# vshmyhlo/retinanet-tensorflow

Hardware: AMD Instinct MI355X
Metric: train images/sec (MobileNetV2-FPN RetinaNet 512x512, bs=2/GPU) (higher is better)
Workload: dtype f32

## Files before the change

include/rn_hip.h:

```cpp
#ifndef RN_HIP_H
#define RN_HIP_H

#include <stddef.h>
#include <stdint.h>

#ifdef __cplusplus
extern "C" {
#endif

typedef void* rn_stream_t;

enum rn_status {
  RN_OK = 0,
  RN_EINVAL = -1,
  RN_EUNSUPPORTED = -2,
  RN_EHIP = -3,
  RN_EWORKSPACE = -4
};

enum rn_act { RN_ACT_NONE = 0, RN_ACT_RELU = 1, RN_ACT_ELU = 2, RN_ACT_RELU6 = 3, RN_ACT_SIGMOID = 4 };
enum rn_loss_mode { RN_LOSS_BCE_DICE = 0, RN_LOSS_FOCAL = 1 };
enum rn_opt { RN_OPT_MOMENTUM = 0, RN_OPT_RMSPROP = 1, RN_OPT_ADAM = 2 };

#define RN_MAX_SEG 16

typedef struct rn_reduce_list rn_reduce_list;

#define RN_API_VERSION 408
int rn_version(void);
const char* rn_last_error(void);

void rn_same_pad(int n, int k, int s, int* out, int* pad_before);

typedef struct rn_conv_seg {
  const float* x;
  const float* wgt;
  const float* bias;
  float* y;
  const float* dy;
  float* dx;
  int32_t n, h, w;
  int32_t cout;
  int32_t x_ld;
  int32_t x_coff;
  int64_t wgt_bytes;
} rn_conv_seg;

typedef struct rn_conv_geom {
  int32_t kh, kw, stride, cin;
  int32_t groups;
} rn_conv_geom;

size_t rn_conv2d_fwd_workspace(const rn_conv_seg* segs, int nseg, const rn_conv_geom* g);
size_t rn_conv2d_dgrad_workspace(const rn_conv_seg* segs, int nseg, const rn_conv_geom* g);
int rn_conv2d_fwd(const rn_conv_seg* segs, int nseg, const rn_conv_geom* g, void* workspace, size_t workspace_bytes,
                  rn_stream_t stream);
int rn_conv2d_dgrad(const rn_conv_seg* segs, int nseg, const rn_conv_geom* g, void* workspace, size_t workspace_bytes,
                    rn_stream_t stream);
typedef struct rn_gn_rows {
  void* rows;
  int32_t rows_per_sample, per_group, groups;
} rn_gn_rows;
size_t rn_conv2d_stats_rows(const rn_conv_seg* segs, int nseg, const rn_conv_geom* g, size_t workspace_bytes, int groups,
                            rn_gn_rows* layout);
int rn_conv2d_fwd_stats(const rn_conv_seg* segs, int nseg, const rn_conv_geom* g, void* workspace, size_t workspace_bytes,
                        const rn_gn_rows* rows, rn_stream_t stream);

size_t rn_conv2d_dropout_rows(const rn_conv_seg* segs, int nseg, const rn_conv_geom* g, int groups, rn_gn_rows* layout, int* fused_ok);
int rn_conv2d_fwd_dropout(const rn_conv_seg* segs, int nseg, const rn_conv_geom* g, float rate, uint64_t seed, const uint64_t* seed_dev,
                          const rn_gn_rows* rows, rn_stream_t stream);

size_t rn_conv2d_wgrad_workspace(const rn_conv_seg* segs, int nseg, const rn_conv_geom* g);
int rn_conv2d_wgrad(const rn_conv_seg* segs, int nseg, const rn_conv_geom* g, float* dw, int accumulate,
                    void* workspace, size_t workspace_bytes, rn_stream_t stream, rn_reduce_list* defer);

int rn_conv2d_bwd(const rn_conv_seg* segs, int nseg, const rn_conv_geom* g, float* dw, void* workspace,
                  size_t workspace_bytes, rn_stream_t stream, rn_reduce_list* defer);

size_t rn_conv2d_bias_grad_workspace(int cout);
int rn_conv2d_bias_grad(const rn_conv_seg* segs, int nseg, const rn_conv_geom* g, float* dbias, void* workspace,
                        size_t workspace_bytes, rn_stream_t stream, rn_reduce_list* defer);

typedef struct rn_reduce_desc {
  const float* in;
  float* out;
  int32_t count;
  uint16_t nrows, accumulate;
} rn_reduce_desc;
struct rn_reduce_list {
  rn_reduce_desc* desc;
  int32_t capacity;
  int32_t count;
};
int rn_flush_reductions(rn_reduce_list* list, rn_stream_t stream);

size_t rn_conv3x3_winograd_workspace(const rn_conv_seg* segs, int nseg, int cin, int cout, int tile);
int rn_conv3x3_winograd_keep_bytes(const rn_conv_seg* segs, int nseg, int cin, int cout, int tile, size_t* v_bytes,
                                   size_t* urot_bytes);
int rn_conv3x3_winograd(const rn_conv_seg* segs, int nseg, int cin, int cout, const float* w, const float* bias,
                        int dgrad, int tile, void* workspace, size_t workspace_bytes, float* v_buf, float* urot_buf,
                        rn_stream_t stream);
int rn_gemm_batched(const float* A, const float* B, float* C, int M, int K, int N, int nbatch, int b_nk, rn_stream_t stream);
size_t rn_winograd_bwd_products_workspace(int M, int Kw, int Nw, int nbatch);
int rn_winograd_bwd_products(const float* Ad, const float* Bd, float* Cd, int M, int Kd, int Nd, const float* Aw,
                             const float* Bw, int Kw, int Nw, int nbatch, void* workspace, size_t workspace_bytes,
                             int* nsplit, rn_stream_t stream);
size_t rn_conv3x3_winograd_wgrad_workspace(const rn_conv_seg* segs, int nseg, int cin, int cout, int tile);
int rn_conv3x3_winograd_wgrad(const rn_conv_seg* segs, int nseg, int cin, int cout, float* dw, int accumulate, int tile,
                              void* workspace, size_t workspace_bytes, const float* v_buf, rn_stream_t stream);

size_t rn_conv3x3_winograd_bwd_workspace(const rn_conv_seg* segs, int nseg, int cin, int cout, int tile, int have_v, int have_urot);
int rn_conv3x3_winograd_bwd(const rn_conv_seg* segs, int nseg, int cin, int cout, const float* w, float* dw, int accumulate, int tile,
                            void* workspace, size_t workspace_bytes, const float* v_buf, const float* urot_buf, rn_stream_t stream);

int rn_set_product_mode(int mode);
int rn_get_product_mode(void);
int rn_set_x3_bfrag(int on);
int rn_get_x3_bfrag(void);
int rn_x3_bfrag_ok(int M, int K, int N);
size_t rn_x3_bfrag_bytes(int K, int N, int nbatch);
int rn_x3_pack_bfrag(const float* B, void* out, int K, int N, int nbatch, int b_nk, rn_stream_t stream);
int rn_gemm_batched_bfrag(const float* A, const void* Bfrag, float* C, int M, int K, int N, int nbatch, int fwd_name, rn_stream_t stream);

size_t rn_pack_weights_f16_bytes(int kh, int kw, int cin_g, int cout);
int rn_pack_weights_f16(const float* w, void* wt, int kh, int kw, int cin_g, int cout, rn_stream_t stream);
int rn_cast_f32_to_f16(const float* x, void* y, int64_t count, rn_stream_t stream);
int rn_pad_cast_rgb_f16(const float* x, void* y, int64_t pixels, rn_stream_t stream);
int rn_conv2d_fwd_f16(const rn_conv_seg* segs, int nseg, const rn_conv_geom* g, int out_f32, rn_stream_t stream);
typedef struct rn_f16_fold {
  const float* in_mean; const float* in_rstd; const float* in_gamma; const float* in_beta;
  int in_groups; int in_act;
  float* partial;
  const int32_t* seg_chunk_start;
  int32_t total_chunks;
} rn_f16_fold;
int rn_conv2d_f16_fold_rows(const rn_conv_seg* segs, int nseg, const rn_conv_geom* g);
int rn_conv2d_f16_stats_tiles(const rn_conv_seg* segs, int nseg, const rn_conv_geom* g, int32_t* tiles_per_sample);
int rn_conv2d_fwd_f16_fold(const rn_conv_seg* segs, int nseg, const rn_conv_geom* g, const rn_f16_fold* fold, rn_stream_t stream);
int rn_group_norm_finalize(const float* partial, int n, int rows_per_sample, int hw, int c, int groups, float eps, float* mean,
                           float* rstd, rn_stream_t stream);
int rn_group_norm_apply_f16(const void* x, const void* residual, void* y, int n, int hw, int c, int groups, const float* mean,
                            const float* rstd, const float* gamma, const float* beta, int act, int act_after_residual,
                            rn_stream_t stream);
typedef struct rn_gn_residual_norm {
  const float* mean; const float* rstd;
  const float* gamma; const float* beta;
  int groups;
} rn_gn_residual_norm;
int rn_group_norm_apply_res_f16(const void* x, const void* residual, const rn_gn_residual_norm* residual_norm, void* y, int n, int hw, int c,
                                int groups, const float* mean, const float* rstd, const float* gamma, const float* beta, int act,
                                int act_after_residual, rn_stream_t stream);

int rn_depthwise_fwd(const float* x, const float* wgt, float* y, int n, int h, int w, int c, int k, int stride,
                     rn_stream_t stream);
size_t rn_depthwise_stats_rows(int n, int h, int w, int c, int k, int stride, int groups, rn_gn_rows* layout);
int rn_depthwise_fwd_stats(const float* x, const float* wgt, float* y, int n, int h, int w, int c, int k, int stride,
                           const rn_gn_rows* rows, rn_stream_t stream);
int rn_depthwise_dgrad(const float* dy, const float* wgt, float* dx, int n, int h, int w, int c, int k,
                       int stride, rn_stream_t stream);
size_t rn_depthwise_wgrad_workspace(int n, int h, int w, int c, int k, int stride);
int rn_depthwise_bwd(const float* x, const float* dy, const float* wgt, float* dx, float* dw, int n, int h, int w, int c, int k,
                     int stride, void* workspace, size_t workspace_bytes, rn_stream_t stream, rn_reduce_list* defer);
int rn_depthwise_wgrad(const float* x, const float* dy, float* dw, int n, int h, int w, int c, int k, int stride,
                       void* workspace, size_t workspace_bytes, rn_stream_t stream, rn_reduce_list* defer);

typedef struct rn_dwgn_params {
  int32_t n, h, w, c;
  int32_t stride;
  int32_t groups, act;
  float eps, drop_rate;
  uint64_t drop_seed1, drop_seed2;
  const uint64_t* drop_seed_dev;
} rn_dwgn_params;
int rn_dwgn_supported(const rn_dwgn_params* p, int backward);
int rn_dwgn_fwd(const float* x, const float* gamma1, const float* beta1, const float* wgt, const float* gamma2,
                const float* beta2, float* y, float* stats, const rn_dwgn_params* p, rn_stream_t stream);
int rn_dwgn_bwd(const float* x, const float* dy, const float* gamma1, const float* beta1, const float* wgt,
                const float* gamma2, const float* beta2, const float* stats, float* dx, float* rows,
                const rn_dwgn_params* p, rn_stream_t stream);

typedef struct rn_gn_seg {
  const float* x;
  float* y;
  const float* residual;
  const float* dy;
  float* dx;
  float* dresidual;
  float* mean;
  float* rstd;
  int32_t n, hw;
  int32_t x_ld;
  int32_t dx_ld;
  int32_t dx_accumulate;
} rn_gn_seg;

typedef struct rn_gn_params {
  int32_t c, groups, act;
  int32_t act_after_residual;
  int32_t in_f16, out_f16;
  float eps;
  float drop_rate;
  uint64_t drop_seed;
  const uint64_t* drop_seed_dev;
  void* sync;
  const rn_gn_rows* stat_rows;
} rn_gn_params;

size_t rn_group_norm_sync_bytes(void);
int rn_group_norm_rows_ok(int c, int groups, int rows_per_sample, int per_group);
size_t rn_group_norm_workspace(const rn_gn_seg* segs, int nseg, const rn_gn_params* p);
int rn_group_norm_fwd(const rn_gn_seg* segs, int nseg, const rn_gn_params* p, const float* gamma,
                      const float* beta, void* workspace, size_t workspace_bytes, rn_stream_t stream);
int rn_group_norm_fwd_f16_tiles(const rn_gn_seg* segs, int nseg, const rn_gn_params* p, const float* gamma, const float* beta,
                                const float* partial, const int32_t* tiles_per_sample, rn_stream_t stream);
int rn_group_norm_bwd(const rn_gn_seg* segs, int nseg, const rn_gn_params* p, const float* gamma,
                      const float* beta, float* dgamma, float* dbeta, void* workspace, size_t workspace_bytes,
                      rn_stream_t stream, rn_reduce_list* defer);

int rn_act_fwd(const float* x, float* y, int64_t count, int act, rn_stream_t stream);
int rn_act_bwd(const float* x, const float* dy, float* dx, int64_t count, int act, rn_stream_t stream);
int rn_upsample_add_fwd(const float* lateral, const float* top, float* y, int n, int h, int w, int th, int tw, int c,
                        rn_stream_t stream);
int rn_upsample_add_bwd_top(const float* dy, float* dtop, int n, int h, int w, int th, int tw, int c,
                            rn_stream_t stream);

int rn_dropout(const float* x, float* y, int64_t count, float rate, uint64_t seed, const uint64_t* seed_dev,
               rn_stream_t stream);
int rn_dropout_strided(const float* x, float* y, int64_t pixels, int c, int x_ld, int x_coff, int y_ld, int y_coff, float rate,
                       uint64_t seed, const uint64_t* seed_dev, rn_stream_t stream);
int rn_maxpool_fwd(const float* x, float* y, uint8_t* argmax, int n, int h, int w, int c, int k, int stride,
                   rn_stream_t stream);
int rn_act_fwd_f16(const void* x, void* y, int64_t count, int act, rn_stream_t stream);
int rn_maxpool_fwd_f16(const void* x, void* y, int n, int h, int w, int c, int k, int stride, rn_stream_t stream);
int rn_maxpool_gn_fwd_f16(const void* x, void* y, int n, int h, int w, int c, int k, int stride, const float* mean, const float* rstd,
                          const float* gamma, const float* beta, int groups, int act, rn_stream_t stream);
int rn_upsample_add_fwd_f16(const void* lateral, const void* top, void* y, int n, int h, int w, int th, int tw, int c,
                            rn_stream_t stream);
int rn_maxpool_bwd(const float* x, const float* dy, float* dx, int n, int h, int w, int c, int k, int stride,
                   rn_stream_t stream);
int rn_maxpool_bwd_arg(const uint8_t* argmax, const float* dy, float* dx, int n, int h, int w, int c, int k, int stride,
                       rn_stream_t stream);
int rn_avgpool_fwd(const float* x, float* y, int n, int h, int w, int c, int k, int stride, rn_stream_t stream);
int rn_avgpool_bwd(const float* dy, float* dx, int n, int h, int w, int c, int k, int stride, rn_stream_t stream);

int rn_flip_width(const void* x, void* y, int64_t outer, int w, int64_t inner, int elem_bytes, int neg_mod, int neg_idx,
                  rn_stream_t stream);

int rn_resize_bilinear_normalize(const void* x, int in_u8, float* y, int n, int h, int w, int c, int oh, int ow,
                                 const float* mean, const float* stdv, rn_stream_t stream);

typedef struct rn_resize_desc {
  int32_t h, w;
  float hs, ws;
} rn_resize_desc;
int rn_resize_pair_u8(const uint8_t* raw, int64_t raw_capacity, const rn_resize_desc* desc, float* pair, int oh, int ow,
                      const float* mean, const float* stdv, rn_stream_t stream);

typedef struct rn_loss_seg {
  const float* cls_logit;
  const float* cls_label;
  const float* reg_pred;
  const float* reg_label;
  const uint8_t* trainable;
  float* d_cls_logit;
  float* d_reg_pred;
  int64_t rows;
} rn_loss_seg;

#define RN_LOSS_STATS_HEADER 8
size_t rn_loss_workspace(const rn_loss_seg* segs, int nseg, int num_classes);
int rn_loss_fwd(const rn_loss_seg* segs, int nseg, int num_classes, int mode, float* stats, float* class_loss_out,
                float* regr_loss_out, void* workspace, size_t workspace_bytes, rn_stream_t stream);
int rn_loss_bwd(const rn_loss_seg* segs, int nseg, int num_classes, int mode, const float* stats,
                const float* g_cls, const float* g_reg, rn_stream_t stream);

typedef struct rn_wino_gn {
  const float* in_rows;
  const float* in_gamma;
  const float* in_beta;
  int32_t in_groups, in_act;
  float in_eps;
  float* out_rows;
  int32_t out_groups;
  const void* u_ready;
  int32_t urot_ready;
} rn_wino_gn;
size_t rn_wino_gn_rows(const rn_conv_seg* segs, int nseg, int tile);
size_t rn_conv3x3_winograd_gn_u_bytes(int cin, int cout, int tile);
int rn_conv3x3_winograd_gn_weights(const float* w, int cin, int cout, int tile, void* u_out, size_t u_out_bytes, float* urot_out,
                                   rn_stream_t stream);
int rn_conv3x3_winograd_gn(const rn_conv_seg* segs, int nseg, int cin, int cout, const float* w, const float* bias, int tile,
                           const rn_wino_gn* gn, void* workspace, size_t workspace_bytes, float* v_buf, float* urot_buf,
                           rn_stream_t stream);
typedef struct rn_wino_gn_bwd {
  const float* in_rows;
  const float* in_gamma;
  const float* in_beta;
  int32_t in_groups, in_act;
  float in_eps;
  float* in_g_rows_group;
  float* in_g_rows_chan;
  const float* out_rows;
  const float* out_g_rows_group;
  const float* out_gamma;
  int32_t out_groups;
  float out_eps;
  int32_t defer_wgrad;
} rn_wino_gn_bwd;
int rn_conv3x3_winograd_gn_bwd(const rn_conv_seg* segs, int nseg, int cin, int cout, const float* w, float* dw, int accumulate,
                               int tile, const rn_wino_gn_bwd* gn, void* workspace, size_t workspace_bytes, const float* v_buf,
                               const float* urot_buf, rn_stream_t stream);
int rn_conv3x3_winograd_gn_bwd_wgrad(const rn_conv_seg* segs, int nseg, int cin, int cout, float* dw, int accumulate, int tile,
                                     void* workspace, size_t workspace_bytes, const float* v_buf, int urot_was_given, rn_stream_t stream);
int rn_reduce_rows(const float* in, float* out, int64_t count, int nrows, int accumulate, rn_stream_t stream, rn_reduce_list* defer);

typedef struct rn_mb_rows {
  float* rows;
  int32_t rows_per_sample, width, bn;
} rn_mb_rows;

typedef struct rn_mb_norm {
  const float* y;
  rn_mb_rows stat;
  float* mean; float* rstd;
  const float* gamma; const float* beta;
  int32_t c, groups, act;
  float eps, drop_rate;
  uint64_t drop_seed; const uint64_t* drop_seed_dev;
} rn_mb_norm;

int rn_mb_rows_max(void);
size_t rn_mb_compact_rows_layout(int n, const rn_mb_rows* in, rn_mb_rows* out);
int rn_mb_compact_rows(const rn_mb_rows* in, const rn_mb_rows* out, int n, rn_stream_t stream);

size_t rn_mb_pointwise_rows(int n, int hw, int cin, int cout, int groups, rn_mb_rows* layout);
int rn_mb_pointwise_fwd(const float* x, const rn_mb_norm* in, const float* residual, float* materialise, const float* w, float* y,
                        int n, int hw, int cin, int cout, const rn_mb_rows* stat_out, int stat_groups, rn_stream_t stream);
size_t rn_mb_depthwise_rows(int n, int h, int w, int c, int stride, int groups, rn_mb_rows* layout);
int rn_mb_depthwise_fwd(const rn_mb_norm* in, const float* w, float* y, int n, int h, int wd, int stride, const rn_mb_rows* stat_out,
                        int stat_groups, rn_stream_t stream);
int rn_mb_apply(const rn_mb_norm* in, const float* residual, float* out, int n, int hw, rn_stream_t stream);

enum { RN_MB_PHASE_POINTWISE = 0, RN_MB_PHASE_DEPTHWISE = 1 };
typedef struct rn_mb_phase {
  int32_t kind;
  const rn_mb_norm* in;
  const float* residual;
  float* materialise;
  const float* w; float* y;
  int32_t h, wd, cin, cout, stride;
  rn_mb_rows stat_out;
  int32_t stat_groups;
} rn_mb_phase;
size_t rn_mb_resident_sync_bytes(void);
size_t rn_mb_resident_rows(int kind, int n, int h, int wd, int cin, int cout, int stride, int groups, rn_mb_rows* layout);
int rn_mb_resident_fwd(const rn_mb_phase* phases, int nphase, int n, void* sync, rn_stream_t stream);

typedef struct rn_mb_dy {
  const float* dy;
  const rn_mb_norm* norm;
  const float* g;
  int32_t g_plain;
  rn_mb_rows grows;
} rn_mb_dy;
typedef struct rn_mb_gout {
  float* out;
  const float* add1; const float* add2;
  const rn_mb_norm* norm;
  int32_t store_plain;
  rn_mb_rows grows;
  float* planes;
} rn_mb_gout;
size_t rn_mb_pointwise_bwd_rows(int n, int hw, int cin, int cout, int groups, rn_mb_rows* layout);
size_t rn_mb_pointwise_bwd_workspace(int n, int hw, int cin, int cout);
int rn_mb_pointwise_bwd(const float* x, const rn_mb_norm* in, const rn_mb_dy* dy, const float* w, float* dw, const rn_mb_gout* gout,
                        int n, int hw, int cin, int cout, void* workspace, size_t workspace_bytes, rn_stream_t stream,
                        rn_reduce_list* defer);
size_t rn_mb_depthwise_bwd_rows(int n, int h, int w, int c, int stride, int groups, rn_mb_rows* layout);
size_t rn_mb_depthwise_bwd_workspace(int n, int h, int w, int c, int stride);
int rn_mb_depthwise_bwd(const rn_mb_norm* in, const rn_mb_dy* dy, const float* w, float* dw, const rn_mb_gout* gout, int n, int h,
                        int wd, int stride, void* workspace, size_t workspace_bytes, rn_stream_t stream, rn_reduce_list* defer);

int rn_iou(const float* a, int64_t na, const float* b, int64_t nb, int pairwise, float* out, int32_t* malformed,
           rn_stream_t stream);

int rn_anchor_assign(const float* boxes, const int32_t* class_ids, const int32_t* num_obj, int nimg, int max_obj,
                     const float* anchor_sizes, int num_anchors, int grid_h, int grid_w, int num_classes,
                     float* cls_out, float* reg_out, uint8_t* trainable_out, int32_t* argmax_out,
                     rn_stream_t stream);
#define RN_MAX_LEVELS 8
typedef struct rn_assign_level {
  const float* anchor_sizes;
  int grid_h, grid_w;
  float* cls_out;
  float* reg_out;
  uint8_t* trainable_out;
  int32_t* argmax_out;
} rn_assign_level;
int rn_anchor_assign_levels(const float* boxes, const int32_t* class_ids, const int32_t* num_obj, int nimg, int max_obj,
                            const rn_assign_level* levels, int nlevel, int num_anchors, int num_classes,
                            rn_stream_t stream);
int rn_anchor_assign_levels_pair(const float* boxes, const int32_t* class_ids, const int32_t* num_obj, int nimg, int max_obj,
                                 const rn_assign_level* levels, int nlevel, int num_anchors, int num_classes,
                                 rn_stream_t stream);

int rn_decode_boxes(const float* reg, const float* anchor_sizes, float* boxes, int n, int h, int w, int num_anchors,
                    rn_stream_t stream);

typedef struct rn_det_level {
  const void* prob;
  const float* boxes;
  int64_t rows_per_image;
  const void* regression;
  const float* anchor_sizes;
  int32_t grid_h, grid_w, num_anchors;
  int32_t prob_f16;
  int32_t regression_f16;
  int32_t prob_is_logit;
} rn_det_level;

typedef struct rn_det_params {
  int32_t n, num_classes, max_per_class;
  float score_threshold, iou_threshold;
  int64_t max_candidates;
} rn_det_params;

size_t rn_detect_workspace(const rn_det_level* levels, int nlevels, const rn_det_params* p);
int rn_detect(const rn_det_level* levels, int nlevels, const rn_det_params* p, float* out_boxes, float* out_scores,
              int32_t* out_class, int32_t* out_image, int64_t* out_anchor, int64_t* counts, void* workspace,
              size_t workspace_bytes, rn_stream_t stream);

int rn_boxes_decode(const rn_det_level* levels, int nlevels, const rn_det_params* p, float* out_boxes,
                    float* out_scores, int32_t* out_class, int32_t* out_image, int64_t* out_anchor, int64_t* counts,
                    void* workspace, size_t workspace_bytes, rn_stream_t stream);
size_t rn_nms_classwise_workspace(const rn_det_params* p);
int rn_nms_classwise(const float* boxes, const float* scores, const int32_t* class_ids, const int32_t* image_ids,
                     const int64_t* count_dev, const rn_det_params* p, float* out_boxes, float* out_scores,
                     int32_t* out_class, int32_t* out_image, int64_t* out_index, int64_t* counts, void* workspace,
                     size_t workspace_bytes, rn_stream_t stream);

#define RN_OPT_BLOCK 1024
size_t rn_optimizer_workspace(int64_t count);
int rn_grad_norm_l2reg(const float* w, const float* grad, const float* wd_per_block, int64_t count,
                       float grad_scale, float* out2, void* workspace, size_t workspace_bytes, rn_stream_t stream);
int rn_optimizer_step(int kind, float* w, const float* grad, float* state1, float* state2,
                      const float* wd_per_block, int64_t count, float lr, float grad_scale, float clip_norm,
                      const float* norm_sq, int64_t step, uint64_t* advance_counter, uint64_t advance_by, rn_stream_t stream);
int64_t rn_optimizer_norm_pairs(int64_t count);
int rn_optimizer_step_norm(int kind, float* w, const float* grad, float* state1, float* state2, const float* wd_per_block,
                           int64_t count, float lr, float grad_scale, int64_t step, uint64_t* advance_counter,
                           uint64_t advance_by, double* partial, rn_stream_t stream);
int rn_norm_reg_finalize(const double* partial, int64_t npairs, float* out2, rn_stream_t stream);
int rn_counter_add(uint64_t* counter, uint64_t inc, rn_stream_t stream);
int rn_zero(float* p, int64_t count, rn_stream_t stream);

typedef struct rn_add_seg { const float* a; const float* b; float* out; int64_t count; } rn_add_seg;
int rn_add_segs(const rn_add_seg* segs, int nseg, rn_stream_t stream);

int rn_debug_collective_standin(const void* src, void* dst, int64_t bytes, int blocks, float target_us, rn_stream_t stream);

#ifdef __cplusplus
}
#endif
#endif
```

retinanet-tensorflow_amd/_rn.py:

```python
import ctypes as C
import os

import torch

_HERE = os.path.dirname(os.path.abspath(__file__))
LIB_PATH = os.environ.get("RN_LIB_PATH") or os.path.join(_HERE, "librn_hip.so")

MAX_SEG = 16
ACT = {None: 0, "none": 0, "linear": 0, "relu": 1, "elu": 2, "relu6": 3, "sigmoid": 4}
LOSS_MODE = {"bce_dice": 0, "focal": 1}
OPT = {"momentum": 0, "rmsprop": 1, "adam": 2}
OPT_BLOCK = 1024
LOSS_STATS_HEADER = 8
API_VERSION = 408


class RnError(RuntimeError):
    pass


class ConvSeg(C.Structure):
    _fields_ = [("x", C.c_void_p), ("wgt", C.c_void_p), ("bias", C.c_void_p), ("y", C.c_void_p),
                ("dy", C.c_void_p), ("dx", C.c_void_p),
                ("n", C.c_int32), ("h", C.c_int32), ("w", C.c_int32), ("cout", C.c_int32),
                ("x_ld", C.c_int32), ("x_coff", C.c_int32), ("wgt_bytes", C.c_int64)]


class AssignLevel(C.Structure):
    _fields_ = [("anchor_sizes", C.c_void_p), ("grid_h", C.c_int32), ("grid_w", C.c_int32), ("cls_out", C.c_void_p),
                ("reg_out", C.c_void_p), ("trainable_out", C.c_void_p), ("argmax_out", C.c_void_p)]


class ConvGeom(C.Structure):
    _fields_ = [("kh", C.c_int32), ("kw", C.c_int32), ("stride", C.c_int32), ("cin", C.c_int32),
                ("groups", C.c_int32)]


class WinoGn(C.Structure):
    _fields_ = [("in_rows", C.c_void_p), ("in_gamma", C.c_void_p), ("in_beta", C.c_void_p), ("in_groups", C.c_int32),
                ("in_act", C.c_int32), ("in_eps", C.c_float), ("out_rows", C.c_void_p), ("out_groups", C.c_int32),
                ("u_ready", C.c_void_p), ("urot_ready", C.c_int32)]


class WinoGnBwd(C.Structure):
    _fields_ = [("in_rows", C.c_void_p), ("in_gamma", C.c_void_p), ("in_beta", C.c_void_p), ("in_groups", C.c_int32),
                ("in_act", C.c_int32), ("in_eps", C.c_float), ("in_g_rows_group", C.c_void_p), ("in_g_rows_chan", C.c_void_p),
                ("out_rows", C.c_void_p), ("out_g_rows_group", C.c_void_p), ("out_gamma", C.c_void_p),
                ("out_groups", C.c_int32), ("out_eps", C.c_float), ("defer_wgrad", C.c_int32)]


class ReduceDesc(C.Structure):
    _fields_ = [("in_", C.c_void_p), ("out", C.c_void_p), ("count", C.c_int32), ("nrows", C.c_uint16), ("accumulate", C.c_uint16)]


class ReduceList(C.Structure):
    _fields_ = [("desc", C.POINTER(ReduceDesc)), ("capacity", C.c_int32), ("count", C.c_int32)]

    @classmethod
    def make(cls, capacity=1024):
        arr = (ReduceDesc * capacity)()
        lst = cls(C.cast(arr, C.POINTER(ReduceDesc)), capacity, 0)
        lst._keep = arr
        return lst


class AddSeg(C.Structure):
    _fields_ = [("a", C.c_void_p), ("b", C.c_void_p), ("out", C.c_void_p), ("count", C.c_int64)]


class DwGnParams(C.Structure):
    _fields_ = [("n", C.c_int32), ("h", C.c_int32), ("w", C.c_int32), ("c", C.c_int32), ("stride", C.c_int32),
                ("groups", C.c_int32), ("act", C.c_int32), ("eps", C.c_float), ("drop_rate", C.c_float),
                ("drop_seed1", C.c_uint64), ("drop_seed2", C.c_uint64), ("drop_seed_dev", C.c_void_p)]


class GnSeg(C.Structure):
    _fields_ = [("x", C.c_void_p), ("y", C.c_void_p), ("residual", C.c_void_p), ("dy", C.c_void_p),
                ("dx", C.c_void_p), ("dresidual", C.c_void_p), ("mean", C.c_void_p), ("rstd", C.c_void_p),
                ("n", C.c_int32), ("hw", C.c_int32), ("x_ld", C.c_int32), ("dx_ld", C.c_int32), ("dx_accumulate", C.c_int32)]


class GnParams(C.Structure):
    _fields_ = [("c", C.c_int32), ("groups", C.c_int32), ("act", C.c_int32), ("act_after_residual", C.c_int32),
                ("in_f16", C.c_int32), ("out_f16", C.c_int32), ("eps", C.c_float),
                ("drop_rate", C.c_float), ("drop_seed", C.c_uint64), ("drop_seed_dev", C.c_void_p), ("sync", C.c_void_p),
                ("stat_rows", C.c_void_p)]


class GnRows(C.Structure):
    _fields_ = [("rows", C.c_void_p), ("rows_per_sample", C.c_int32), ("per_group", C.c_int32), ("groups", C.c_int32)]


class GnResidualNorm(C.Structure):
    _fields_ = [("mean", C.c_void_p), ("rstd", C.c_void_p), ("gamma", C.c_void_p), ("beta", C.c_void_p), ("groups", C.c_int)]


class F16Fold(C.Structure):
    _fields_ = [("in_mean", C.c_void_p), ("in_rstd", C.c_void_p), ("in_gamma", C.c_void_p), ("in_beta", C.c_void_p),
                ("in_groups", C.c_int32), ("in_act", C.c_int32), ("partial", C.c_void_p),
                ("seg_chunk_start", C.c_void_p), ("total_chunks", C.c_int32)]


class MbRows(C.Structure):
    _fields_ = [("rows", C.c_void_p), ("rows_per_sample", C.c_int32), ("width", C.c_int32), ("bn", C.c_int32)]


class MbNorm(C.Structure):
    _fields_ = [("y", C.c_void_p), ("stat", MbRows), ("mean", C.c_void_p), ("rstd", C.c_void_p), ("gamma", C.c_void_p),
                ("beta", C.c_void_p), ("c", C.c_int32), ("groups", C.c_int32), ("act", C.c_int32), ("eps", C.c_float),
                ("drop_rate", C.c_float), ("drop_seed", C.c_uint64), ("drop_seed_dev", C.c_void_p)]


class MbPhase(C.Structure):
    _fields_ = [("kind", C.c_int32), ("in_", C.POINTER(MbNorm)), ("residual", C.c_void_p), ("materialise", C.c_void_p),
                ("w", C.c_void_p), ("y", C.c_void_p), ("h", C.c_int32), ("wd", C.c_int32), ("cin", C.c_int32), ("cout", C.c_int32),
                ("stride", C.c_int32), ("stat_out", MbRows), ("stat_groups", C.c_int32)]


MB_PHASE_POINTWISE, MB_PHASE_DEPTHWISE = 0, 1


class MbDy(C.Structure):
    _fields_ = [("dy", C.c_void_p), ("norm", C.POINTER(MbNorm)), ("g", C.c_void_p), ("g_plain", C.c_int32), ("grows", MbRows)]


class MbGout(C.Structure):
    _fields_ = [("out", C.c_void_p), ("add1", C.c_void_p), ("add2", C.c_void_p), ("norm", C.POINTER(MbNorm)),
                ("store_plain", C.c_int32), ("grows", MbRows), ("planes", C.c_void_p)]


class LossSeg(C.Structure):
    _fields_ = [("cls_logit", C.c_void_p), ("cls_label", C.c_void_p), ("reg_pred", C.c_void_p),
                ("reg_label", C.c_void_p), ("trainable", C.c_void_p), ("d_cls_logit", C.c_void_p),
                ("d_reg_pred", C.c_void_p), ("rows", C.c_int64)]


class DetLevel(C.Structure):
    _fields_ = [("prob", C.c_void_p), ("boxes", C.c_void_p), ("rows_per_image", C.c_int64),
                ("regression", C.c_void_p), ("anchor_sizes", C.c_void_p),
                ("grid_h", C.c_int32), ("grid_w", C.c_int32), ("num_anchors", C.c_int32),
                ("prob_f16", C.c_int32), ("regression_f16", C.c_int32), ("prob_is_logit", C.c_int32)]


class DetParams(C.Structure):
    _fields_ = [("n", C.c_int32), ("num_classes", C.c_int32), ("max_per_class", C.c_int32),
                ("score_threshold", C.c_float), ("iou_threshold", C.c_float), ("max_candidates", C.c_int64)]


_lib = None

SYMBOLS = [
    "rn_version", "rn_last_error", "rn_same_pad",
    "rn_conv2d_fwd_workspace", "rn_conv2d_dgrad_workspace",
    "rn_zero", "rn_conv2d_fwd", "rn_conv2d_stats_rows", "rn_conv2d_fwd_stats", "rn_conv2d_dropout_rows", "rn_conv2d_fwd_dropout", "rn_depthwise_stats_rows", "rn_depthwise_fwd_stats", "rn_group_norm_rows_ok",
    "rn_conv2d_dgrad", "rn_conv2d_wgrad_workspace", "rn_conv2d_wgrad", "rn_conv2d_bwd",
    "rn_conv2d_bias_grad_workspace", "rn_conv2d_bias_grad", "rn_conv3x3_winograd_workspace", "rn_conv3x3_winograd",
    "rn_conv3x3_winograd_wgrad_workspace", "rn_conv3x3_winograd_wgrad", "rn_conv3x3_winograd_keep_bytes",
    "rn_conv3x3_winograd_bwd_workspace", "rn_conv3x3_winograd_bwd", "rn_flush_reductions", "rn_gemm_batched",
    "rn_winograd_bwd_products_workspace", "rn_winograd_bwd_products", "rn_wino_gn_rows", "rn_conv3x3_winograd_gn", "rn_conv3x3_winograd_gn_bwd", "rn_conv3x3_winograd_gn_bwd_wgrad", "rn_reduce_rows", "rn_resize_bilinear_normalize", "rn_resize_pair_u8",
    "rn_dwgn_supported", "rn_dwgn_fwd", "rn_dwgn_bwd", "rn_depthwise_fwd", "rn_depthwise_dgrad", "rn_depthwise_wgrad_workspace", "rn_depthwise_wgrad", "rn_depthwise_bwd",
    "rn_group_norm_sync_bytes", "rn_group_norm_workspace", "rn_group_norm_fwd", "rn_group_norm_bwd",
    "rn_act_fwd", "rn_act_bwd", "rn_upsample_add_fwd", "rn_upsample_add_bwd_top",
    "rn_pack_weights_f16", "rn_pack_weights_f16_bytes", "rn_cast_f32_to_f16", "rn_pad_cast_rgb_f16", "rn_conv2d_fwd_f16", "rn_conv2d_f16_fold_rows", "rn_conv2d_fwd_f16_fold", "rn_group_norm_finalize", "rn_group_norm_apply_f16", "rn_group_norm_apply_res_f16", "rn_maxpool_fwd_f16", "rn_maxpool_gn_fwd_f16", "rn_upsample_add_fwd_f16",
    "rn_act_fwd_f16", "rn_flip_width", "rn_dropout", "rn_dropout_strided", "rn_maxpool_fwd", "rn_maxpool_bwd", "rn_maxpool_bwd_arg", "rn_avgpool_fwd", "rn_avgpool_bwd",
    "rn_loss_workspace", "rn_loss_fwd", "rn_loss_bwd",
    "rn_iou", "rn_anchor_assign", "rn_anchor_assign_levels", "rn_anchor_assign_levels_pair", "rn_decode_boxes", "rn_detect_workspace", "rn_detect",
    "rn_boxes_decode", "rn_nms_classwise_workspace", "rn_nms_classwise",
    "rn_optimizer_workspace", "rn_grad_norm_l2reg", "rn_optimizer_step", "rn_counter_add", "rn_add_segs",
    "rn_mb_rows_max", "rn_mb_compact_rows_layout", "rn_mb_compact_rows", "rn_mb_pointwise_rows", "rn_mb_pointwise_fwd", "rn_mb_depthwise_rows", "rn_mb_depthwise_fwd", "rn_mb_apply",
    "rn_mb_resident_sync_bytes", "rn_mb_resident_rows", "rn_mb_resident_fwd", "rn_set_product_mode", "rn_get_product_mode",
    "rn_set_x3_bfrag", "rn_get_x3_bfrag", "rn_x3_bfrag_ok", "rn_x3_bfrag_bytes", "rn_x3_pack_bfrag", "rn_gemm_batched_bfrag", "rn_conv3x3_winograd_gn_u_bytes", "rn_conv3x3_winograd_gn_weights",
    "rn_conv2d_f16_stats_tiles", "rn_group_norm_fwd_f16_tiles",
    "rn_mb_pointwise_bwd_rows", "rn_mb_pointwise_bwd_workspace", "rn_mb_pointwise_bwd",
    "rn_mb_depthwise_bwd_rows", "rn_mb_depthwise_bwd_workspace", "rn_mb_depthwise_bwd",
    "rn_debug_collective_standin", "rn_optimizer_norm_pairs", "rn_optimizer_step_norm", "rn_norm_reg_finalize",
]


def lib():
    global _lib
    if _lib is None:
        if not os.path.exists(LIB_PATH):
            raise RnError("librn_hip.so not found at %s: build it with "
                          "`make -C retinanet-tensorflow_amd/csrc` (there is no fallback path)" % LIB_PATH)
        L = C.CDLL(LIB_PATH)
        if not hasattr(L, "rn_version") or L.rn_version() != API_VERSION:
            raise RnError("%s reports ABI version %s, these bindings need %d: rebuild it (make -C retinanet-tensorflow_amd/csrc)"
                          % (LIB_PATH, L.rn_version() if hasattr(L, "rn_version") else "none", API_VERSION))
        L.rn_last_error.restype = C.c_char_p
        L.rn_group_norm_sync_bytes.argtypes = []
        for name in ("rn_conv2d_wgrad_workspace", "rn_depthwise_wgrad_workspace", "rn_group_norm_workspace", "rn_group_norm_sync_bytes",
                     "rn_loss_workspace", "rn_detect_workspace", "rn_optimizer_workspace",
                     "rn_conv2d_bias_grad_workspace", "rn_nms_classwise_workspace", "rn_conv3x3_winograd_workspace", "rn_conv2d_fwd_workspace",
                     "rn_conv2d_dgrad_workspace",
                     "rn_conv3x3_winograd_wgrad_workspace", "rn_conv3x3_winograd_bwd_workspace", "rn_wino_gn_rows",
                     "rn_winograd_bwd_products_workspace", "rn_conv2d_stats_rows", "rn_depthwise_stats_rows", "rn_conv2d_dropout_rows",
                     "rn_x3_bfrag_bytes", "rn_conv3x3_winograd_gn_u_bytes"):
            getattr(L, name).restype = C.c_size_t
        L.rn_optimizer_workspace.argtypes = [C.c_int64]
        L.rn_dwgn_supported.argtypes = [C.c_void_p, C.c_int]
        L.rn_dwgn_fwd.argtypes = [C.c_void_p] * 10
        L.rn_dwgn_bwd.argtypes = [C.c_void_p] * 12
        L.rn_depthwise_fwd.argtypes = [C.c_void_p] * 3 + [C.c_int] * 6 + [C.c_void_p]
        L.rn_depthwise_dgrad.argtypes = [C.c_void_p] * 3 + [C.c_int] * 6 + [C.c_void_p]
        L.rn_depthwise_bwd.argtypes = [C.c_void_p] * 5 + [C.c_int] * 6 + [C.c_void_p, C.c_size_t, C.c_void_p, C.c_void_p]
        L.rn_depthwise_wgrad_workspace.argtypes = [C.c_int] * 6
        L.rn_depthwise_wgrad.argtypes = [C.c_void_p] * 3 + [C.c_int] * 6 + [C.c_void_p, C.c_size_t, C.c_void_p, C.c_void_p]
        L.rn_conv2d_fwd.argtypes = [C.c_void_p, C.c_int, C.c_void_p, C.c_void_p, C.c_size_t, C.c_void_p]
        L.rn_conv2d_dgrad.argtypes = [C.c_void_p, C.c_int, C.c_void_p, C.c_void_p, C.c_size_t, C.c_void_p]
        L.rn_zero.argtypes = [C.c_void_p, C.c_int64, C.c_void_p]
        L.rn_optimizer_norm_pairs.argtypes = [C.c_int64]
        L.rn_optimizer_norm_pairs.restype = C.c_int64
        L.rn_optimizer_step_norm.argtypes = [C.c_int] + [C.c_void_p] * 5 + [C.c_int64, C.c_float, C.c_float, C.c_int64, C.c_void_p, C.c_uint64,
                                             C.c_void_p, C.c_void_p]
        L.rn_norm_reg_finalize.argtypes = [C.c_void_p, C.c_int64, C.c_void_p, C.c_void_p]
        L.rn_debug_collective_standin.argtypes = [C.c_void_p, C.c_void_p, C.c_int64, C.c_int, C.c_float, C.c_void_p]
        L.rn_conv2d_stats_rows.argtypes = [C.c_void_p, C.c_int, C.c_void_p, C.c_size_t, C.c_int, C.c_void_p]
        L.rn_conv2d_fwd_stats.argtypes = [C.c_void_p, C.c_int, C.c_void_p, C.c_void_p, C.c_size_t, C.c_void_p, C.c_void_p]
        L.rn_conv2d_dropout_rows.argtypes = [C.c_void_p, C.c_int, C.c_void_p, C.c_int, C.c_void_p, C.c_void_p]
        L.rn_conv2d_fwd_dropout.argtypes = [C.c_void_p, C.c_int, C.c_void_p, C.c_float, C.c_uint64, C.c_void_p, C.c_void_p, C.c_void_p]
        L.rn_depthwise_stats_rows.argtypes = [C.c_int] * 7 + [C.c_void_p]
        L.rn_group_norm_rows_ok.argtypes = [C.c_int] * 4
        L.rn_depthwise_fwd_stats.argtypes = [C.c_void_p] * 3 + [C.c_int] * 6 + [C.c_void_p, C.c_void_p]
        L.rn_conv2d_fwd_workspace.argtypes = [C.c_void_p, C.c_int, C.c_void_p]
        L.rn_conv2d_dgrad_workspace.argtypes = [C.c_void_p, C.c_int, C.c_void_p]
        L.rn_conv2d_bwd.argtypes = [C.c_void_p, C.c_int, C.c_void_p, C.c_void_p, C.c_void_p, C.c_size_t, C.c_void_p, C.c_void_p]
        L.rn_conv2d_wgrad_workspace.argtypes = [C.c_void_p, C.c_int, C.c_void_p]
        L.rn_conv2d_wgrad.argtypes = [C.c_void_p, C.c_int, C.c_void_p, C.c_void_p, C.c_int, C.c_void_p,
                                      C.c_size_t, C.c_void_p, C.c_void_p]
        L.rn_conv2d_bias_grad_workspace.argtypes = [C.c_int]
        L.rn_conv3x3_winograd_workspace.argtypes = [C.c_void_p, C.c_int, C.c_int, C.c_int, C.c_int]
        L.rn_resize_bilinear_normalize.argtypes = [C.c_void_p, C.c_int, C.c_void_p] + [C.c_int] * 6 + [C.c_void_p, C.c_void_p,
                                                                                                         C.c_void_p]
        L.rn_resize_pair_u8.argtypes = [C.c_void_p, C.c_int64, C.c_void_p, C.c_void_p, C.c_int, C.c_int, C.c_void_p, C.c_void_p,
                                        C.c_void_p]
        L.rn_gemm_batched.argtypes = [C.c_void_p] * 3 + [C.c_int] * 5 + [C.c_void_p]
        L.rn_flush_reductions.argtypes = [C.c_void_p, C.c_void_p]
        L.rn_conv3x3_winograd_wgrad_workspace.argtypes = [C.c_void_p, C.c_int, C.c_int, C.c_int, C.c_int]
        L.rn_conv3x3_winograd_wgrad.argtypes = [C.c_void_p, C.c_int, C.c_int, C.c_int, C.c_void_p, C.c_int, C.c_int,
                                                C.c_void_p, C.c_size_t, C.c_void_p, C.c_void_p]
        L.rn_conv3x3_winograd_bwd_workspace.argtypes = [C.c_void_p] + [C.c_int] * 6
        L.rn_conv3x3_winograd_bwd.argtypes = [C.c_void_p, C.c_int, C.c_int, C.c_int, C.c_void_p, C.c_void_p, C.c_int, C.c_int,
                                              C.c_void_p, C.c_size_t, C.c_void_p, C.c_void_p, C.c_void_p]
        L.rn_conv3x3_winograd_keep_bytes.argtypes = [C.c_void_p, C.c_int, C.c_int, C.c_int, C.c_int, C.c_void_p, C.c_void_p]
        L.rn_conv3x3_winograd.argtypes = [C.c_void_p, C.c_int, C.c_int, C.c_int, C.c_void_p, C.c_void_p, C.c_int, C.c_int,
                                          C.c_void_p, C.c_size_t, C.c_void_p, C.c_void_p, C.c_void_p]
        L.rn_wino_gn_rows.argtypes = [C.c_void_p, C.c_int, C.c_int]
        L.rn_winograd_bwd_products_workspace.argtypes = [C.c_int] * 4
        L.rn_winograd_bwd_products.argtypes = [C.c_void_p] * 3 + [C.c_int] * 3 + [C.c_void_p] * 2 + [C.c_int] * 3 + \
                                              [C.c_void_p, C.c_size_t, C.c_void_p, C.c_void_p]
        L.rn_x3_bfrag_ok.argtypes = [C.c_int] * 3
        L.rn_conv2d_f16_stats_tiles.argtypes = [C.c_void_p, C.c_int, C.c_void_p, C.c_void_p]
        L.rn_group_norm_fwd_f16_tiles.argtypes = [C.c_void_p, C.c_int, C.c_void_p, C.c_void_p, C.c_void_p, C.c_void_p, C.c_void_p, C.c_void_p]
        L.rn_conv3x3_winograd_gn_u_bytes.argtypes = [C.c_int] * 3
        L.rn_conv3x3_winograd_gn_weights.argtypes = [C.c_void_p, C.c_int, C.c_int, C.c_int, C.c_void_p, C.c_size_t, C.c_void_p, C.c_void_p]
        L.rn_x3_bfrag_bytes.argtypes = [C.c_int] * 3
        L.rn_x3_pack_bfrag.argtypes = [C.c_void_p, C.c_void_p] + [C.c_int] * 4 + [C.c_void_p]
        L.rn_gemm_batched_bfrag.argtypes = [C.c_void_p] * 3 + [C.c_int] * 5 + [C.c_void_p]
        L.rn_set_x3_bfrag.argtypes = [C.c_int]
        L.rn_conv3x3_winograd_gn.argtypes = [C.c_void_p, C.c_int, C.c_int, C.c_int, C.c_void_p, C.c_void_p, C.c_int, C.c_void_p,
                                             C.c_void_p, C.c_size_t, C.c_void_p, C.c_void_p, C.c_void_p]
        L.rn_conv3x3_winograd_gn_bwd_wgrad.argtypes = [C.c_void_p, C.c_int, C.c_int, C.c_int, C.c_void_p, C.c_int, C.c_int, C.c_void_p, C.c_size_t,
                                                       C.c_void_p, C.c_int, C.c_void_p]
        L.rn_conv3x3_winograd_gn_bwd.argtypes = [C.c_void_p, C.c_int, C.c_int, C.c_int, C.c_void_p, C.c_void_p, C.c_int, C.c_int,
                                                 C.c_void_p, C.c_void_p, C.c_size_t, C.c_void_p, C.c_void_p, C.c_void_p]
        L.rn_reduce_rows.argtypes = [C.c_void_p, C.c_void_p, C.c_int64, C.c_int, C.c_int, C.c_void_p, C.c_void_p]
        L.rn_conv2d_bias_grad.argtypes = [C.c_void_p, C.c_int, C.c_void_p, C.c_void_p, C.c_void_p, C.c_size_t,
                                          C.c_void_p, C.c_void_p]
        L.rn_group_norm_workspace.argtypes = [C.c_void_p, C.c_int, C.c_void_p]
        L.rn_group_norm_fwd.argtypes = [C.c_void_p, C.c_int, C.c_void_p, C.c_void_p, C.c_void_p, C.c_void_p,
                                        C.c_size_t, C.c_void_p]
        L.rn_group_norm_bwd.argtypes = [C.c_void_p, C.c_int, C.c_void_p, C.c_void_p, C.c_void_p, C.c_void_p,
                                        C.c_void_p, C.c_void_p, C.c_size_t, C.c_void_p, C.c_void_p]
        L.rn_act_fwd.argtypes = [C.c_void_p, C.c_void_p, C.c_int64, C.c_int, C.c_void_p]
        L.rn_act_bwd.argtypes = [C.c_void_p, C.c_void_p, C.c_void_p, C.c_int64, C.c_int, C.c_void_p]
        L.rn_upsample_add_fwd.argtypes = [C.c_void_p] * 3 + [C.c_int] * 6 + [C.c_void_p]
        L.rn_upsample_add_bwd_top.argtypes = [C.c_void_p] * 2 + [C.c_int] * 6 + [C.c_void_p]
        L.rn_pack_weights_f16.argtypes = [C.c_void_p, C.c_void_p, C.c_int, C.c_int, C.c_int, C.c_int, C.c_void_p]
        L.rn_pack_weights_f16_bytes.argtypes = [C.c_int, C.c_int, C.c_int, C.c_int]
        L.rn_pack_weights_f16_bytes.restype = C.c_size_t
        L.rn_cast_f32_to_f16.argtypes = [C.c_void_p, C.c_void_p, C.c_int64, C.c_void_p]
        L.rn_pad_cast_rgb_f16.argtypes = [C.c_void_p, C.c_void_p, C.c_int64, C.c_void_p]
        L.rn_conv2d_fwd_f16.argtypes = [C.c_void_p, C.c_int, C.c_void_p, C.c_int, C.c_void_p]
        L.rn_conv2d_f16_fold_rows.argtypes = [C.c_void_p, C.c_int, C.c_void_p]
        L.rn_conv2d_fwd_f16_fold.argtypes = [C.c_void_p, C.c_int, C.c_void_p, C.c_void_p, C.c_void_p]
        L.rn_group_norm_finalize.argtypes = [C.c_void_p, C.c_int, C.c_int, C.c_int, C.c_int, C.c_int, C.c_float, C.c_void_p, C.c_void_p, C.c_void_p]
        L.rn_group_norm_apply_f16.argtypes = [C.c_void_p, C.c_void_p, C.c_void_p, C.c_int, C.c_int, C.c_int, C.c_int, C.c_void_p, C.c_void_p,
                                              C.c_void_p, C.c_void_p, C.c_int, C.c_int, C.c_void_p]
        L.rn_group_norm_apply_res_f16.argtypes = [C.c_void_p, C.c_void_p, C.c_void_p, C.c_void_p, C.c_int, C.c_int, C.c_int, C.c_int, C.c_void_p,
                                                  C.c_void_p, C.c_void_p, C.c_void_p, C.c_int, C.c_int, C.c_void_p]
        L.rn_maxpool_fwd_f16.argtypes = [C.c_void_p] * 2 + [C.c_int] * 6 + [C.c_void_p]
        L.rn_maxpool_gn_fwd_f16.argtypes = [C.c_void_p] * 2 + [C.c_int] * 6 + [C.c_void_p] * 4 + [C.c_int] * 2 + [C.c_void_p]
        L.rn_upsample_add_fwd_f16.argtypes = [C.c_void_p] * 3 + [C.c_int] * 6 + [C.c_void_p]
        L.rn_act_fwd_f16.argtypes = [C.c_void_p, C.c_void_p, C.c_int64, C.c_int, C.c_void_p]
        L.rn_flip_width.argtypes = [C.c_void_p, C.c_void_p, C.c_int64, C.c_int, C.c_int64, C.c_int, C.c_int, C.c_int, C.c_void_p]
        L.rn_dropout_strided.argtypes = [C.c_void_p, C.c_void_p, C.c_int64] + [C.c_int] * 5 + [C.c_float, C.c_uint64, C.c_void_p, C.c_void_p]
        L.rn_dropout.argtypes = [C.c_void_p, C.c_void_p, C.c_int64, C.c_float, C.c_uint64, C.c_void_p, C.c_void_p]
        L.rn_maxpool_fwd.argtypes = [C.c_void_p] * 3 + [C.c_int] * 6 + [C.c_void_p]
        L.rn_maxpool_bwd_arg.argtypes = [C.c_void_p] * 3 + [C.c_int] * 6 + [C.c_void_p]
        L.rn_maxpool_bwd.argtypes = [C.c_void_p] * 3 + [C.c_int] * 6 + [C.c_void_p]
        L.rn_avgpool_fwd.argtypes = [C.c_void_p] * 2 + [C.c_int] * 6 + [C.c_void_p]
        L.rn_avgpool_bwd.argtypes = [C.c_void_p] * 2 + [C.c_int] * 6 + [C.c_void_p]
        L.rn_loss_workspace.argtypes = [C.c_void_p, C.c_int, C.c_int]
        L.rn_loss_fwd.argtypes = [C.c_void_p, C.c_int, C.c_int, C.c_int, C.c_void_p, C.c_void_p, C.c_void_p, C.c_void_p, C.c_size_t,
                                  C.c_void_p]
        L.rn_loss_bwd.argtypes = [C.c_void_p, C.c_int, C.c_int, C.c_int, C.c_void_p, C.c_void_p, C.c_void_p,
                                  C.c_void_p]
        L.rn_iou.argtypes = [C.c_void_p, C.c_int64, C.c_void_p, C.c_int64, C.c_int, C.c_void_p, C.c_void_p, C.c_void_p]
        L.rn_anchor_assign.argtypes = [C.c_void_p] * 3 + [C.c_int, C.c_int, C.c_void_p] + [C.c_int] * 4 + \
                                      [C.c_void_p] * 4 + [C.c_void_p]
        L.rn_anchor_assign_levels.argtypes = [C.c_void_p] * 3 + [C.c_int, C.c_int, C.c_void_p, C.c_int, C.c_int, C.c_int,
                                              C.c_void_p]
        L.rn_anchor_assign_levels_pair.argtypes = L.rn_anchor_assign_levels.argtypes
        L.rn_decode_boxes.argtypes = [C.c_void_p] * 3 + [C.c_int] * 4 + [C.c_void_p]
        L.rn_detect_workspace.argtypes = [C.c_void_p, C.c_int, C.c_void_p]
        L.rn_detect.argtypes = [C.c_void_p, C.c_int, C.c_void_p] + [C.c_void_p] * 6 + [C.c_void_p, C.c_size_t,
                                                                                     C.c_void_p]
        L.rn_boxes_decode.argtypes = L.rn_detect.argtypes
        L.rn_nms_classwise_workspace.argtypes = [C.c_void_p]
        L.rn_nms_classwise.argtypes = [C.c_void_p] * 5 + [C.c_void_p] + [C.c_void_p] * 6 + [C.c_void_p, C.c_size_t,
                                                                                        C.c_void_p]
        L.rn_grad_norm_l2reg.argtypes = [C.c_void_p] * 3 + [C.c_int64, C.c_float, C.c_void_p, C.c_void_p,
                                                             C.c_size_t, C.c_void_p]
        L.rn_optimizer_step.argtypes = [C.c_int] + [C.c_void_p] * 5 + [C.c_int64, C.c_float, C.c_float,
                                                                       C.c_float, C.c_void_p, C.c_int64,
                                                                       C.c_void_p, C.c_uint64, C.c_void_p]
        L.rn_counter_add.argtypes = [C.c_void_p, C.c_uint64, C.c_void_p]
        L.rn_add_segs.argtypes = [C.c_void_p, C.c_int, C.c_void_p]
        for name in ("rn_mb_pointwise_rows", "rn_mb_depthwise_rows", "rn_mb_pointwise_bwd_rows", "rn_mb_pointwise_bwd_workspace",
                     "rn_mb_depthwise_bwd_rows", "rn_mb_depthwise_bwd_workspace"):
            getattr(L, name).restype = C.c_size_t
        L.rn_mb_resident_sync_bytes.restype = C.c_size_t
        L.rn_mb_resident_rows.restype = C.c_size_t
        L.rn_mb_resident_rows.argtypes = [C.c_int] * 8 + [C.c_void_p]
        L.rn_mb_resident_fwd.argtypes = [C.c_void_p, C.c_int, C.c_int, C.c_void_p, C.c_void_p]
        L.rn_mb_compact_rows_layout.restype = C.c_size_t
        L.rn_mb_compact_rows_layout.argtypes = [C.c_int, C.c_void_p, C.c_void_p]
        L.rn_mb_compact_rows.argtypes = [C.c_void_p, C.c_void_p, C.c_int, C.c_void_p]
        L.rn_mb_pointwise_rows.argtypes = [C.c_int] * 5 + [C.c_void_p]
        L.rn_mb_pointwise_fwd.argtypes = [C.c_void_p] * 6 + [C.c_int] * 4 + [C.c_void_p, C.c_int, C.c_void_p]
        L.rn_mb_depthwise_rows.argtypes = [C.c_int] * 6 + [C.c_void_p]
        L.rn_mb_depthwise_fwd.argtypes = [C.c_void_p] * 3 + [C.c_int] * 4 + [C.c_void_p, C.c_int, C.c_void_p]
        L.rn_mb_apply.argtypes = [C.c_void_p] * 3 + [C.c_int, C.c_int, C.c_void_p]
        L.rn_mb_pointwise_bwd_rows.argtypes = [C.c_int] * 5 + [C.c_void_p]
        L.rn_mb_pointwise_bwd_workspace.argtypes = [C.c_int] * 4
        L.rn_mb_pointwise_bwd.argtypes = [C.c_void_p] * 6 + [C.c_int] * 4 + [C.c_void_p, C.c_size_t, C.c_void_p, C.c_void_p]
        L.rn_mb_depthwise_bwd_rows.argtypes = [C.c_int] * 6 + [C.c_void_p]
        L.rn_mb_depthwise_bwd_workspace.argtypes = [C.c_int] * 5
        L.rn_mb_depthwise_bwd.argtypes = [C.c_void_p] * 5 + [C.c_int] * 4 + [C.c_void_p, C.c_size_t, C.c_void_p, C.c_void_p]
        L.rn_same_pad.argtypes = [C.c_int, C.c_int, C.c_int, C.POINTER(C.c_int), C.POINTER(C.c_int)]
        L.rn_same_pad.restype = None
        _lib = L
    return _lib


def check(status, what):
    if status != 0:
        raise RnError("%s failed (status %d): %s" % (what, status, lib().rn_last_error().decode()))


def same_pad(n, k, s):
    out = -(-n // s)
    total = max((out - 1) * s + k - n, 0)
    return out, total // 2


def ptr(t):
    if t is None:
        return None
    if not t.is_cuda:
        raise RnError("rn_hip kernels need device tensors (got a CPU tensor): there is no CPU fallback")
    if not t.is_contiguous():
        raise RnError("rn_hip kernels need contiguous tensors")
    return t.data_ptr()


def f32(t):
    if t.dtype != torch.float32:
        raise RnError("this rn_hip kernel is fp32 (got %s)" % t.dtype)
    return ptr(t)


def f16(t):
    if t.dtype != torch.float16:
        raise RnError("this rn_hip kernel takes fp16 storage (got %s)" % t.dtype)
    return ptr(t)


def stream():
    return C.c_void_p(torch.cuda.current_stream().cuda_stream)


_workspaces = {}
WORKSPACE_MIN_BYTES = 256 << 20


SIDE_STREAMS = set()
_side_streams = {}


_sync_words = {}


def sync_counters(device):
    h = stream().value or 0
    capturing = torch.cuda.is_current_stream_capturing() if device.type == 'cuda' else False
    key = (device.type, device.index, h if h in SIDE_STREAMS else 0)
    if key[2] == 0:
        _hand_over(('gn',) + key, h, device)
    t = _sync_words.get(key)
    if t is None:
        if capturing:
            raise RnError("the grid-resident GroupNorm's exchange region must exist before graph capture (run the step once eagerly)")
        t = torch.zeros(lib().rn_group_norm_sync_bytes() // 4, dtype=torch.int32, device=device)
        _sync_words[key] = t
    return t


_resident_words = {}
_region_owner = {}


def _hand_over(key, h, device):
    last = _region_owner.get(key)
    if last is not None and last != h and device.type == 'cuda' and not torch.cuda.is_current_stream_capturing():
        try:
            ev = torch.cuda.Event()
            ev.record(torch.cuda.ExternalStream(last, device=device) if last else torch.cuda.default_stream(device))
            torch.cuda.current_stream(device).wait_event(ev)
        except RuntimeError:
            pass
    if device.type != 'cuda' or not torch.cuda.is_current_stream_capturing():
        _region_owner[key] = h


def resident_sync(device):
    h = stream().value or 0
    key = (device.type, device.index, h if h in SIDE_STREAMS else 0)
    if key[2] == 0:
        _hand_over(('mb',) + key, h, device)
    t = _resident_words.get(key)
    if t is None:
        if device.type == 'cuda' and torch.cuda.is_current_stream_capturing():
            raise RnError("the resident section's counters must exist before graph capture (run the step once eagerly)")
        t = torch.zeros(lib().rn_mb_resident_sync_bytes() // 4, dtype=torch.int32, device=device)
        _resident_words[key] = t
    return t


def resident_errors():
    e = 0
    for t in _resident_words.values():
        e |= int(t[512].item())
    return e


def barrier_timeout_sources():
    return (sum(int(t[2].item()) for t in {id(t): t for t in _sync_words.values()}.values()),
            sum(1 for t in _resident_words.values() if int(t[512].item()) != 0))


def barrier_timeouts():
    return (sum(int(t[2].item()) for t in {id(t): t for t in _sync_words.values()}.values()) +
            sum(1 for t in _resident_words.values() if int(t[512].item()) != 0))


def reset_barrier_timeouts():
    for t in {id(t): t for t in _sync_words.values()}.values():
        t[2] = 0
    for t in _resident_words.values():
        t.zero_()


def side_stream(device, index=0):
    key = (device.type, device.index, index)
    st = _side_streams.get(key)
    if st is None:
        lo, hi = torch.cuda.Stream.priority_range() if hasattr(torch.cuda.Stream, 'priority_range') else (0, 0)
        st = torch.cuda.Stream(device=device, priority=int(os.environ.get('RN_SIDE_PRIO', lo)))
        _side_streams[key] = st
        SIDE_STREAMS.add(st.cuda_stream)
    return st


def join_side_streams(device, skip=()):
    cur = torch.cuda.current_stream(device)
    for (t, i, idx), st in _side_streams.items():
        if t == device.type and i == device.index and idx not in skip:
            cur.wait_stream(st)


def workspace(nbytes, device):
    h = torch.cuda.current_stream(device).cuda_stream if device.type == "cuda" else 0
    key = (device.type, device.index, h if h in SIDE_STREAMS else 0)
    ws = _workspaces.get(key)
# ... 8 lines not shown
```

retinanet-tensorflow_amd/csrc/mb_common.h:

```cpp
#pragma once
#include <stdlib.h>
#include <string.h>

#include "conv_tiles.h"
#include "rn_common.h"

namespace {
using namespace rn_tiles;

constexpr int T = 256;
constexpr int KMAX = 1024;
constexpr int GMAX = 32;
constexpr int RMAX = 256;

struct RowsDev { float2* rows; int R, W, bn; };
struct NormDev {
  const float* y; RowsDev st; float* mean; float* rstd; const float* gamma; const float* beta;
  int c, groups, cpg, act;
  float eps, drop_rate, keep_scale;
  uint64_t seed; const uint64_t* seed_dev;
};

template <int NJ>
struct ChanPre { float g[NJ], b[NJ]; };
template <int NJ>
__device__ __forceinline__ void prefetch_chan(const float* gamma, const float* beta, int c0, int nc, int tid, ChanPre<NJ>& p) {
#pragma unroll
  for (int j = 0; j < NJ; ++j) {
    const int i = min(tid % T + j * T, nc - 1);
    p.g[j] = (tid < T) ? gamma[c0 + i] : 0.f;
    p.b[j] = (tid < T && beta) ? beta[c0 + i] : 0.f;
  }
}
struct GroupPre { float mean, rstd; };
__device__ __forceinline__ GroupPre prefetch_groups(const NormDev& nd, int sample, int g0, int ng, int tid) {
  GroupPre p = {0.f, 1.f};
  if (nd.st.rows == nullptr && tid < T) {
    const int g = g0 + min(tid, ng - 1);
    p.mean = nd.mean[sample * nd.groups + g];
    p.rstd = nd.rstd[sample * nd.groups + g];
  }
  return p;
}

__device__ __forceinline__ void merge_rows(const RowsDev& st, int sample, int cpg, int C, int g0, int ng, double (*part)[2],
                                           double (*tot)[2], int tid) {
  const int RL = T / ng, gl = tid % ng, rl = tid / ng;
  double S = 0.0, Q = 0.0;
  if (tid < T && rl < RL) {
    const int g = g0 + gl;
    const int t0 = (g * cpg) / st.bn, t1 = (min((g + 1) * cpg, C) - 1) / st.bn;
    const double w1 = t1 > t0 ? 1.0 : 0.0;
    const float2* __restrict__ base = st.rows + (size_t)sample * st.R * st.W + g;
    for (int r0 = rl; r0 < st.R; r0 += 8 * RL) {
      float2 a[8], b[8];
#pragma unroll
      for (int j = 0; j < 8; ++j) {
        const size_t rr = (size_t)min(r0 + j * RL, st.R - 1) * st.W;
        a[j] = base[rr + t0];
        b[j] = base[rr + t1];
      }
#pragma unroll
      for (int j = 0; j < 8; ++j)
        if (r0 + j * RL < st.R) {
          S += (double)a[j].x + w1 * (double)b[j].x;
          Q += (double)a[j].y + w1 * (double)b[j].y;
        }
    }
  }
  if (tid < T) { part[tid][0] = S; part[tid][1] = Q; }
  __syncthreads();
  if (tid < ng) {
    S = 0.0; Q = 0.0;
    for (int l = 0; l < RL; ++l) { S += part[l * ng + tid][0]; Q += part[l * ng + tid][1]; }
    tot[tid][0] = S; tot[tid][1] = Q;
  }
  __syncthreads();
}

__device__ __forceinline__ void group_stats(const NormDev& nd, int sample, int hw, int g0, int ng, bool publish, void* scratch,
                                            float (*gstat)[2], const GroupPre& pre, int tid) {
  if (nd.st.rows) {
    double (*part)[2] = reinterpret_cast<double (*)[2]>(scratch);
    double (*tot)[2] = part + T;
    merge_rows(nd.st, sample, nd.cpg, nd.c, g0, ng, part, tot, tid);
    if (tid < ng) {
      const double m = (double)hw * (double)nd.cpg;
      const double mean = tot[tid][0] / m;
      double var = tot[tid][1] / m - mean * mean;
      if (var < 0.0) var = 0.0;
      const float rstd = (float)(1.0 / sqrt(var + (double)nd.eps));
      gstat[tid][0] = (float)mean; gstat[tid][1] = rstd;
      if (publish) { nd.mean[sample * nd.groups + g0 + tid] = (float)mean; nd.rstd[sample * nd.groups + g0 + tid] = rstd; }
    }
  } else if (tid < ng) {
    gstat[tid][0] = pre.mean; gstat[tid][1] = pre.rstd;
  }
  __syncthreads();
}

template <int NJ>
__device__ __forceinline__ void scale_shift_table(const NormDev& nd, int c0, int nc, int g0, const float (*gstat)[2], float* sc, float* sh,
                                                  const ChanPre<NJ>& p, int tid) {
  if (tid < T) {
#pragma unroll
    for (int j = 0; j < NJ; ++j) {
      const int i = tid + j * T;
      if (i < nc) {
        const int g = (c0 + i) / nd.cpg - g0;
        const float s = gstat[g][1] * p.g[j];
        sc[i] = s;
        sh[i] = p.b[j] - gstat[g][0] * s;
      }
    }
  }
  __syncthreads();
}

template <int ACT>
__device__ __forceinline__ float act_of(float z, int act_rt) { return ACT >= 0 ? rn::act_fwd(z, ACT) : rn::act_fwd(z, act_rt); }
template <int ACT>
__device__ __forceinline__ float actgrad_of(float z, int act_rt) { return ACT >= 0 ? rn::act_grad(z, ACT) : rn::act_grad(z, act_rt); }

__device__ __forceinline__ void keep4(uint64_t seed, uint64_t eidx, float rate, float keep, float (&m)[4]) {
  const uint32_t s_lo = (uint32_t)seed, s_hi = (uint32_t)(seed >> 32);
  uint32_t h0 = (uint32_t)eidx * 0x9E3779B1u + s_lo;
#pragma unroll
  for (int j = 0; j < 4; ++j) {
    uint32_t h = h0 ^ s_hi;
    h0 += 0x9E3779B1u;
    h ^= h >> 16; h *= 0x85EBCA6Bu;
    h ^= h >> 13; h *= 0xC2B2AE35u;
    h ^= h >> 16;
    m[j] = ((float)(h >> 8) * (1.0f / 16777216.0f) >= rate) ? keep : 0.f;
  }
}
__device__ __forceinline__ float keep1(uint64_t seed, uint64_t eidx, float rate, float keep) {
  uint32_t h = ((uint32_t)eidx * 0x9E3779B1u + (uint32_t)seed) ^ (uint32_t)(seed >> 32);
  h ^= h >> 16; h *= 0x85EBCA6Bu;
  h ^= h >> 13; h *= 0xC2B2AE35u;
  h ^= h >> 16;
  return ((float)(h >> 8) * (1.0f / 16777216.0f) >= rate) ? keep : 0.f;
}

template <int ACT>
__device__ __forceinline__ float4 norm_act_drop(float4 v, float4 sc, float4 sh, int act_rt, bool drop, float rate, float keep,
                                                uint64_t seed, uint64_t eidx) {
  float o[4] = {fmaf(v.x, sc.x, sh.x), fmaf(v.y, sc.y, sh.y), fmaf(v.z, sc.z, sh.z), fmaf(v.w, sc.w, sh.w)};
#pragma unroll
  for (int j = 0; j < 4; ++j) o[j] = act_of<ACT>(o[j], act_rt);
  if (drop) {
    float m[4];
    keep4(seed, eidx, rate, keep, m);
#pragma unroll
    for (int j = 0; j < 4; ++j) o[j] *= m[j];
  }
  return make_float4(o[0], o[1], o[2], o[3]);
}

template <int BM, int BN, int WM, int WN>
__device__ __forceinline__ void reduce_group_rows(const float (&s1)[BN / WN / 32], const float (&s2)[BN / WN / 32], float* smem, float2* row,
                                                  int n0, int C, int cpg, int tile_n, int tid, const float* wgt, float* plane1, float* plane2) {
  constexpr int TN = BN / WN / 32;
  const bool on = tid < WM * WN * 64;
  const int lane = tid & 63, wave = (tid >> 6) % (WM * WN), wm = wave / WN, wn = wave % WN, l31 = lane & 31;
  float* red = smem;
  float* chan = smem + WM * BN * 2;
#pragma unroll
  for (int tn = 0; tn < TN; ++tn) {
    float a = s1[tn], b = s2[tn];
    a += __shfl_xor(a, 32, 64);
    b += __shfl_xor(b, 32, 64);
    if (on && lane < 32) {
      const int col = wn * (BN / WN) + tn * 32 + l31;
      red[(wm * BN + col) * 2 + 0] = a;
      red[(wm * BN + col) * 2 + 1] = b;
    }
  }
  __syncthreads();
  if (tid < BN) {
    float t1 = 0.f, t2 = 0.f;
#pragma unroll
    for (int w = 0; w < WM; ++w) { t1 += red[(w * BN + tid) * 2 + 0]; t2 += red[(w * BN + tid) * 2 + 1]; }
    chan[tid * 2 + 0] = t1; chan[tid * 2 + 1] = t2;
    if (plane1 && n0 + tid < C) { plane1[n0 + tid] = t1; plane2[n0 + tid] = t2; }
  }
  __syncthreads();
  const int cend = min(n0 + BN, C);
  const int g_lo = n0 / cpg, g_hi = (cend - 1) / cpg;
  if (tid <= g_hi - g_lo) {
    const int g = g_lo + tid;
    const int c_lo = max(g * cpg, n0), c_hi = min((g + 1) * cpg, cend);
    float t1 = 0.f, t2 = 0.f;
    for (int c = c_lo; c < c_hi; ++c) {
      const float w = wgt ? wgt[c] : 1.f;
      t1 += w * chan[(c - n0) * 2 + 0]; t2 += w * chan[(c - n0) * 2 + 1];
    }
    row[g + tile_n] = make_float2(t1, t2);
  }
}

template <int KS, int NACC, int TG = T>
__device__ __forceinline__ void sum_groups(f32x16* acc, float* red, int grp, int lt) {
  if (KS == 1) return;
  if (grp > 0) {
#pragma unroll
    for (int i = 0; i < NACC; ++i)
#pragma unroll
      for (int r = 0; r < 16; ++r) red[((size_t)((grp - 1) * NACC + i) * 16 + r) * TG + lt] = acc[i][r];
  }
  __syncthreads();
  if (grp == 0) {
    for (int g = 1; g < KS; ++g)
#pragma unroll
      for (int i = 0; i < NACC; ++i)
#pragma unroll
        for (int r = 0; r < 16; ++r) acc[i][r] += red[((size_t)((g - 1) * NACC + i) * 16 + r) * TG + lt];
  }
  __syncthreads();
}

struct PwFwdArgs {
  int dbg;
  const float* x; const float* res; float* mat; const float* w; float* y;
  NormDev in;
  int n, hw, cin, cout, tiles_n;
  RowsDev ost; int ocpg;
};

struct DwFwdArgs {
  int dbg;
  NormDev in; const float* w; float* y;
  int n, h, wd, c, stride, oh, ow, pad_t, pad_l;
  int th, tw, tiles_h, tiles_w, sw, nslab, ph, pw;
  int tpb, nblk;
  RowsDev ost; int ocpg;
};
constexpr int NP = 8;

struct PatchElem { int q, pix; bool inside, live; };
__device__ __forceinline__ PatchElem patch_elem(int idx, int total, int SQ, int pw, int y0, int x0, int h, int w) {
  PatchElem e;
  e.live = idx < total;
  const int i = min(idx, total - 1);
  const int pp = i / SQ;
  e.q = i - pp * SQ;
  const int py = pp / pw, px = pp - py * pw;
  const int yy = y0 + py, xx = x0 + px;
  e.inside = (unsigned)yy < (unsigned)h && (unsigned)xx < (unsigned)w;
  e.pix = min(max(yy, 0), h - 1) * w + min(max(xx, 0), w - 1);
  return e;
}
__device__ __forceinline__ int patch_pack(int idx, int total, int SQ, int pw) {
  const int i = min(idx, total - 1);
  const int pp = i / SQ, q = i - pp * SQ;
  const int py = pp / pw, px = pp - py * pw;
  return q | (py << 8) | (px << 16) | (idx < total ? (1 << 24) : 0);
}
__device__ __forceinline__ PatchElem patch_at(int pk, int y0, int x0, int h, int w) {
  PatchElem e;
  e.live = (pk >> 24) != 0;
  e.q = pk & 255;
  const int yy = y0 + ((pk >> 8) & 255), xx = x0 + ((pk >> 16) & 255);
  e.inside = (unsigned)yy < (unsigned)h && (unsigned)xx < (unsigned)w;
  e.pix = min(max(yy, 0), h - 1) * w + min(max(xx, 0), w - 1);
  return e;
}

int dbg_word(const char* kernel) {
  const char* e = getenv("RN_MB_DBG");
  if (!e || strncmp(e, kernel, 3) != 0 || e[3] != ':') return 0;
  return atoi(e + 4);
}
int fill_norm(const rn_mb_norm* s, NormDev* d, int n, bool need_rows, const char* what) {
  RN_CHECK_ARG(s && s->y && s->mean && s->rstd && s->gamma && s->beta, "%s: null pointer in rn_mb_norm", what);
  RN_CHECK_ARG(s->c >= 4 && s->groups >= 1 && s->c % s->groups == 0, "%s: c=%d groups=%d", what, s->c, s->groups);
  RN_UNSUPPORTED(s->c % 4 != 0 || s->c > KMAX || s->groups > GMAX, "%s: c=%d (multiple of 4, <= %d), groups=%d (<= %d)", what, s->c, KMAX,
                 s->groups, GMAX);
  RN_CHECK_ARG(s->drop_rate >= 0.f && s->drop_rate < 1.f, "%s: drop_rate %f", what, s->drop_rate);
  d->y = s->y; d->mean = s->mean; d->rstd = s->rstd; d->gamma = s->gamma; d->beta = s->beta;
  d->c = s->c; d->groups = s->groups; d->cpg = s->c / s->groups; d->act = s->act;
  d->eps = s->eps; d->drop_rate = s->drop_rate; d->keep_scale = s->drop_rate > 0.f ? 1.f / (1.f - s->drop_rate) : 1.f;
  d->seed = s->drop_seed; d->seed_dev = s->drop_seed_dev;
  d->st.rows = (float2*)s->stat.rows; d->st.R = s->stat.rows_per_sample; d->st.W = s->stat.width; d->st.bn = s->stat.bn;
  if (need_rows) RN_CHECK_ARG(s->stat.rows, "%s: the forward pass needs the statistic rows", what);
  if (s->stat.rows) {
    RN_CHECK_ARG(d->st.R >= 1 && d->st.W >= d->groups && d->st.bn >= 1, "%s: bad row layout", what);
    RN_UNSUPPORTED(d->st.R > RMAX || d->cpg > d->st.bn, "%s: %d rows per sample (<= %d) / groups wider than an N-tile", what, d->st.R, RMAX);
  }
  (void)n;
  return RN_OK;
}

struct PwCfg { int id, bm, bn, ks; };
PwCfg pw_cfg(int n, int hw, int kdim, int ncols) {
  static const bool no_ks = getenv("RN_MB_NO_SPLITK") != nullptr;
  static const bool no_t32 = getenv("RN_MB_NO_TILE32") != nullptr;
  if (const char* f = getenv("RN_MB_PW_CFG")) {
    const int c = atoi(f);
    if (c == 1 && hw % 128 == 0) return {1, 128, 32, 1};
    if (c == 2 && hw % 128 == 0) return {2, 128, 64, 1};
    if (c == 0) return {0, 64, 64, 1};
  }
  const long m = (long)n * hw;
  if (hw % 128 == 0 && ncols <= 32 && m / 128 >= 128) return {1, 128, 32, 1};
  if (hw % 128 == 0 && hw > 4096) return {2, 128, 64, 1};
  const long blocks64 = m / 64 * rn::ceil_div(ncols, 64);
  const int nkt = rn::ceil_div(kdim, BK);
  if (blocks64 <= 96 && nkt >= 4 && !no_ks) {
    if (!no_t32) return {3, 32, 32, nkt >= 16 ? 8 : 4};
    return {0, 64, 64, 4};
  }
  return {0, 64, 64, 1};
}

int dw_slab(int c, int cpg) {
  int unit = cpg;
  while (unit % 4) unit += cpg;
  for (int sw = unit; sw <= c; sw += unit)
    if (c % sw == 0 && sw >= 32) return sw <= 128 ? sw : 0;
  return c <= 128 ? c : 0;
}

struct DwPlan { int th, tw, tiles_h, tiles_w, sw, nslab, ph, pw, tpb, nblk; };
int dw_tiles_per_block(long blocks, int ntile) {
  static const int forced = getenv("RN_MB_DW_TPB") ? atoi(getenv("RN_MB_DW_TPB")) : 0;
  static const int target = getenv("RN_MB_DW_BLOCKS") ? atoi(getenv("RN_MB_DW_BLOCKS")) : 512;
  int tpb = forced > 0 ? forced : (int)(blocks / (target > 0 ? target : 512));
  if (tpb < 1) tpb = 1;
  if (tpb > ntile) tpb = ntile;
  return tpb;
}
bool dw_plan(int n, int oh, int ow, int c, int stride, int cpg, DwPlan* p) {
  p->sw = dw_slab(c, cpg);
  if (!p->sw) return false;
  p->nslab = c / p->sw;
  static const int th_big = getenv("RN_MB_DWF_TH") ? atoi(getenv("RN_MB_DWF_TH")) : 8;
  static const int tw_big = getenv("RN_MB_DWF_TW") ? atoi(getenv("RN_MB_DWF_TW")) : 8;
  const bool big = (long)oh * ow >= 16384;
  int th = stride == 1 ? (big ? th_big : 8) : (big ? th_big / 2 : 4), tw = big ? tw_big : 8;
  if (th > oh) th = oh;
  if (tw > ow) tw = ow;
  auto blocks = [&]() { return (long)n * rn::ceil_div(oh, th) * rn::ceil_div(ow, tw) * p->nslab; };
  auto patch = [&]() { return (long)((th - 1) * stride + 3) * ((tw - 1) * stride + 3) * (p->sw / 4); };
  while ((blocks() < 384 && th * tw > 16) || (patch() > NP * T && th * tw > 1)) {
    if (th >= tw) th = (th + 1) / 2; else tw = (tw + 1) / 2;
  }
  if (patch() > NP * T) return false;
// ... 17 lines not shown
```

retinanet-tensorflow_amd/csrc/mbconv.hip:

```cpp
#include "mb_common.h"

namespace {


template <int BM, int BN, int WM, int WN, bool NORM, int ACT, int KS, int NST>
__global__ __launch_bounds__(WM* WN * 64 * KS) void mb_pw_fwd_kernel(const PwFwdArgs a) {
  constexpr int TG = WM * WN * 64;
  constexpr bool RES = NORM && ACT != RN_ACT_ELU && ACT != RN_ACT_RELU6 && ACT != RN_ACT_RELU;
  static_assert(TG * KS >= T || !NORM, "the prologue needs 256 threads");
  constexpr int TM = BM / WM / 32, TN = BN / WN / 32;
  constexpr int KQ = BK / 4, A_RPP = TG / KQ, A_PASS = BM / A_RPP;
  constexpr int NQ = BN / 4, B_RPP = TG / NQ, B_PASS = BK / B_RPP;
  static_assert(A_PASS >= 1 && B_PASS >= 1 && BM % A_RPP == 0 && BK % B_RPP == 0, "tile/threads mismatch");
  constexpr int OPF = BM * LDK + BK * BN;
  static_assert(KS * OPF * 4 >= (T + GMAX) * 16 && OPF >= (WM + 1) * BN * 2, "operand tiles double as scratch");
  static_assert(KS == 1 || KS * OPF >= (KS - 1) * TM * TN * 16 * TG, "operand tiles double as the split-K exchange");
  __shared__ __attribute__((aligned(16))) float smem[KS * OPF];
  __shared__ __attribute__((aligned(16))) float tab[NORM ? 2 * KMAX : 4];
  __shared__ float gstat[NORM ? GMAX : 1][2];
  const int tid = threadIdx.x, grp = tid / TG, lt = tid % TG, lane = lt & 63, wave = lt >> 6;
  float* As = smem + grp * OPF;
  float* Bs = As + BM * LDK;
  const int wm = wave / WN, wn = wave % WN;
  const int bid = rn::xcd_remap(blockIdx.x, gridDim.x);
  const int tile_n = bid % a.tiles_n, tile_m = bid / a.tiles_n;
  const int K = a.cin, N = a.cout, M = a.n * a.hw;
  const int m0 = tile_m * BM, n0 = tile_n * BN;
  const int sample = m0 / a.hw;
  const float* asrc = NORM ? a.in.y : a.x;
  const __amdgpu_buffer_rsrc_t xa = make_rsrc(asrc, (unsigned)M * K * 4u);
  const __amdgpu_buffer_rsrc_t xr = make_rsrc(a.res ? a.res : asrc, (unsigned)M * K * 4u);
  const __amdgpu_buffer_rsrc_t wb = make_rsrc(a.w, (unsigned)K * N * 4u);
  const bool has_res = RES && a.res != nullptr;

  const int kq = lt % KQ, arow = lt / KQ;
  const int nq = lt % NQ;
  const int bcol = n0 + nq * 4;
  const unsigned boff0 = bcol < N ? ((unsigned)(lt / NQ) * N + bcol) * 4u : OOB;
  const int nk = (K + BK - 1) / BK, nit = (nk + KS - 1) / KS;
  float4 ra[NST][A_PASS], rr[RES ? NST : 1][A_PASS], rb[NST][B_PASS];
  auto load_tiles = [&](int it, const int st) {
    const int kt = it * KS + grp;
    const int k = kt * BK + kq * 4;
    const bool kok = k < K;
#pragma unroll
    for (int i = 0; i < A_PASS; ++i) {
      const unsigned off = kok ? ((unsigned)(m0 + arow + i * A_RPP) * K + k) * 4u : OOB;
      ra[st][i] = Vec<4>::load(xa, off);
      if (RES) rr[st][i] = Vec<4>::load(xr, has_res ? off : OOB);
    }
    const unsigned bo = (kt < nk && boff0 != OOB) ? boff0 + (unsigned)kt * BK * N * 4u : OOB;
#pragma unroll
    for (int j = 0; j < B_PASS; ++j) rb[st][j] = Vec<4>::load(wb, bo == OOB ? OOB : bo + (unsigned)j * B_RPP * N * 4u);
  };
  ChanPre<NORM ? KMAX / T : 1> pre;
  GroupPre gpre = {0.f, 1.f};
  if (NORM) {
    prefetch_chan(a.in.gamma, a.in.beta, 0, K, tid, pre);
    gpre = prefetch_groups(a.in, sample, 0, a.in.groups, tid);
  }
#pragma unroll
  for (int st = 0; st < NST; ++st)
    if (st < nit) load_tiles(st, st);
  uint64_t seed = 0;
  bool drop = false;
  if (NORM) {
    group_stats(a.in, sample, a.hw, 0, a.in.groups, tile_n == 0 && m0 == sample * a.hw, smem, gstat, gpre, tid);
    scale_shift_table(a.in, 0, K, 0, gstat, tab, tab + KMAX, pre, tid);
    drop = a.in.drop_rate > 0.f;
    seed = a.in.seed + (a.in.seed_dev ? *a.in.seed_dev : 0ull);
  }
  if (a.dbg == 1) return;
  const bool write_mat = NORM && a.mat != nullptr && tile_n == 0;
  auto store_tiles = [&](int it, const int st) {
    const int k = (it * KS + grp) * BK + kq * 4;
#pragma unroll
    for (int i = 0; i < A_PASS; ++i) {
      float4 v = ra[st][i];
      if (NORM) {
        if (k < K) {
          const int m = m0 + arow + i * A_RPP;
          const float4 sc = *reinterpret_cast<const float4*>(&tab[k]);
          const float4 sh = *reinterpret_cast<const float4*>(&tab[KMAX + k]);
          v = norm_act_drop<ACT>(v, sc, sh, a.in.act, drop, a.in.drop_rate, a.in.keep_scale, seed, (uint64_t)m * K + k);
          if (RES) { v.x += rr[st][i].x; v.y += rr[st][i].y; v.z += rr[st][i].z; v.w += rr[st][i].w; }
          if (write_mat) *reinterpret_cast<float4*>(a.mat + (size_t)m * K + k) = v;
        } else {
          v = make_float4(0.f, 0.f, 0.f, 0.f);
        }
      }
      *reinterpret_cast<float4*>(&As[(arow + i * A_RPP) * LDK + kq * 4]) = v;
    }
#pragma unroll
    for (int j = 0; j < B_PASS; ++j) *reinterpret_cast<float4*>(&Bs[(lt / NQ + j * B_RPP) * BN + nq * 4]) = rb[st][j];
  };

  f32x16 acc[TM][TN];
  zero_acc<TM, TN>(acc);
  for (int it0 = 0; it0 < nit; it0 += NST) {
#pragma unroll
    for (int st = 0; st < NST; ++st) {
      const int it = it0 + st;
      if (it < nit) {
        store_tiles(it, st);
        __syncthreads();
        if (it + NST < nit) load_tiles(it + NST, st);
        if (it * KS + grp < nk) mma_ktile<BM, BN, WM, WN, false, false>(As, Bs, acc, wm, wn, lane);
        __syncthreads();
      }
    }
  }
  if (a.dbg == 2) { if (acc[0][0][0] == 123.456f) a.y[0] = 0.f; return; }
  sum_groups<KS, TM * TN, TG>(&acc[0][0], smem, grp, lt);
  if (grp == 0) store_tile<BM, BN, WM, WN>(acc, a.y, nullptr, m0, n0, M, N, N, wm, wn, lane);
  if (a.dbg == 3) return;
  if (a.ost.rows) {
    float2* row = a.ost.rows + ((size_t)sample * a.ost.R + (m0 - sample * a.hw) / BM) * a.ost.W;
    float s1[TN], s2[TN];
#pragma unroll
    for (int tn = 0; tn < TN; ++tn) {
      s1[tn] = 0.f; s2[tn] = 0.f;
#pragma unroll
      for (int tm = 0; tm < TM; ++tm)
#pragma unroll
        for (int r = 0; r < 16; ++r) { const float v = acc[tm][tn][r]; s1[tn] += v; s2[tn] = fmaf(v, v, s2[tn]); }
    }
    reduce_group_rows<BM, BN, WM, WN>(s1, s2, smem, row, n0, N, a.ocpg, tile_n, tid, nullptr, nullptr, nullptr);
  }
}


template <int ACT, bool PF>
__global__ __launch_bounds__(T) void mb_dw_fwd_kernel(const DwFwdArgs a) {
  extern __shared__ __attribute__((aligned(16))) float dsm[];
  __shared__ __attribute__((aligned(16))) float tab[2 * 128];
  __shared__ float gstat[GMAX][2];
  const int tid = threadIdx.x;
  const int bid = rn::xcd_remap(blockIdx.x, gridDim.x);
  const int slab = bid % a.nslab;
  const int tt = bid / a.nslab;
  const int ntile = a.tiles_h * a.tiles_w;
  const int blk = tt % a.nblk, sample = tt / a.nblk;
  const int tile_lo = blk * a.tpb, tile_hi = min(tile_lo + a.tpb, ntile);
  const int C = a.c, SW = a.sw, SQ = SW >> 2, c0 = slab * SW;
  const int g0 = c0 / a.in.cpg, ng = SW / a.in.cpg;
  ChanPre<1> pre;
  prefetch_chan(a.in.gamma, a.in.beta, c0, SW, tid, pre);
  const GroupPre gpre = prefetch_groups(a.in, sample, g0, ng, tid);
  const int total = a.ph * a.pw * SQ;
  const __amdgpu_buffer_rsrc_t xs = make_rsrc(a.in.y + (size_t)sample * a.h * a.wd * C + c0, (unsigned)(a.h * a.wd * C - c0) * 4u);
  float4 pv[NP];
  int pk[NP];
#pragma unroll
  for (int j = 0; j < NP; ++j) pk[j] = patch_pack(tid + j * T, total, SQ, a.pw);
  auto load_patch = [&](int tile) {
    const int ih0 = (tile / a.tiles_w) * a.th * a.stride - a.pad_t, iw0 = (tile % a.tiles_w) * a.tw * a.stride - a.pad_l;
#pragma unroll
    for (int j = 0; j < NP; ++j) {
      const PatchElem e = patch_at(pk[j], ih0, iw0, a.h, a.wd);
      pv[j] = Vec<4>::load(xs, (e.live && e.inside) ? ((unsigned)e.pix * C + e.q * 4) * 4u : OOB);
    }
  };
  load_patch(tile_lo);
  const int lanes = T / SQ, q4 = tid % SQ, pl = tid / SQ;
  float4 wv[9];
#pragma unroll
  for (int t = 0; t < 9; ++t) wv[t] = *reinterpret_cast<const float4*>(a.w + (size_t)t * C + c0 + min(q4, SQ - 1) * 4);
  group_stats(a.in, sample, a.h * a.wd, g0, ng, blk == 0, dsm, gstat, gpre, tid);
  scale_shift_table(a.in, c0, SW, g0, gstat, tab, tab + 128, pre, tid);
  if (a.dbg == 1) { if (pv[0].x == 123.456f && wv[0].x == 1.f) a.y[0] = 0.f; return; }
  const bool drop = a.in.drop_rate > 0.f;
  const uint64_t seed = a.in.seed + (a.in.seed_dev ? *a.in.seed_dev : 0ull);
  const uint64_t samp_off = (uint64_t)sample * a.h * a.wd * C;
  float s1[4] = {0.f, 0.f, 0.f, 0.f}, s2[4] = {0.f, 0.f, 0.f, 0.f};
  float* __restrict__ ys = a.y + (size_t)sample * a.oh * a.ow * C + c0 + q4 * 4;
  auto process_tile = [&](int tile) {
    const int oh0 = (tile / a.tiles_w) * a.th, ow0 = (tile % a.tiles_w) * a.tw;
    const int ih0 = oh0 * a.stride - a.pad_t, iw0 = ow0 * a.stride - a.pad_l;
#pragma unroll
    for (int j = 0; j < NP; ++j) {
      const PatchElem e = patch_at(pk[j], ih0, iw0, a.h, a.wd);
      if (e.live) {
        float4 o = norm_act_drop<ACT>(pv[j], *reinterpret_cast<const float4*>(&tab[e.q * 4]), *reinterpret_cast<const float4*>(&tab[128 + e.q * 4]),
                                      a.in.act, drop, a.in.drop_rate, a.in.keep_scale, seed, samp_off + (uint64_t)e.pix * C + c0 + e.q * 4);
        if (!e.inside) o = make_float4(0.f, 0.f, 0.f, 0.f);
        *reinterpret_cast<float4*>(&dsm[(size_t)(tid + j * T) * 4]) = o;
      }
    }
    __syncthreads();
    if (PF && tile + 1 < tile_hi) load_patch(tile + 1);
    if (pl < lanes) {
      for (int p = pl; p < a.th * a.tw; p += lanes) {
        const int oy = p / a.tw, ox = p - oy * a.tw;
        const int oh_ = oh0 + oy, ow_ = ow0 + ox;
        if (oh_ < a.oh && ow_ < a.ow) {
          float4 acc = make_float4(0.f, 0.f, 0.f, 0.f);
#pragma unroll
          for (int kh = 0; kh < 3; ++kh)
#pragma unroll
            for (int kw = 0; kw < 3; ++kw) {
              const float4 xv = *reinterpret_cast<const float4*>(&dsm[((size_t)(oy * a.stride + kh) * a.pw + ox * a.stride + kw) * SW + q4 * 4]);
              const float4 w4 = wv[kh * 3 + kw];
              acc.x = fmaf(xv.x, w4.x, acc.x); acc.y = fmaf(xv.y, w4.y, acc.y);
              acc.z = fmaf(xv.z, w4.z, acc.z); acc.w = fmaf(xv.w, w4.w, acc.w);
            }
          *reinterpret_cast<float4*>(ys + (size_t)(oh_ * a.ow + ow_) * C) = acc;
          s1[0] += acc.x; s1[1] += acc.y; s1[2] += acc.z; s1[3] += acc.w;
          s2[0] = fmaf(acc.x, acc.x, s2[0]); s2[1] = fmaf(acc.y, acc.y, s2[1]);
          s2[2] = fmaf(acc.z, acc.z, s2[2]); s2[3] = fmaf(acc.w, acc.w, s2[3]);
        }
      }
    }
    __syncthreads();
  };
  if (PF) {
#pragma nounroll
    for (int tile = tile_lo; tile < tile_hi; ++tile) process_tile(tile);
  } else {
    process_tile(tile_lo);
#pragma nounroll
    for (int tile = tile_lo + 1; tile < tile_hi; ++tile) {
      load_patch(tile);
      process_tile(tile);
    }
  }
  if (!a.ost.rows || a.dbg == 3) return;
  float (*red)[8] = reinterpret_cast<float (*)[8]>(dsm);
  float (*chan)[2] = reinterpret_cast<float (*)[2]>(dsm + T * 8);
#pragma unroll
  for (int j = 0; j < 4; ++j) { red[tid][j] = s1[j]; red[tid][4 + j] = s2[j]; }
  __syncthreads();
  for (int e = tid; e < SQ * 8; e += T) {
    const int qd = e >> 3, comp = e & 7;
    float t = 0.f;
    for (int l = 0; l < lanes; ++l) t += red[l * SQ + qd][comp];
    chan[qd * 4 + (comp & 3)][comp >> 2] = t;
  }
  __syncthreads();
  const int ong = SW / a.ocpg, og0 = c0 / a.ocpg;
  if (tid < ong) {
    float t1 = 0.f, t2 = 0.f;
    for (int j = 0; j < a.ocpg; ++j) { t1 += chan[tid * a.ocpg + j][0]; t2 += chan[tid * a.ocpg + j][1]; }
    a.ost.rows[((size_t)sample * a.ost.R + blk) * a.ost.W + og0 + tid] = make_float2(t1, t2);
  }
}

struct ApplyArgs { NormDev in; const float* res; float* out; int n, hw, ppb; };

__global__ __launch_bounds__(T) void mb_apply_kernel(const ApplyArgs a) {
  __shared__ __attribute__((aligned(16))) double scratch[(T + GMAX) * 2];
  __shared__ __attribute__((aligned(16))) float tab[2 * KMAX];
  __shared__ float gstat[GMAX][2];
  const int tid = threadIdx.x, sample = blockIdx.y, C = a.in.c, CQ = C >> 2;
  ChanPre<KMAX / T> pre;
  prefetch_chan(a.in.gamma, a.in.beta, 0, C, tid, pre);
  const GroupPre gpre = prefetch_groups(a.in, sample, 0, a.in.groups, tid);
  group_stats(a.in, sample, a.hw, 0, a.in.groups, blockIdx.x == 0, scratch, gstat, gpre, tid);
  scale_shift_table(a.in, 0, C, 0, gstat, tab, tab + KMAX, pre, tid);
  const bool drop = a.in.drop_rate > 0.f;
  const uint64_t seed = a.in.seed + (a.in.seed_dev ? *a.in.seed_dev : 0ull);
  const int p_begin = blockIdx.x * a.ppb, p_end = min(p_begin + a.ppb, a.hw);
  const size_t base = (size_t)sample * a.hw * C;
  for (int i = tid; i < (p_end - p_begin) * CQ; i += T) {
    const int p = p_begin + i / CQ, q = i % CQ;
    const size_t e = base + (size_t)p * C + q * 4;
    const float4 v = *reinterpret_cast<const float4*>(a.in.y + e);
    float4 o = norm_act_drop<-1>(v, *reinterpret_cast<const float4*>(&tab[q * 4]), *reinterpret_cast<const float4*>(&tab[KMAX + q * 4]),
                                 a.in.act, drop, a.in.drop_rate, a.in.keep_scale, seed, (uint64_t)e);
    if (a.res) {
      const float4 r = *reinterpret_cast<const float4*>(a.res + e);
      o.x += r.x; o.y += r.y; o.z += r.z; o.w += r.w;
    }
    *reinterpret_cast<float4*>(a.out + e) = o;
  }
}

struct CompactArgs { const float2* in; float2* out; int R, W, F, Rout; };
__global__ __launch_bounds__(T) void mb_compact_rows_kernel(const CompactArgs a) {
  __shared__ double part[T][2];
  const int tid = threadIdx.x, ro = blockIdx.x, sample = blockIdx.y;
  const int RL = T / a.W, e = tid % a.W, rl = tid / a.W;
  const int r_begin = ro * a.F, r_end = min(r_begin + a.F, a.R);
  double S = 0.0, Q = 0.0;
  if (rl < RL) {
    const float2* __restrict__ base = a.in + (size_t)sample * a.R * a.W + e;
    for (int r0 = r_begin + rl; r0 < r_end; r0 += 8 * RL) {
      float2 v[8];
#pragma unroll
      for (int j = 0; j < 8; ++j) v[j] = base[(size_t)min(r0 + j * RL, r_end - 1) * a.W];
#pragma unroll
      for (int j = 0; j < 8; ++j)
        if (r0 + j * RL < r_end) { S += (double)v[j].x; Q += (double)v[j].y; }
    }
  }
  part[tid][0] = S; part[tid][1] = Q;
  __syncthreads();
  if (tid < a.W) {
    S = 0.0; Q = 0.0;
    for (int l = 0; l < RL; ++l) { S += part[l * a.W + tid][0]; Q += part[l * a.W + tid][1]; }
    a.out[((size_t)sample * a.Rout + ro) * a.W + tid] = make_float2((float)S, (float)Q);
  }
}

struct DyDev {
  const float* dy;
  const float* g; int g_plain; NormDev nd; RowsDev grows;
};
struct GoutDev {
  float* out; const float* add1; const float* add2;
  int has_norm; NormDev nd; int store_plain; RowsDev grows; float* planes; long plane_stride;
};

template <int NJ>
__device__ __forceinline__ void dy_table(const DyDev& d, int sample, int hw, int c0, int nc, void* scratch, float (*gstat)[2], float (*gc)[2],
                                         float* tab, int stride, const GroupPre& gp, const ChanPre<NJ>& p, int tid) {
  const int g0 = c0 / d.nd.cpg, ng = (c0 + nc - 1) / d.nd.cpg - g0 + 1;
  double (*part)[2] = reinterpret_cast<double (*)[2]>(scratch);
  double (*tot)[2] = part + T;
  merge_rows(d.grows, sample, d.nd.cpg, d.nd.c, g0, ng, part, tot, tid);
  if (tid < ng) {
    const double m = (double)hw * (double)d.nd.cpg;
    gc[tid][0] = (float)(tot[tid][0] / m); gc[tid][1] = (float)(tot[tid][1] / m);
    gstat[tid][0] = gp.mean; gstat[tid][1] = gp.rstd;
  }
  __syncthreads();
  if (tid < T) {
#pragma unroll
    for (int j = 0; j < NJ; ++j) {
      const int i = tid + j * T;
      if (i < nc) {
        const int g = (c0 + i) / d.nd.cpg - g0;
        const float mean = gstat[g][0], rstd = gstat[g][1], c1 = gc[g][0], c2 = gc[g][1];
        tab[i] = rstd * p.g[j];
        tab[stride + i] = rstd * (rstd * c2 * mean - c1);
        tab[2 * stride + i] = -rstd * rstd * c2;
      }
    }
  }
  __syncthreads();
// ... 492 lines not shown
      if (a_slot(j, row, col)) {
        float4 v = va[j];
        if (!Y_IS_A && a.has_in)
          v = norm_act_drop<-1>(v, *reinterpret_cast<const float4*>(&tabA[col]), *reinterpret_cast<const float4*>(&tabA[CI + col]),
                                a.in.act, drop_in, a.in.drop_rate, a.in.keep_scale, seed_in, (uint64_t)(p + row) * KI + col);
        *reinterpret_cast<float4*>(&At[row * SA + col]) = v;
      }
    }
    float yo[NE], ad[NE];
#pragma unroll
    for (int t = 0; t < NE; ++t) { yo[t] = eyo[t]; ad[t] = e1[t] + e2[t]; }
    __builtin_amdgcn_fence(__ATOMIC_RELEASE, "wavefront");
    __builtin_amdgcn_wave_barrier();
    if (PF && ch + 4 < nchunk) load_chunk(p + 64);
    if (a.dbg == 2) continue;
    f32x4 accd[NTI];
#pragma unroll
    for (int i = 0; i < NTI; ++i) accd[i] = f32x4{0.f, 0.f, 0.f, 0.f};
#pragma unroll 2
    for (int ks = 0; ks < NTO; ++ks) {
      const float4 a4 = *reinterpret_cast<const float4*>(&Dt[l15 * SD + 16 * ks + 4 * lq]);
      const float aa[4] = {a4.x, a4.y, a4.z, a4.w};
#pragma unroll
      for (int i = 0; i < NTI; ++i) {
        const float4 b4 = *reinterpret_cast<const float4*>(&Wl[(i * 16 + l15) * SD + 16 * ks + 4 * lq]);
        const float bb[4] = {b4.x, b4.y, b4.z, b4.w};
#pragma unroll
        for (int t = 0; t < 4; ++t) accd[i] = __builtin_amdgcn_mfma_f32_16x16x4f32(aa[t], bb[t], accd[i], 0, 0, 0);
      }
    }
#pragma unroll
    for (int t = 0; t < 4; ++t) {
      const int row = 4 * lq + t;
      float bv[NTO];
#pragma unroll
      for (int o = 0; o < NTO; ++o) bv[o] = Dt[row * SD + o * 16 + l15];
#pragma unroll
      for (int i = 0; i < NTI; ++i) {
        const int col = i * 16 + l15;
        const bool cok = col < KI;
        float av = At[row * SA + col];
        if (Y_IS_A) {
          const float raw = av;
          const float z = fmaf(raw, tabA[col], tabA[CI + col]);
          const float m = drop_in ? keep1(seed_in, (uint64_t)(p + row) * KI + col, a.in.drop_rate, a.in.keep_scale) : 1.f;
          float fa, fg;
          if (a.in.act == RN_ACT_ELU) { const float ez = __expf(fminf(z, 0.f)); fa = z > 0.f ? z : ez - 1.f; fg = z > 0.f ? 1.f : ez; }
          else { fa = act_of<-1>(z, a.in.act); fg = actgrad_of<-1>(z, a.in.act); }
          av = cok ? fa * m : 0.f;
          const float xh = (raw - tabO[col]) * tabO[CI + col];
          const float d = accd[i][t];
          float g = cok ? d * fg * m : 0.f;
          s1[i] += g; s2[i] = fmaf(g, xh, s2[i]);
          At[row * SA + col] = cok ? (go.store_plain ? d : g) : 0.f;
        }
#pragma unroll
        for (int o = 0; o < NTO; ++o) accw[i][o] = __builtin_amdgcn_mfma_f32_16x16x4f32(av, bv[o], accw[i][o], 0, 0, 0);
      }
    }
    if (!Y_IS_A) {
#pragma unroll
      for (int i = 0; i < NTI; ++i) {
        const int col = i * 16 + l15;
        const bool cok = col < KI;
#pragma unroll
        for (int r = 0; r < 4; ++r) {
          const int row = 4 * lq + r;
          const float d = accd[i][r] + ad[(i * 4 + r) % NE];
          float outv = d;
          if (go.has_norm) {
            const float xh = (yo[(i * 4 + r) % NE] - tabO[col]) * tabO[CI + col];
            const float z = fmaf(xh, tabO[2 * CI + col], tabO[3 * CI + col]);
            float g = d * actgrad_of<-1>(z, ond.act);
            if (odrop) g *= keep1(oseed, (uint64_t)(p + row) * KI + col, ond.drop_rate, ond.keep_scale);
            if (!cok) g = 0.f;
            s1[i] += g; s2[i] = fmaf(g, xh, s2[i]);
            outv = go.store_plain ? d : g;
          }
          if (!cok) outv = 0.f;
          At[row * SA + col] = outv;
        }
      }
    }
    __builtin_amdgcn_fence(__ATOMIC_RELEASE, "wavefront");
    __builtin_amdgcn_wave_barrier();
#pragma unroll
    for (int j = 0; j < NA; ++j) {
      int row, col;
      if (a_slot(j, row, col))
        *reinterpret_cast<float4*>(go.out + (size_t)p * KI + (size_t)(lane + 64 * j) * 4) = *reinterpret_cast<const float4*>(&At[row * SA + col]);
    }
    __builtin_amdgcn_fence(__ATOMIC_RELEASE, "wavefront");
    __builtin_amdgcn_wave_barrier();
  }
  if (a.dbg == 3) { if (accw[0][0][0] == 123.456f) a.slab[0] = s1[0]; return; }
  __syncthreads();
  float* ex = lds;
  auto put = [&](int slot) {
#pragma unroll
    for (int i = 0; i < NTI; ++i)
#pragma unroll
      for (int o = 0; o < NTO; ++o)
#pragma unroll
        for (int r = 0; r < 4; ++r) ex[((slot * NTI * NTO + i * NTO + o) * 4 + r) * 64 + lane] = accw[i][o][r];
  };
  auto add = [&](int slot) {
#pragma unroll
    for (int i = 0; i < NTI; ++i)
#pragma unroll
      for (int o = 0; o < NTO; ++o)
#pragma unroll
        for (int r = 0; r < 4; ++r) accw[i][o][r] += ex[((slot * NTI * NTO + i * NTO + o) * 4 + r) * 64 + lane];
  };
  if (wave >= 2) put(wave - 2);
  __syncthreads();
  if (wave < 2) add(wave);
  __syncthreads();
  if (wave < 2) put(wave);
  __syncthreads();
  {
    float* slab = a.slab + (size_t)blk * KI * NO;
    for (int e = tid; e < NTI * NTO * 256; e += T) {
      const int ln = e & 63, r = (e >> 6) & 3, tl = e >> 8;
      const int i = tl / NTO, o = tl - i * NTO;
      const int ci = i * 16 + 4 * (ln >> 4) + r, co = o * 16 + (ln & 15);
      if (ci < KI && co < NO) slab[(size_t)ci * NO + co] = ex[((0 * NTI * NTO + tl) * 4 + r) * 64 + ln] + ex[((1 * NTI * NTO + tl) * 4 + r) * 64 + ln];
    }
  }
  if (!go.has_norm) return;
  __syncthreads();
  float* red = lds;
#pragma unroll
  for (int i = 0; i < NTI; ++i) {
    float t1 = s1[i], t2 = s2[i];
    t1 += __shfl_xor(t1, 16, 64); t1 += __shfl_xor(t1, 32, 64);
    t2 += __shfl_xor(t2, 16, 64); t2 += __shfl_xor(t2, 32, 64);
    if (lane < 16) { red[(wave * 2 + 0) * CI + i * 16 + lane] = t1; red[(wave * 2 + 1) * CI + i * 16 + lane] = t2; }
  }
  __syncthreads();
  float* chan = lds + 8 * CI;
  const int prow = sample * a.bps + bis;
  for (int c = tid; c < KI; c += T) {
    float t1 = 0.f, t2 = 0.f;
#pragma unroll
    for (int w = 0; w < 4; ++w) { t1 += red[(w * 2 + 0) * CI + c]; t2 += red[(w * 2 + 1) * CI + c]; }
    chan[c * 2 + 0] = t1; chan[c * 2 + 1] = t2;
    go.planes[(size_t)prow * KI + c] = t1;
    go.planes[go.plane_stride + (size_t)prow * KI + c] = t2;
  }
  __syncthreads();
  if (tid < ond.groups) {
    float t1 = 0.f, t2 = 0.f;
    for (int c = tid * ond.cpg; c < (tid + 1) * ond.cpg; ++c) {
      const float w = ond.gamma[c];
      t1 += w * chan[c * 2 + 0]; t2 += w * chan[c * 2 + 1];
    }
    go.grows.rows[(size_t)prow * go.grows.W + tid] = make_float2(t1, t2);
  }
}

struct DwBwdArgs {
  int dbg;
  NormDev in; DyDev dy; const float* w; float* partial; GoutDev go;
  int n, h, wd, c, stride, oh, ow, pad_t, pad_l;
  int th, tw, tiles_h, tiles_w, sw, nslab;
  int oph, opw;
  int tpb, nblk;
};

__device__ __forceinline__ int floor_div(int a, int b) { return a >= 0 ? a / b : -((-a + b - 1) / b); }

template <int ACT, bool MULTI, int S, int NPA = NP, int NPD = NP, bool PF = false>
__global__ __launch_bounds__(T, 2) void mb_dw_bwd_kernel(const DwBwdArgs a) {
  extern __shared__ __attribute__((aligned(16))) float dsm[];
  __shared__ __attribute__((aligned(16))) float tabA[4 * 128];
  __shared__ __attribute__((aligned(16))) float tabD[3 * 128];
  __shared__ __attribute__((aligned(16))) float wtab[9 * 128];
  __shared__ float gstat[GMAX][2];
  __shared__ float gc[GMAX][2];
  const int tid = threadIdx.x;
  const int bid = rn::xcd_remap(blockIdx.x, gridDim.x);
  const int slab = bid % a.nslab;
  const int tt = bid / a.nslab;
  const int ntile = a.tiles_h * a.tiles_w;
  const int blk = tt % a.nblk, sample = tt / a.nblk;
  const int tile_lo = MULTI ? blk * a.tpb : blk, tile_hi = MULTI ? min(tile_lo + a.tpb, ntile) : tile_lo + 1;
  const int C = a.c, SW = a.sw, SQ = SW >> 2, c0 = slab * SW;
  constexpr int s = S;
  const int tw_shift = 31 - __builtin_clz(a.tw);
  const int aph = a.th + 2, apw = a.tw + 2;
  float* a1p = dsm;
  float* dyp = dsm + (size_t)aph * apw * SW;
  const int g0 = c0 / a.in.cpg, ng = SW / a.in.cpg;
  ChanPre<1> pre_a, pre_d;
  prefetch_chan<1>(a.in.gamma, a.in.beta, c0, SW, tid, pre_a);
  prefetch_chan<1>(a.dy.nd.gamma, nullptr, c0, SW, tid, pre_d);
  const GroupPre gp_a = prefetch_groups(a.in, sample, g0, ng, tid);
  const GroupPre gp_d = prefetch_groups(a.dy.nd, sample, g0, ng, tid);
  const int atotal = aph * apw * SQ;
  const int dtotal = a.oph * a.opw * SQ;
  const __amdgpu_buffer_rsrc_t xs = make_rsrc(a.in.y + (size_t)sample * a.h * a.wd * C + c0, (unsigned)(a.h * a.wd * C - c0) * 4u);
  const __amdgpu_buffer_rsrc_t gs = make_rsrc(a.dy.g + (size_t)sample * a.oh * a.ow * C + c0, (unsigned)(a.oh * a.ow * C - c0) * 4u);
  const __amdgpu_buffer_rsrc_t ys = make_rsrc(a.dy.nd.y + (size_t)sample * a.oh * a.ow * C + c0, (unsigned)(a.oh * a.ow * C - c0) * 4u);
  float4 av[NPA], gv[NPD], yv2[NPD];
  int pka[NPA], pkd[NPD];
#pragma unroll
  for (int j = 0; j < NPA; ++j) pka[j] = patch_pack(tid + j * T, atotal, SQ, apw);
#pragma unroll
  for (int j = 0; j < NPD; ++j) pkd[j] = patch_pack(tid + j * T, dtotal, SQ, a.opw);
  auto load_patches = [&](int tile) {
    const int ih0 = (tile / a.tiles_w) * a.th, iw0 = (tile % a.tiles_w) * a.tw;
    const int ay0 = ih0 - a.pad_t, ax0 = iw0 - a.pad_l;
#pragma unroll
    for (int j = 0; j < NPA; ++j) {
      const PatchElem e = patch_at(pka[j], ay0, ax0, a.h, a.wd);
      av[j] = Vec<4>::load(xs, (e.live && e.inside) ? ((unsigned)e.pix * C + e.q * 4) * 4u : OOB);
    }
    const int oy0 = floor_div(ih0 + a.pad_t - 2 + (s - 1), s), ox0 = floor_div(iw0 + a.pad_l - 2 + (s - 1), s);
#pragma unroll
    for (int j = 0; j < NPD; ++j) {
      const PatchElem e = patch_at(pkd[j], oy0, ox0, a.oh, a.ow);
      const unsigned off = (e.live && e.inside) ? ((unsigned)e.pix * C + e.q * 4) * 4u : OOB;
      gv[j] = Vec<4>::load(gs, off);
      yv2[j] = Vec<4>::load(ys, off);
    }
  };
  load_patches(tile_lo);
  const int lanes = T / SQ, q4 = tid % SQ, pl = tid / SQ;
  const bool active = pl < lanes;
  float4 wv[9];
  if (MULTI) {
    for (int e = tid; e < 9 * SQ; e += T)
      *reinterpret_cast<float4*>(&wtab[(e / SQ) * 128 + (e % SQ) * 4]) = *reinterpret_cast<const float4*>(a.w + (size_t)(e / SQ) * C + c0 + (e % SQ) * 4);
  } else {
#pragma unroll
    for (int t = 0; t < 9; ++t) wv[t] = *reinterpret_cast<const float4*>(a.w + (size_t)t * C + c0 + q4 * 4);
  }
  dy_table(a.dy, sample, a.oh * a.ow, c0, SW, dsm, gstat, gc, tabD, 128, gp_d, pre_d, tid);
  group_stats(a.in, sample, a.h * a.wd, g0, ng, false, dsm, gstat, gp_a, tid);
  scale_shift_table(a.in, c0, SW, g0, gstat, tabA, tabA + 128, pre_a, tid);
  for (int i = tid; i < SW; i += T) {
    const int g = (c0 + i) / a.in.cpg - g0;
    tabA[256 + i] = gstat[g][0]; tabA[384 + i] = gstat[g][1];
  }
  __syncthreads();
  if (a.dbg == 1) { if (av[0].x == 123.456f && gv[0].x == 1.f && yv2[0].x == 1.f) a.go.out[0] = 0.f; return; }
  const bool drop = a.in.drop_rate > 0.f;
  const uint64_t seed = a.in.seed + (a.in.seed_dev ? *a.in.seed_dev : 0ull);
  const uint64_t samp_off = (uint64_t)sample * a.h * a.wd * C;
  float s1[4] = {0.f, 0.f, 0.f, 0.f}, s2[4] = {0.f, 0.f, 0.f, 0.f};
  float4 wacc[9];
#pragma unroll
  for (int t = 0; t < 9; ++t) wacc[t] = make_float4(0.f, 0.f, 0.f, 0.f);
  const float* __restrict__ y1 = a.in.y + (size_t)sample * a.h * a.wd * C + c0 + q4 * 4;
  float* __restrict__ go = a.go.out + (size_t)sample * a.h * a.wd * C + c0 + q4 * 4;
  auto process_tile = [&](int tile) {
    const int ih0 = (tile / a.tiles_w) * a.th, iw0 = (tile % a.tiles_w) * a.tw;
    const int ay0 = ih0 - a.pad_t, ax0 = iw0 - a.pad_l;
    const int oy0 = floor_div(ih0 + a.pad_t - 2 + (s - 1), s), ox0 = floor_div(iw0 + a.pad_l - 2 + (s - 1), s);
#pragma unroll
    for (int j = 0; j < NPA; ++j) {
      const PatchElem e = patch_at(pka[j], ay0, ax0, a.h, a.wd);
      if (e.live) {
        float4 o = norm_act_drop<ACT>(av[j], *reinterpret_cast<const float4*>(&tabA[e.q * 4]), *reinterpret_cast<const float4*>(&tabA[128 + e.q * 4]),
                                      a.in.act, drop, a.in.drop_rate, a.in.keep_scale, seed, samp_off + (uint64_t)e.pix * C + c0 + e.q * 4);
        if (!e.inside) o = make_float4(0.f, 0.f, 0.f, 0.f);
        *reinterpret_cast<float4*>(&a1p[(size_t)(tid + j * T) * 4]) = o;
      }
    }
#pragma unroll
    for (int j = 0; j < NPD; ++j) {
      const PatchElem e = patch_at(pkd[j], oy0, ox0, a.oh, a.ow);
      if (e.live) {
        float4 o = dy_of(gv[j], yv2[j], tabD, 128, e.q * 4, false, 0.f, 1.f, 0ull, 0ull);
        if (!e.inside) o = make_float4(0.f, 0.f, 0.f, 0.f);
        *reinterpret_cast<float4*>(&dyp[(size_t)(tid + j * T) * 4]) = o;
      }
    }
    __syncthreads();
    if (PF && tile + 1 < tile_hi) load_patches(tile + 1);
    if (active) {
      const float4 sc = *reinterpret_cast<const float4*>(&tabA[q4 * 4]), sh = *reinterpret_cast<const float4*>(&tabA[128 + q4 * 4]);
      const float4 mn = *reinterpret_cast<const float4*>(&tabA[256 + q4 * 4]), rs = *reinterpret_cast<const float4*>(&tabA[384 + q4 * 4]);
      for (int p = pl; p < a.th * a.tw; p += lanes) {
        const int ty = p >> tw_shift, tx = p - (ty << tw_shift);
        const int ih = ih0 + ty, iw = iw0 + tx;
        if (ih < a.h && iw < a.wd) {
          const float4 yv = *reinterpret_cast<const float4*>(y1 + (size_t)(ih * a.wd + iw) * C);
          float4 acc = make_float4(0.f, 0.f, 0.f, 0.f);
#pragma unroll
          for (int kh = 0; kh < 3; ++kh) {
            const int ohs = ih + a.pad_t - kh;
            const int oh_ = S == 1 ? ohs : (ohs >> 1);
            const bool rok = ohs >= 0 && oh_ * s == ohs && oh_ < a.oh;
            const int py = min(max(oh_ - oy0, 0), a.oph - 1);
#pragma unroll
            for (int kw = 0; kw < 3; ++kw) {
              const int ows = iw + a.pad_l - kw;
              const int ow_ = S == 1 ? ows : (ows >> 1);
              const float m = (rok && ows >= 0 && ow_ * s == ows && ow_ < a.ow) ? 1.f : 0.f;
              const int px = min(max(ow_ - ox0, 0), a.opw - 1);
              const float4 dv = *reinterpret_cast<const float4*>(&dyp[((size_t)py * a.opw + px) * SW + q4 * 4]);
              const float4 w4 = MULTI ? *reinterpret_cast<const float4*>(&wtab[(kh * 3 + kw) * 128 + q4 * 4]) : wv[kh * 3 + kw];
              acc.x = fmaf(dv.x * m, w4.x, acc.x); acc.y = fmaf(dv.y * m, w4.y, acc.y);
              acc.z = fmaf(dv.z * m, w4.z, acc.z); acc.w = fmaf(dv.w * m, w4.w, acc.w);
            }
          }
          const float yy[4] = {yv.x, yv.y, yv.z, yv.w}, dd[4] = {acc.x, acc.y, acc.z, acc.w};
          const float scv[4] = {sc.x, sc.y, sc.z, sc.w}, shv[4] = {sh.x, sh.y, sh.z, sh.w};
          const float mnv[4] = {mn.x, mn.y, mn.z, mn.w}, rsv[4] = {rs.x, rs.y, rs.z, rs.w};
          float g[4], mk[4] = {1.f, 1.f, 1.f, 1.f};
          if (drop) keep4(seed, samp_off + (uint64_t)(ih * a.wd + iw) * C + c0 + q4 * 4, a.in.drop_rate, a.in.keep_scale, mk);
#pragma unroll
          for (int j = 0; j < 4; ++j) {
            const float z = fmaf(yy[j], scv[j], shv[j]);
            const float xh = (yy[j] - mnv[j]) * rsv[j];
            const float t = dd[j] * actgrad_of<ACT>(z, a.in.act) * mk[j];
            g[j] = t;
            s1[j] += t; s2[j] = fmaf(t, xh, s2[j]);
          }
          *reinterpret_cast<float4*>(go + (size_t)(ih * a.wd + iw) * C) = make_float4(g[0], g[1], g[2], g[3]);
        }
      }
    }
    if (active) {
      const int noy = (a.th + s - 1) / s, nox = (a.tw + s - 1) / s;
      const int oyb = ih0 / s, oxb = iw0 / s;
      for (int p = pl; p < noy * nox; p += lanes) {
        const int ty = p / nox, tx = p - ty * nox;
        const int oh_ = oyb + ty, ow_ = oxb + tx;
        if (oh_ < a.oh && ow_ < a.ow) {
          const float4 dv = *reinterpret_cast<const float4*>(&dyp[((size_t)(oh_ - oy0) * a.opw + (ow_ - ox0)) * SW + q4 * 4]);
#pragma unroll
          for (int kh = 0; kh < 3; ++kh)
#pragma unroll
            for (int kw = 0; kw < 3; ++kw) {
              const float4 xv = *reinterpret_cast<const float4*>(&a1p[((size_t)(ty * s + kh) * apw + tx * s + kw) * SW + q4 * 4]);
              float4& t = wacc[kh * 3 + kw];
              t.x = fmaf(xv.x, dv.x, t.x); t.y = fmaf(xv.y, dv.y, t.y); t.z = fmaf(xv.z, dv.z, t.z); t.w = fmaf(xv.w, dv.w, t.w);
            }
        }
      }
    }
    __syncthreads();
  };
  process_tile(tile_lo);
  if (MULTI) {
#pragma nounroll
    for (int tile = tile_lo + 1; tile < tile_hi; ++tile) {
      if (!PF) load_patches(tile);
      process_tile(tile);
    }
  }
  if (a.dbg == 4) { if (wacc[0].x == 123.456f && s1[0] == 1.f) a.go.out[0] = 0.f; return; }
  constexpr int RW = 44;
  float* red = dsm;
#pragma unroll
  for (int t = 0; t < 9; ++t) {
    red[tid * RW + t * 4 + 0] = wacc[t].x; red[tid * RW + t * 4 + 1] = wacc[t].y;
    red[tid * RW + t * 4 + 2] = wacc[t].z; red[tid * RW + t * 4 + 3] = wacc[t].w;
  }
#pragma unroll
  for (int j = 0; j < 4; ++j) { red[tid * RW + 36 + j] = s1[j]; red[tid * RW + 40 + j] = s2[j]; }
  __syncthreads();
  float* chan = dsm + T * RW;
  const int brow = sample * a.nblk + blk;
  for (int e = tid; e < 11 * SW; e += T) {
    const int k = e / SW, ch = e - k * SW;
    const int qd = ch >> 2, comp = ch & 3;
    float t = 0.f;
    for (int l = 0; l < lanes; ++l) t += red[(l * SQ + qd) * RW + k * 4 + comp];
    if (k < 9) {
      a.partial[((size_t)brow * 9 + k) * C + c0 + ch] = t;
    } else {
      chan[ch * 2 + (k - 9)] = t;
      a.go.planes[(size_t)(k - 9) * a.go.plane_stride + (size_t)brow * C + c0 + ch] = t;
    }
  }
  __syncthreads();
  const int cpg = a.in.cpg;
  if (tid < ng) {
    float t1 = 0.f, t2 = 0.f;
    for (int j = 0; j < cpg; ++j) {
      const float w = a.in.gamma[c0 + tid * cpg + j];
      t1 += w * chan[(tid * cpg + j) * 2 + 0]; t2 += w * chan[(tid * cpg + j) * 2 + 1];
    }
    a.go.grows.rows[(size_t)brow * a.go.grows.W + g0 + tid] = make_float2(t1, t2);
  }
}

}

extern "C" size_t rn_mb_pointwise_rows(int n, int hw, int cin, int cout, int groups, rn_mb_rows* layout) {
  if (n < 1 || hw < 1 || cin < 4 || cout < 4 || groups < 1 || cout % groups) return 0;
  const PwCfg c = pw_cfg(n, hw, cin, cout);
  if (hw % c.bm) return 0;
  const int R = hw / c.bm, W = groups + rn::ceil_div(cout, c.bn);
  if (cout / groups > c.bn) return 0;
  if (layout) { layout->rows_per_sample = R; layout->width = W; layout->bn = c.bn; }
  return (size_t)n * R * W * 8;
}

extern "C" int rn_mb_pointwise_fwd(const float* x, const rn_mb_norm* in, const float* residual, float* materialise, const float* w, float* y,
                                   int n, int hw, int cin, int cout, const rn_mb_rows* stat_out, int stat_groups, rn_stream_t stream) {
  RN_CHECK_ARG((x != nullptr) != (in != nullptr), "mb pointwise fwd: exactly one of x / in");
  RN_CHECK_ARG(w && y && n >= 1 && hw >= 1, "mb pointwise fwd: bad argument");
  RN_UNSUPPORTED(cin % 4 || cout % 4 || cin > KMAX || cout > KMAX, "mb pointwise fwd: cin=%d cout=%d (multiples of 4, <= %d)", cin, cout, KMAX);
  RN_UNSUPPORTED((double)n * hw * cin >= 536870912.0 || (double)n * hw * cout >= 536870912.0, "mb pointwise fwd: tensor >= 2 GiB");
  RN_CHECK_ARG(in || (!residual && !materialise), "mb pointwise fwd: residual / materialise come with `in`");
  PwFwdArgs a = {};
  a.dbg = dbg_word("pwf");
  a.x = x; a.res = residual; a.mat = materialise; a.w = w; a.y = y;
  a.n = n; a.hw = hw; a.cin = cin; a.cout = cout;
  if (in) {
    if (int e = fill_norm(in, &a.in, n, true, "mb pointwise fwd")) return e;
    RN_CHECK_ARG(in->c == cin, "mb pointwise fwd: in->c %d != cin %d", in->c, cin);
  }
  const PwCfg c = pw_cfg(n, hw, cin, cout);
  RN_UNSUPPORTED(hw % c.bm, "mb pointwise fwd: %d pixels per sample, tile height %d", hw, c.bm);
  a.tiles_n = rn::ceil_div(cout, c.bn);
  if (stat_out) {
    RN_CHECK_ARG(stat_out->rows && stat_groups >= 1 && cout % stat_groups == 0, "mb pointwise fwd: bad stat_out");
    rn_mb_rows want = {};
    RN_UNSUPPORTED(!rn_mb_pointwise_rows(n, hw, cin, cout, stat_groups, &want), "mb pointwise fwd: this shape cannot emit rows");
    RN_CHECK_ARG(want.rows_per_sample == stat_out->rows_per_sample && want.width == stat_out->width && want.bn == stat_out->bn,
                 "mb pointwise fwd: stat_out layout differs from rn_mb_pointwise_rows");
    a.ost.rows = (float2*)stat_out->rows; a.ost.R = want.rows_per_sample; a.ost.W = want.width; a.ost.bn = want.bn;
    a.ocpg = cout / stat_groups;
  }
  const long blocks = (long)n * hw / c.bm * a.tiles_n;
  const dim3 grid((unsigned)blocks);
  hipStream_t st = (hipStream_t)stream;
#define RN_PW(BM_, BN_, WM_, WN_, KS_, NST_)                                                                              \
  do {                                                                                                                \
    constexpr int TB = WM_ * WN_ * 64 * KS_;                                                                          \
    if (!in) hipLaunchKernelGGL((mb_pw_fwd_kernel<BM_, BN_, WM_, WN_, false, 0, KS_, NST_>), grid, dim3(TB), 0, st, a);      \
    else if (in->act == RN_ACT_NONE) hipLaunchKernelGGL((mb_pw_fwd_kernel<BM_, BN_, WM_, WN_, true, RN_ACT_NONE, KS_, NST_>), grid, dim3(TB), 0, st, a); \
    else if (in->act == RN_ACT_ELU) hipLaunchKernelGGL((mb_pw_fwd_kernel<BM_, BN_, WM_, WN_, true, RN_ACT_ELU, KS_, NST_>), grid, dim3(TB), 0, st, a);   \
    else hipLaunchKernelGGL((mb_pw_fwd_kernel<BM_, BN_, WM_, WN_, true, -1, KS_, NST_>), grid, dim3(TB), 0, st, a);          \
  } while (0)
  switch (c.id) {
    case 1: RN_PW(128, 32, 4, 1, 1, 1); break;
    case 2: RN_PW(128, 64, 2, 2, 1, 1); break;
    case 3:
      if (c.ks == 8) RN_PW(32, 32, 1, 1, 8, 2);
      else RN_PW(32, 32, 1, 1, 4, 2);
      break;
    default:
      if (c.ks == 4) RN_PW(64, 64, 2, 2, 4, 1);
      else RN_PW(64, 64, 2, 2, 1, 1);
      break;
  }
#undef RN_PW
  RN_LAUNCH_CHECK();
  return RN_OK;
}

extern "C" size_t rn_mb_depthwise_rows(int n, int h, int w, int c, int stride, int groups, rn_mb_rows* layout) {
  if (n < 1 || h < 1 || w < 1 || c < 4 || c % 4 || groups < 1 || c % groups || (stride != 1 && stride != 2)) return 0;
  int oh, ow, pt, pl;
  rn::same_pad(h, 3, stride, &oh, &pt);
  rn::same_pad(w, 3, stride, &ow, &pl);
  DwPlan p;
  if (!dw_plan(n, oh, ow, c, stride, c / groups, &p)) return 0;
  const int R = p.nblk;
  if (layout) { layout->rows_per_sample = R; layout->width = groups; layout->bn = c; }
  return (size_t)n * R * groups * 8;
}

extern "C" int rn_mb_depthwise_fwd(const rn_mb_norm* in, const float* w, float* y, int n, int h, int wd, int stride, const rn_mb_rows* stat_out,
                                   int stat_groups, rn_stream_t stream) {
  RN_CHECK_ARG(in && w && y && n >= 1 && h >= 1 && wd >= 1 && (stride == 1 || stride == 2), "mb depthwise fwd: bad argument");
  DwFwdArgs a = {};
  a.dbg = dbg_word("dwf");
  if (int e = fill_norm(in, &a.in, n, true, "mb depthwise fwd")) return e;
  const int c = in->c;
  RN_UNSUPPORTED((double)n * h * wd * c >= 536870912.0, "mb depthwise fwd: tensor >= 2 GiB");
  a.w = w; a.y = y; a.n = n; a.h = h; a.wd = wd; a.c = c; a.stride = stride;
  rn::same_pad(h, 3, stride, &a.oh, &a.pad_t);
  rn::same_pad(wd, 3, stride, &a.ow, &a.pad_l);
  DwPlan p;
  RN_UNSUPPORTED(stat_out && stat_groups != in->groups, "mb depthwise fwd: the GroupNorms around a depthwise conv share their grouping");
  RN_UNSUPPORTED(!dw_plan(n, a.oh, a.ow, c, stride, a.in.cpg, &p), "mb depthwise fwd: no channel slab for c=%d groups=%d", c, in->groups);
  a.th = p.th; a.tw = p.tw; a.tiles_h = p.tiles_h; a.tiles_w = p.tiles_w; a.sw = p.sw; a.nslab = p.nslab; a.ph = p.ph; a.pw = p.pw;
  a.tpb = p.tpb; a.nblk = p.nblk;
  if (stat_out) {
    rn_mb_rows want = {};
    RN_UNSUPPORTED(!rn_mb_depthwise_rows(n, h, wd, c, stride, stat_groups, &want), "mb depthwise fwd: this shape cannot emit rows");
    RN_CHECK_ARG(stat_out->rows && want.rows_per_sample == stat_out->rows_per_sample && want.width == stat_out->width && want.bn == stat_out->bn,
                 "mb depthwise fwd: stat_out layout differs from rn_mb_depthwise_rows");
    a.ost.rows = (float2*)stat_out->rows; a.ost.R = want.rows_per_sample; a.ost.W = want.width; a.ost.bn = want.bn;
    a.ocpg = c / stat_groups;
  }
  const size_t lds = dw_lds_bytes(p);
  RN_UNSUPPORTED(lds > 64 * 1024, "mb depthwise fwd: patch of %zu bytes", lds);
  const dim3 grid((unsigned)((long)n * p.nblk * p.nslab));
  hipStream_t st = (hipStream_t)stream;
  static const bool pf = !(getenv("RN_MB_DW_NO_PF") && atoi(getenv("RN_MB_DW_NO_PF")));
  if (in->act == RN_ACT_ELU && pf && p.tpb > 1) hipLaunchKernelGGL((mb_dw_fwd_kernel<RN_ACT_ELU, true>), grid, dim3(T), lds, st, a);
  else if (in->act == RN_ACT_ELU) hipLaunchKernelGGL((mb_dw_fwd_kernel<RN_ACT_ELU, false>), grid, dim3(T), lds, st, a);
  else if (in->act == RN_ACT_RELU6) hipLaunchKernelGGL((mb_dw_fwd_kernel<RN_ACT_RELU6, false>), grid, dim3(T), lds, st, a);
  else hipLaunchKernelGGL((mb_dw_fwd_kernel<-1, false>), grid, dim3(T), lds, st, a);
  RN_LAUNCH_CHECK();
  return RN_OK;
}

extern "C" int rn_mb_apply(const rn_mb_norm* in, const float* residual, float* out, int n, int hw, rn_stream_t stream) {
  RN_CHECK_ARG(in && out && n >= 1 && hw >= 1, "mb apply: bad argument");
  ApplyArgs a = {};
  if (int e = fill_norm(in, &a.in, n, false, "mb apply")) return e;
  RN_UNSUPPORTED((double)n * hw * in->c >= 536870912.0, "mb apply: tensor >= 2 GiB");
  a.res = residual; a.out = out; a.n = n; a.hw = hw;
  const long elems = (long)hw * (in->c / 4);
  int chunks = (int)((elems + 4 * T - 1) / (4 * T));
  if (chunks > hw) chunks = hw;
  if (chunks < 1) chunks = 1;
  a.ppb = rn::ceil_div(hw, chunks);
  hipLaunchKernelGGL(mb_apply_kernel, dim3((unsigned)rn::ceil_div(hw, a.ppb), (unsigned)n), dim3(T), 0, (hipStream_t)stream, a);
  RN_LAUNCH_CHECK();
  return RN_OK;
}

namespace {
int fill_dy(const rn_mb_dy* s, DyDev* d, int n, int channels, const char* what) {
  RN_CHECK_ARG(s, "%s: null rn_mb_dy", what);
  if (s->dy) { d->dy = s->dy; return RN_OK; }
  RN_CHECK_ARG(s->norm && s->g && s->grows.rows, "%s: rn_mb_dy needs dy, or norm + g + grows", what);
  if (int e = fill_norm(s->norm, &d->nd, n, false, what)) return e;
  RN_CHECK_ARG(s->norm->c == channels, "%s: rn_mb_dy.norm->c %d != %d", what, s->norm->c, channels);
  RN_CHECK_ARG(!s->g_plain || s->norm->act == RN_ACT_NONE, "%s: g_plain needs a block without activation", what);
  d->nd.st.rows = nullptr;
  d->g = s->g; d->g_plain = s->g_plain ? 1 : 0;
  d->grows.rows = (float2*)s->grows.rows; d->grows.R = s->grows.rows_per_sample; d->grows.W = s->grows.width; d->grows.bn = s->grows.bn;
  RN_CHECK_ARG(d->grows.R >= 1 && d->grows.W >= d->nd.groups && d->grows.bn >= 1, "%s: bad grows layout", what);
  RN_UNSUPPORTED(d->grows.R > RMAX || d->nd.cpg > d->grows.bn, "%s: %d gradient rows per sample (<= %d)", what, d->grows.R, RMAX);
  return RN_OK;
}
int fill_gout(const rn_mb_gout* s, GoutDev* d, int n, int channels, const rn_mb_rows& want, const char* what) {
  RN_CHECK_ARG(s && s->out, "%s: null rn_mb_gout", what);
  d->out = s->out; d->add1 = s->add1; d->add2 = s->add2; d->store_plain = s->store_plain ? 1 : 0;
  if (!s->norm) return RN_OK;
  if (int e = fill_norm(s->norm, &d->nd, n, false, what)) return e;
  RN_CHECK_ARG(s->norm->c == channels, "%s: rn_mb_gout.norm->c %d != %d", what, s->norm->c, channels);
  d->nd.st.rows = nullptr;
  d->has_norm = 1;
  RN_CHECK_ARG(s->grows.rows && s->planes, "%s: rn_mb_gout with a norm needs grows + planes", what);
  RN_CHECK_ARG(s->grows.rows_per_sample == want.rows_per_sample && s->grows.width == want.width && s->grows.bn == want.bn,
               "%s: gout->grows layout differs from the *_bwd_rows query", what);
  d->grows.rows = (float2*)s->grows.rows; d->grows.R = want.rows_per_sample; d->grows.W = want.width; d->grows.bn = want.bn;
  d->planes = s->planes; d->plane_stride = (long)n * want.rows_per_sample * channels;
  return RN_OK;
}
struct PwBwdCfg { int dpb, dks, wpb, wks; };
PwBwdCfg pw_bwd_cfg(int n, int hw, int cin, int cout) {
  static const bool no_ks = getenv("RN_MB_NO_SPLITK") != nullptr;
  static const bool no_t32 = getenv("RN_MB_NO_TILE32") != nullptr;
  const long dblocks = (long)n * hw / 64 * rn::ceil_div(cin, 64);
  const int nkt = rn::ceil_div(cout, BK);
  if (!no_ks && dblocks <= 96 && nkt >= 4) {
    if (no_t32) return {64, 4, 64, 4};
    return nkt >= 16 ? PwBwdCfg{32, 8, 64, 2} : PwBwdCfg{32, 4, 64, 1};
  }
  return {64, 1, 64, 1};
}
void pw_wgrad_plan(int n, int hw, int cin, int cout, int pb, int ks, int* chunk, int* sps) {
  const int tiles = rn::ceil_div(cin, pb) * rn::ceil_div(cout, pb);
  int want = rn::ceil_div(384, tiles * n);
  static const int big_blocks = getenv("RN_MB_WGRAD_BIG_BLOCKS") ? atoi(getenv("RN_MB_WGRAD_BIG_BLOCKS")) : 384;
  if (hw >= 16384 && big_blocks > 0) want = rn::ceil_div(big_blocks, tiles * n);
  if (const char* f = getenv("RN_MB_WGRAD_SPS")) { if (atoi(f) > 0) want = atoi(f); }
  const int unit = 128 * ks;
  const int units = hw % unit == 0 ? hw / unit : 1;
  int best = 1;
  for (int d = 1; d <= units && d <= want; ++d)
    if (units % d == 0) best = d;
  *sps = best; *chunk = hw / best;
}
struct PwBigCfg { int nti, nto, ppb, bps; };
bool pw_big_cfg(int n, int hw, int cin, int cout, PwBigCfg* c) {
  static const bool on = !(getenv("RN_MB_PW_BIG") && atoi(getenv("RN_MB_PW_BIG")) == 0);
  static const int min_hw = getenv("RN_MB_PW_BIG_MIN_HW") ? atoi(getenv("RN_MB_PW_BIG_MIN_HW")) : 16384;
  if (!on || hw < min_hw || hw % 64 || cin % 4 || cout % 4) return false;
  const int nti = rn::ceil_div(cin, 16), nto = rn::ceil_div(cout, 16);
  const bool built = (nti == 2 && nto == 2) || (nti == 1 && nto == 6) || (nti == 2 && nto == 9) || (nti == 2 && nto == 1) ||
                     (nti == 6 && nto == 2) || (nti == 9 && nto == 2);
  if (!built) return false;
  if (nti == 9 && hw < 65536 && !getenv("RN_MB_PW_BIG_MIN_HW")) return false;
  static const int target = getenv("RN_MB_PW_BIG_BLOCKS") ? atoi(getenv("RN_MB_PW_BIG_BLOCKS")) : 512;
  int ppb = 64;
  while ((long)n * hw / ppb > target && hw % (ppb * 2) == 0) ppb *= 2;
  while (hw / ppb > RMAX && hw % (ppb * 2) == 0) ppb *= 2;
  if (hw / ppb > RMAX) return false;
  c->nti = nti; c->nto = nto; c->ppb = ppb; c->bps = hw / ppb;
  return true;
}
struct DwBwdPlan { int th, tw, tiles_h, tiles_w, sw, nslab, oph, opw, tpb, nblk; };
bool dw_bwd_plan(int n, int h, int w, int c, int stride, int cpg, DwBwdPlan* p) {
  p->sw = dw_slab(c, cpg);
  if (!p->sw) return false;
  p->nslab = c / p->sw;
  static const int th_big = getenv("RN_MB_DWB_TH") ? atoi(getenv("RN_MB_DWB_TH")) : 8;
  static const int tw_big = getenv("RN_MB_DWB_TW") ? atoi(getenv("RN_MB_DWB_TW")) : 8;
  const bool big = (long)h * w >= 16384;
  int th = big ? th_big : 8, tw = big ? tw_big : 8;
  auto blocks = [&]() { return (long)n * rn::ceil_div(h, th) * rn::ceil_div(w, tw) * p->nslab; };
  auto too_big = [&]() { return (long)(th + 2) * (tw + 2) * (p->sw / 4) > NP * T || (long)(th / stride + 2) * (tw / stride + 2) * (p->sw / 4) > NP * T; };
  while ((blocks() < 384 && th * tw > 16) || (too_big() && th * tw > 16)) {
    if (th >= tw) th /= 2; else tw /= 2;
  }
  p->th = th; p->tw = tw;
  p->tiles_h = rn::ceil_div(h, th); p->tiles_w = rn::ceil_div(w, tw);
  p->oph = th / stride + 2; p->opw = tw / stride + 2;
  if ((long)(th + 2) * (tw + 2) * (p->sw / 4) > NP * T || (long)p->oph * p->opw * (p->sw / 4) > NP * T) return false;
  p->tpb = dw_tiles_per_block(blocks(), p->tiles_h * p->tiles_w);
  p->nblk = rn::ceil_div(p->tiles_h * p->tiles_w, p->tpb);
  return true;
}
size_t dw_bwd_lds_bytes(const DwBwdPlan& p) {
  size_t patches = ((size_t)(p.th + 2) * (p.tw + 2) + (size_t)p.oph * p.opw) * p.sw * 4;
  size_t scratch = (size_t)(T + GMAX) * 16;
  size_t red = (size_t)(T * 44 + 2 * p.sw) * 4;
  size_t m = patches > scratch ? patches : scratch;
  return m > red ? m : red;
}
}

extern "C" size_t rn_mb_pointwise_bwd_rows(int n, int hw, int cin, int cout, int groups, rn_mb_rows* layout) {
  if (n < 1 || hw < 1 || cin < 4 || cout < 4 || groups < 1 || cin % groups || hw % 64) return 0;
  PwBigCfg big;
  if (pw_big_cfg(n, hw, cin, cout, &big)) {
    if (layout) { layout->rows_per_sample = big.bps; layout->width = groups + 1; layout->bn = big.nti * 16; }
    return (size_t)n * big.bps * (groups + 1) * 8;
  }
  const int pb = pw_bwd_cfg(n, hw, cin, cout).dpb;
  const int R = hw / pb, W = groups + rn::ceil_div(cin, pb);
  if (cin / groups > pb) return 0;
  if (layout) { layout->rows_per_sample = R; layout->width = W; layout->bn = pb; }
  return (size_t)n * R * W * 8;
}
extern "C" size_t rn_mb_pointwise_bwd_workspace(int n, int hw, int cin, int cout) {
  if (n < 1 || hw < 64 || hw % 64 || cin < 4 || cout < 4) return 0;
  PwBigCfg big;
  if (pw_big_cfg(n, hw, cin, cout, &big)) return (size_t)n * big.bps * cin * cout * sizeof(float);
  int chunk, sps;
  const PwBwdCfg c = pw_bwd_cfg(n, hw, cin, cout);
  pw_wgrad_plan(n, hw, cin, cout, c.wpb, c.wks, &chunk, &sps);
  return (size_t)n * sps * cin * cout * sizeof(float);
}

extern "C" int rn_mb_pointwise_bwd(const float* x, const rn_mb_norm* in, const rn_mb_dy* dy, const float* w, float* dw, const rn_mb_gout* gout,
                                   int n, int hw, int cin, int cout, void* workspace, size_t workspace_bytes, rn_stream_t stream,
                                   rn_reduce_list* defer) {
  rn::DeferScope defer_scope_(defer);
  RN_CHECK_ARG((x != nullptr) != (in != nullptr), "mb pointwise bwd: exactly one of x / in");
  RN_CHECK_ARG(w && dw && dy && gout && workspace && n >= 1 && hw >= 1, "mb pointwise bwd: bad argument");
  RN_UNSUPPORTED(cin % 4 || cout % 4 || cin > KMAX || cout > KMAX, "mb pointwise bwd: cin=%d cout=%d (multiples of 4, <= %d)", cin, cout, KMAX);
  RN_UNSUPPORTED(hw % 64, "mb pointwise bwd: %d pixels per sample, tile height 64", hw);
  RN_UNSUPPORTED((double)n * hw * cin >= 536870912.0 || (double)n * hw * cout >= 536870912.0, "mb pointwise bwd: tensor >= 2 GiB");
  PwBwdArgs a = {};
  a.dbg = dbg_word("pwb");
  a.x = x; a.w = w; a.n = n; a.hw = hw; a.cin = cin; a.cout = cout;
  if (in) {
    if (int e = fill_norm(in, &a.in, n, false, "mb pointwise bwd")) return e;
    RN_CHECK_ARG(in->c == cin, "mb pointwise bwd: in->c %d != cin %d", in->c, cin);
    a.in.st.rows = nullptr;
    a.has_in = 1;
  }
  if (int e = fill_dy(dy, &a.dy, n, cout, "mb pointwise bwd")) return e;
  rn_mb_rows want = {};
  if (gout->norm) RN_UNSUPPORTED(!rn_mb_pointwise_bwd_rows(n, hw, cin, cout, gout->norm->groups, &want), "mb pointwise bwd: this shape cannot emit gradient rows");
  if (int e = fill_gout(gout, &a.go, n, cin, want, "mb pointwise bwd")) return e;
  PwBigCfg big;
  if (pw_big_cfg(n, hw, cin, cout, &big)) {
    PwBigArgs b = {};
    b.dbg = dbg_word("pwB");
    b.x = a.x; b.in = a.in; b.has_in = a.has_in; b.dy = a.dy; b.w = w; b.go = a.go;
    b.n = n; b.hw = hw; b.cin = cin; b.cout = cout; b.ppb = big.ppb; b.bps = big.bps;
    const int nsplit = n * big.bps;
    const size_t need = (size_t)nsplit * cin * cout * sizeof(float);
    if (workspace_bytes < need) { rn::set_error("mb pointwise bwd: workspace %zu < %zu bytes", workspace_bytes, need); return RN_EWORKSPACE; }
    b.slab = (float*)workspace;
    const bool y_is_a = a.has_in && a.go.has_norm && a.go.nd.y == a.in.y && !a.go.add1 && !a.go.add2;
    const dim3 grid((unsigned)nsplit);
    hipStream_t st = (hipStream_t)stream;
#define RN_PWBIG(NTI_, NTO_)                                                                                                    \
  do {                                                                                                                          \
    constexpr size_t lds = (size_t)pw_big_lds_floats(NTI_, NTO_) * 4;                                                           \
    static const bool attr_ = (hipFuncSetAttribute((const void*)mb_pw_bwd_big_kernel<NTI_, NTO_, true>, hipFuncAttributeMaxDynamicSharedMemorySize, (int)lds) == hipSuccess) & \
                              (hipFuncSetAttribute((const void*)mb_pw_bwd_big_kernel<NTI_, NTO_, false>, hipFuncAttributeMaxDynamicSharedMemorySize, (int)lds) == hipSuccess); \
    RN_UNSUPPORTED(!attr_, "mb pointwise bwd: %zu bytes of LDS per block refused", lds);                                                                                                                \
    if (y_is_a) hipLaunchKernelGGL((mb_pw_bwd_big_kernel<NTI_, NTO_, true>), grid, dim3(T), lds, st, b);                        \
    else hipLaunchKernelGGL((mb_pw_bwd_big_kernel<NTI_, NTO_, false>), grid, dim3(T), lds, st, b);                              \
  } while (0)
    if (big.nti == 2 && big.nto == 2) RN_PWBIG(2, 2);
    else if (big.nti == 1 && big.nto == 6) RN_PWBIG(1, 6);
    else if (big.nti == 2 && big.nto == 9) RN_PWBIG(2, 9);
    else if (big.nti == 2 && big.nto == 1) RN_PWBIG(2, 1);
    else if (big.nti == 6 && big.nto == 2) RN_PWBIG(6, 2);
    else RN_PWBIG(9, 2);
#undef RN_PWBIG
    RN_LAUNCH_CHECK();
    return rn::launch_reduce_rows((const float*)workspace, dw, (int64_t)cin * cout, nsplit, 0, st);
  }
  const PwBwdCfg cfg = pw_bwd_cfg(n, hw, cin, cout);
  a.d_tiles_n = rn::ceil_div(cin, cfg.dpb);
  a.dblocks = n * hw / cfg.dpb * a.d_tiles_n;
  a.w_tiles_m = rn::ceil_div(cin, cfg.wpb); a.w_tiles_n = rn::ceil_div(cout, cfg.wpb);
  pw_wgrad_plan(n, hw, cin, cout, cfg.wpb, cfg.wks, &a.chunk, &a.sps);
  const int nsplit = n * a.sps;
  const size_t need = (size_t)nsplit * cin * cout * sizeof(float);
  if (workspace_bytes < need) { rn::set_error("mb pointwise bwd: workspace %zu < %zu bytes", workspace_bytes, need); return RN_EWORKSPACE; }
  a.slab = nsplit == 1 ? dw : (float*)workspace;
  static const int wfirst_env = getenv("RN_MB_WGRAD_FIRST") ? atoi(getenv("RN_MB_WGRAD_FIRST")) : 1;
  a.wfirst = (wfirst_env && a.dblocks > 1024) ? 1 : 0;
  const dim3 grid((unsigned)(a.dblocks + nsplit * a.w_tiles_m * a.w_tiles_n));
  hipStream_t st = (hipStream_t)stream;
  const int act_in = in ? in->act : -2, act_out = gout->norm ? gout->norm->act : RN_ACT_NONE;
#define RN_PWB(DPB_, DKS_, WPB_, WKS_)                                                                                               \
  do {                                                                                                                               \
    constexpr int TB = (DPB_ / 32) * (DPB_ / 32) * 64 * DKS_;                                                                        \
    if (act_in == -2 && act_out == RN_ACT_NONE) hipLaunchKernelGGL((mb_pw_bwd_kernel<-2, RN_ACT_NONE, DPB_, DKS_, WPB_, WKS_>), grid, dim3(TB), 0, st, a); \
    else if (act_in == -2) hipLaunchKernelGGL((mb_pw_bwd_kernel<-2, -1, DPB_, DKS_, WPB_, WKS_>), grid, dim3(TB), 0, st, a);          \
    else if (act_in == RN_ACT_ELU && act_out == RN_ACT_ELU) hipLaunchKernelGGL((mb_pw_bwd_kernel<RN_ACT_ELU, RN_ACT_ELU, DPB_, DKS_, WPB_, WKS_>), grid, dim3(TB), 0, st, a); \
    else hipLaunchKernelGGL((mb_pw_bwd_kernel<-1, -1, DPB_, DKS_, WPB_, WKS_>), grid, dim3(TB), 0, st, a);                            \
  } while (0)
  if (cfg.dpb == 32 && cfg.dks == 8) RN_PWB(32, 8, 64, 2);
  else if (cfg.dpb == 32) RN_PWB(32, 4, 64, 1);
  else if (cfg.dks == 4) RN_PWB(64, 4, 64, 4);
  else RN_PWB(64, 1, 64, 1);
#undef RN_PWB
  RN_LAUNCH_CHECK();
  if (nsplit == 1) return RN_OK;
  return rn::launch_reduce_rows((const float*)workspace, dw, (int64_t)cin * cout, nsplit, 0, st);
}

extern "C" size_t rn_mb_depthwise_bwd_rows(int n, int h, int w, int c, int stride, int groups, rn_mb_rows* layout) {
  if (n < 1 || h < 1 || w < 1 || c < 4 || c % 4 || groups < 1 || c % groups || (stride != 1 && stride != 2)) return 0;
  DwBwdPlan p;
  if (!dw_bwd_plan(n, h, w, c, stride, c / groups, &p)) return 0;
  const int R = p.nblk;
  if (layout) { layout->rows_per_sample = R; layout->width = groups; layout->bn = c; }
  return (size_t)n * R * groups * 8;
}
extern "C" size_t rn_mb_depthwise_bwd_workspace(int n, int h, int w, int c, int stride) {
  if (n < 1 || h < 1 || w < 1 || c < 4 || c % 4 || (stride != 1 && stride != 2)) return 0;
  return (size_t)n * rn::ceil_div(h, 4) * rn::ceil_div(w, 4) * 9 * c * sizeof(float);
}

extern "C" int rn_mb_depthwise_bwd(const rn_mb_norm* in, const rn_mb_dy* dy, const float* w, float* dw, const rn_mb_gout* gout, int n, int h,
                                   int wd, int stride, void* workspace, size_t workspace_bytes, rn_stream_t stream, rn_reduce_list* defer) {
  rn::DeferScope defer_scope_(defer);
  RN_CHECK_ARG(in && dy && w && dw && gout && gout->norm && workspace && n >= 1 && h >= 1 && wd >= 1 && (stride == 1 || stride == 2),
               "mb depthwise bwd: bad argument");
  RN_CHECK_ARG(!dy->dy && !gout->store_plain && !gout->add1 && !gout->add2, "mb depthwise bwd: dy comes as (g, norm, grows); gout stores g");
  DwBwdArgs a = {};
  a.dbg = dbg_word("dwb");
  if (int e = fill_norm(in, &a.in, n, false, "mb depthwise bwd")) return e;
  a.in.st.rows = nullptr;
  const int c = in->c;
  RN_UNSUPPORTED((double)n * h * wd * c >= 536870912.0, "mb depthwise bwd: tensor >= 2 GiB");
  if (int e = fill_dy(dy, &a.dy, n, c, "mb depthwise bwd")) return e;
  RN_CHECK_ARG(!a.dy.g_plain && dy->norm->groups == in->groups, "mb depthwise bwd: the GroupNorms around a depthwise conv share their grouping");
  a.w = w; a.n = n; a.h = h; a.wd = wd; a.c = c; a.stride = stride;
  rn::same_pad(h, 3, stride, &a.oh, &a.pad_t);
  rn::same_pad(wd, 3, stride, &a.ow, &a.pad_l);
  DwBwdPlan p;
  RN_UNSUPPORTED(!dw_bwd_plan(n, h, wd, c, stride, a.in.cpg, &p), "mb depthwise bwd: no channel slab for c=%d groups=%d", c, in->groups);
  a.th = p.th; a.tw = p.tw; a.tiles_h = p.tiles_h; a.tiles_w = p.tiles_w; a.sw = p.sw; a.nslab = p.nslab; a.oph = p.oph; a.opw = p.opw;
  a.tpb = p.tpb; a.nblk = p.nblk;
  rn_mb_rows want = {};
  RN_UNSUPPORTED(!rn_mb_depthwise_bwd_rows(n, h, wd, c, stride, in->groups, &want), "mb depthwise bwd: this shape cannot emit gradient rows");
  if (int e = fill_gout(gout, &a.go, n, c, want, "mb depthwise bwd")) return e;
  RN_CHECK_ARG(gout->norm->y == in->y, "mb depthwise bwd: gout->norm is the block of `in`");
  const int nrows = n * p.nblk;
  const size_t need = (size_t)nrows * 9 * c * sizeof(float);
  if (workspace_bytes < need) { rn::set_error("mb depthwise bwd: workspace %zu < %zu bytes", workspace_bytes, need); return RN_EWORKSPACE; }
  a.partial = (float*)workspace;
  const size_t lds = dw_bwd_lds_bytes(p);
  RN_UNSUPPORTED(lds > 64 * 1024, "mb depthwise bwd: patches of %zu bytes", lds);
  const dim3 grid((unsigned)((long)nrows * p.nslab));
  hipStream_t st = (hipStream_t)stream;
  RN_CHECK_ARG((p.tw & (p.tw - 1)) == 0, "mb depthwise bwd: tile width %d is not a power of two", p.tw);
#define RN_DWB(ACT_, MULTI_)                                                                                           \
  do {                                                                                                                 \
    if (stride == 1) hipLaunchKernelGGL((mb_dw_bwd_kernel<ACT_, MULTI_, 1>), grid, dim3(T), lds, st, a);               \
    else hipLaunchKernelGGL((mb_dw_bwd_kernel<ACT_, MULTI_, 2>), grid, dim3(T), lds, st, a);                           \
  } while (0)
  static const bool pf_on = !(getenv("RN_MB_DWB_PF") && atoi(getenv("RN_MB_DWB_PF")) == 0);
  const int npa = rn::ceil_div((p.th + 2) * (p.tw + 2) * (p.sw / 4), T), npd = rn::ceil_div(p.oph * p.opw * (p.sw / 4), T);
  if (in->act == RN_ACT_ELU && p.tpb > 1 && pf_on && stride == 1 && npa <= 4 && npd <= 4)
    hipLaunchKernelGGL((mb_dw_bwd_kernel<RN_ACT_ELU, true, 1, 4, 4, true>), grid, dim3(T), lds, st, a);
  else if (in->act == RN_ACT_ELU && p.tpb > 1 && pf_on && stride == 1 && npa <= 5 && npd <= 5)
    hipLaunchKernelGGL((mb_dw_bwd_kernel<RN_ACT_ELU, true, 1, 5, 5, true>), grid, dim3(T), lds, st, a);
  else if (in->act == RN_ACT_ELU && p.tpb > 1 && pf_on && stride == 2 && npa <= 4 && npd <= 2)
    hipLaunchKernelGGL((mb_dw_bwd_kernel<RN_ACT_ELU, true, 2, 4, 2, true>), grid, dim3(T), lds, st, a);
  else if (in->act == RN_ACT_ELU && p.tpb > 1 && pf_on && stride == 2 && npa <= 5 && npd <= 2)
    hipLaunchKernelGGL((mb_dw_bwd_kernel<RN_ACT_ELU, true, 2, 5, 2, true>), grid, dim3(T), lds, st, a);
  else if (in->act == RN_ACT_ELU && p.tpb == 1) RN_DWB(RN_ACT_ELU, false);
  else if (in->act == RN_ACT_ELU) RN_DWB(RN_ACT_ELU, true);
  else if (in->act == RN_ACT_RELU6) RN_DWB(RN_ACT_RELU6, true);
  else RN_DWB(-1, true);
#undef RN_DWB
  RN_LAUNCH_CHECK();
  return rn::launch_reduce_rows((const float*)workspace, dw, (int64_t)9 * c, nrows, 0, st);
}

extern "C" int rn_mb_rows_max(void) { return RMAX; }

extern "C" size_t rn_mb_compact_rows_layout(int n, const rn_mb_rows* in, rn_mb_rows* out) {
  if (!in || !out || n < 1 || in->rows_per_sample < 1 || in->width < 1 || in->width > T) return 0;
  const int F = rn::ceil_div(in->rows_per_sample, 8);
  out->rows_per_sample = rn::ceil_div(in->rows_per_sample, F); out->width = in->width; out->bn = in->bn;
  return (size_t)n * out->rows_per_sample * out->width * 8;
}

extern "C" int rn_mb_compact_rows(const rn_mb_rows* in, const rn_mb_rows* out, int n, rn_stream_t stream) {
  RN_CHECK_ARG(in && out && in->rows && out->rows && n >= 1, "mb compact rows: bad argument");
  rn_mb_rows want = {};
  RN_CHECK_ARG(rn_mb_compact_rows_layout(n, in, &want) && want.rows_per_sample == out->rows_per_sample && want.width == out->width && want.bn == out->bn,
               "mb compact rows: `out` layout differs from rn_mb_compact_rows_layout");
  CompactArgs a = {(const float2*)in->rows, (float2*)out->rows, in->rows_per_sample, in->width, rn::ceil_div(in->rows_per_sample, 8), want.rows_per_sample};
  hipLaunchKernelGGL(mb_compact_rows_kernel, dim3((unsigned)a.Rout, (unsigned)n), dim3(T), 0, (hipStream_t)stream, a);
  RN_LAUNCH_CHECK();
  return RN_OK;
}
```

retinanet-tensorflow_amd/ops_mb.py:

```python
import ctypes as C
import os

import torch

import _rn
import ops


class Norm(object):

    def __init__(self, gamma, beta, groups, eps, act, rate, seed):
        self.gamma, self.beta = gamma, beta
        self.groups_arg, self.eps, self.act, self.rate, self.seed = int(groups), float(eps), act, float(rate), int(seed)


class Block(object):

    def __init__(self, w1, n1, wd, n2, w3, n3, stride, residual):
        self.w1, self.n1, self.wd, self.n2, self.w3, self.n3 = w1, n1, wd, n2, w3, n3
        self.stride, self.residual = int(stride), bool(residual)


def _rows(query, *args):
    lay = _rn.MbRows()
    nbytes = query(*args, C.byref(lay))
    return lay, int(nbytes)


COMPACT_ABOVE = int(os.environ.get('RN_MB_COMPACT_ABOVE', '256'))
RESIDENT = os.environ.get('RN_MB_RESIDENT', '0') == '1'
RESIDENT_MAX_HW = int(os.environ.get('RN_MB_RESIDENT_MAX_HW', '1024'))
RESIDENT_MAX_IN_BYTES = int(os.environ.get('RN_MB_RESIDENT_MAX_IN_BYTES', str(3328 * 1024)))


def _compact(rows, lay, n, dev):
    L = _rn.lib()
    if lay.rows_per_sample <= min(L.rn_mb_rows_max(), COMPACT_ABOVE):
        return rows, lay
    src = _rn.MbRows(rows.data_ptr(), lay.rows_per_sample, lay.width, lay.bn)
    out = _rn.MbRows()
    nbytes = L.rn_mb_compact_rows_layout(n, C.byref(src), C.byref(out))
    assert nbytes
    small = torch.empty(nbytes // 4, dtype=torch.float32, device=dev)
    out.rows = small.data_ptr()
    _rn.check(L.rn_mb_compact_rows(C.byref(src), C.byref(out), n, _rn.stream()), "rn_mb_compact_rows")
    return small, out


class _Stage(object):
    __slots__ = ("y", "rows", "lay", "mean", "rstd", "norm", "c", "groups", "hw")


def _mb_norm(st, training, seed_dev, with_rows):
    nm = st.norm
    m = _rn.MbNorm()
    m.y = st.y.data_ptr()
    if with_rows:
        m.stat = _rn.MbRows(st.rows.data_ptr(), st.lay.rows_per_sample, st.lay.width, st.lay.bn)
    m.mean, m.rstd = st.mean.data_ptr(), st.rstd.data_ptr()
    m.gamma, m.beta = _rn.f32(nm.gamma), _rn.f32(nm.beta)
    m.c, m.groups, m.act, m.eps = st.c, st.groups, _rn.ACT[nm.act], nm.eps
    rate = nm.rate if training else 0.0
    m.drop_rate, m.drop_seed = rate, nm.seed
    m.drop_seed_dev = seed_dev.data_ptr() if (seed_dev is not None and rate > 0.0) else None
    return m


def _count_resident(nphases):
    """(test hook: called with the number of phases whenever a forward pass takes the resident section)"""


def _resident_start(n, h, w, c, blocks_cfg, shapes, tail_cout):
    if not RESIDENT:
        return None
    L = _rn.lib()
    ok = []
    for (stride, _res, n1, n2, n3), (wide, cout) in zip(blocks_cfg, shapes):
        oh, _ = _rn.same_pad(h, 3, stride)
        ow, _ = _rn.same_pad(w, 3, stride)
        g1, g3 = ops.gn_groups(wide, n1.groups_arg), ops.gn_groups(cout, n3.groups_arg)
        acts = (n1.act in ('elu',), n2.act in ('elu',), n3.act is None)
        ok.append(h * w <= RESIDENT_MAX_HW and h * w * c * 4 <= RESIDENT_MAX_IN_BYTES and acts[2] and
                  bool(L.rn_mb_resident_rows(_rn.MB_PHASE_POINTWISE, n, h, w, c, wide, 1, g1, None)))
        ok.append(oh * ow <= RESIDENT_MAX_HW and h * w * wide * 4 <= RESIDENT_MAX_IN_BYTES and acts[0] and
                  bool(L.rn_mb_resident_rows(_rn.MB_PHASE_DEPTHWISE, n, h, w, wide, wide, stride, g1, None)))
        ok.append(oh * ow <= RESIDENT_MAX_HW and oh * ow * wide * 4 <= RESIDENT_MAX_IN_BYTES and acts[1] and
                  bool(L.rn_mb_resident_rows(_rn.MB_PHASE_POINTWISE, n, oh, ow, wide, cout, 1, g3, None)))
        h, w, c = oh, ow, cout
    ok.append(h * w <= RESIDENT_MAX_HW and h * w * c * 4 <= RESIDENT_MAX_IN_BYTES and h * w % 32 == 0 and c % 4 == 0 and tail_cout % 4 == 0)
    ok[0] = False
    start = len(ok)
    while start > 0 and ok[start - 1]:
        start -= 1
    return start if start < len(ok) else None


def chain_supported(shape, blocks):
    L = _rn.lib()
    n, h, w, c = (int(v) for v in shape)
    for b in blocks:
        wide, cout = b.w1.shape[3], b.w3.shape[3]
        if b.w1.shape[2] != c or wide % 4 or cout % 4 or c % 4:
            return False
        g1, g3 = ops.gn_groups(wide, b.n1.groups_arg), ops.gn_groups(cout, b.n3.groups_arg)
        oh, _ = _rn.same_pad(h, 3, b.stride)
        ow, _ = _rn.same_pad(w, 3, b.stride)
        if not L.rn_mb_pointwise_rows(n, h * w, c, wide, g1, None) or not L.rn_mb_depthwise_rows(n, h, w, wide, b.stride, g1, None):
            return False
        if not L.rn_mb_pointwise_rows(n, oh * ow, wide, cout, g3, None):
            return False
        if not L.rn_mb_pointwise_bwd_rows(n, oh * ow, wide, cout, g1, None) or not L.rn_mb_depthwise_bwd_rows(n, h, w, wide, b.stride, g1, None):
            return False
        if not L.rn_mb_pointwise_bwd_rows(n, h * w, c, wide, ops.gn_groups(c, 32), None):
            return False
        h, w, c = oh, ow, cout
    return True


class _MbChain(torch.autograd.Function):
    @staticmethod
    def forward(ctx, cfg, x, *params):
        blocks_cfg, tail_cfg, tap_after, training, seed_dev = cfg
        L = _rn.lib()
        dev = x.device
        x = x.contiguous()
        n, h, w, c = x.shape
        nb = len(blocks_cfg)
        st_ = _rn.stream()

        shapes = [(params[9 * i].shape[3], params[9 * i + 6].shape[3]) for i in range(nb)]
        res_from = _resident_start(n, h, w, c, blocks_cfg, shapes, params[9 * nb].shape[3]) if x.is_cuda else None
        phases, keep = [], []

        def resident(k):
            return res_from is not None and k >= res_from

        def phase(kind, nm, res_t, mat_t, w_t, y_t, hh, ww, cin, cout, stride, s_out, groups):
            ph = _rn.MbPhase()
            ph.kind, ph.in_ = kind, C.pointer(nm)
            ph.residual = _rn.f32(res_t) if res_t is not None else None
            ph.materialise = _rn.f32(mat_t) if mat_t is not None else None
            ph.w, ph.y = _rn.f32(w_t), _rn.f32(y_t)
            ph.h, ph.wd, ph.cin, ph.cout, ph.stride = hh, ww, cin, cout, stride
            if s_out is not None:
                ph.stat_out = _rn.MbRows(s_out.rows.data_ptr(), s_out.lay.rows_per_sample, s_out.lay.width, s_out.lay.bn)
                ph.stat_groups = groups
            keep.append(nm)
            phases.append(ph)

        def new_stage(y, query_args, query, groups, norm, res_kind=None, res_args=None):
            s = _Stage()
            s.y, s.c, s.groups, s.norm, s.hw = y, y.shape[3], groups, norm, y.shape[1] * y.shape[2]
            if res_kind is not None:
                s.lay, nbytes = _rows(L.rn_mb_resident_rows, res_kind, *res_args)
            else:
                s.lay, nbytes = _rows(query, *query_args)
            assert nbytes, "mb_chain: unsupported shape (chain_supported() says so)"
            s.rows = torch.empty(nbytes // 4, dtype=torch.float32, device=dev)
            s.mean = torch.empty((y.shape[0], groups), dtype=torch.float32, device=dev)
            s.rstd = torch.empty((y.shape[0], groups), dtype=torch.float32, device=dev)
            return s

        def rows_arg(s):
            return C.byref(_rn.MbRows(s.rows.data_ptr(), s.lay.rows_per_sample, s.lay.width, s.lay.bn))

        saved = []
        taps = []
        pend, pend_res = None, None
        x_in = x
        pi = 0
        for i, bc in enumerate(blocks_cfg):
            stride, residual, n1, n2, n3 = bc
            w1, g1_, b1_, wd, g2_, b2_, w3, g3_, b3_ = params[pi:pi + 9]
            pi += 9
            n1.gamma, n1.beta, n2.gamma, n2.beta, n3.gamma, n3.beta = g1_, b1_, g2_, b2_, g3_, b3_
            wide, cout = w1.shape[3], w3.shape[3]
            gr1, gr3 = ops.gn_groups(wide, n1.groups_arg), ops.gn_groups(cout, n3.groups_arg)
            oh, _ = _rn.same_pad(h, 3, stride)
            ow, _ = _rn.same_pad(w, 3, stride)
            y1 = torch.empty((n, h, w, wide), dtype=torch.float32, device=dev)
            r0, r1, r2 = resident(3 * i), resident(3 * i + 1), resident(3 * i + 2)
            s1 = new_stage(y1, (n, h * w, c, wide, gr1), L.rn_mb_pointwise_rows, gr1, n1,
                           _rn.MB_PHASE_POINTWISE if r0 else None, (n, h, w, c, wide, 1, gr1))
            if r0:
                x_in = torch.empty((n, h, w, c), dtype=torch.float32, device=dev)
                phase(_rn.MB_PHASE_POINTWISE, _mb_norm(pend, training, seed_dev, True), pend_res, x_in, w1, y1, h, w, c, wide, 1, s1, gr1)
                if (i - 1) in tap_after:
                    taps.append(x_in)
            elif pend is None:
                _rn.check(L.rn_mb_pointwise_fwd(_rn.f32(x_in), None, None, None, _rn.f32(w1), _rn.f32(y1), n, h * w, c, wide, rows_arg(s1), gr1, st_),
                          "rn_mb_pointwise_fwd")
            else:
                x_in = torch.empty((n, h, w, c), dtype=torch.float32, device=dev)
                nm = _mb_norm(pend, training, seed_dev, True)
                _rn.check(L.rn_mb_pointwise_fwd(None, C.byref(nm), _rn.f32(pend_res) if pend_res is not None else None, _rn.f32(x_in),
                                                _rn.f32(w1), _rn.f32(y1), n, h * w, c, wide, rows_arg(s1), gr1, st_), "rn_mb_pointwise_fwd")
                if (i - 1) in tap_after:
                    taps.append(x_in)
            if not r0:
                s1.rows, s1.lay = _compact(s1.rows, s1.lay, n, dev)
            y2 = torch.empty((n, oh, ow, wide), dtype=torch.float32, device=dev)
            s2 = new_stage(y2, (n, h, w, wide, stride, gr1), L.rn_mb_depthwise_rows, gr1, n2,
                           _rn.MB_PHASE_DEPTHWISE if r1 else None, (n, h, w, wide, wide, stride, gr1))
            nm = _mb_norm(s1, training, seed_dev, True)
            if r1:
                phase(_rn.MB_PHASE_DEPTHWISE, nm, None, None, wd, y2, h, w, wide, wide, stride, s2, gr1)
            else:
                _rn.check(L.rn_mb_depthwise_fwd(C.byref(nm), _rn.f32(wd), _rn.f32(y2), n, h, w, stride, rows_arg(s2), gr1, st_), "rn_mb_depthwise_fwd")
                s2.rows, s2.lay = _compact(s2.rows, s2.lay, n, dev)
            y3 = torch.empty((n, oh, ow, cout), dtype=torch.float32, device=dev)
            s3 = new_stage(y3, (n, oh * ow, wide, cout, gr3), L.rn_mb_pointwise_rows, gr3, n3,
                           _rn.MB_PHASE_POINTWISE if r2 else None, (n, oh, ow, wide, cout, 1, gr3))
            nm = _mb_norm(s2, training, seed_dev, True)
            if r2:
                phase(_rn.MB_PHASE_POINTWISE, nm, None, None, w3, y3, oh, ow, wide, cout, 1, s3, gr3)
            else:
                _rn.check(L.rn_mb_pointwise_fwd(None, C.byref(nm), None, None, _rn.f32(w3), _rn.f32(y3), n, oh * ow, wide, cout, rows_arg(s3), gr3, st_),
                          "rn_mb_pointwise_fwd")
                s3.rows, s3.lay = _compact(s3.rows, s3.lay, n, dev)
            saved.append((x_in, s1, s2, s3))
            pend, pend_res = s3, (x_in if residual else None)
            h, w, c = oh, ow, cout
        tail_w = params[pi]
        tail_groups = tail_cfg
        ct = tail_w.shape[3]
        x_last = torch.empty((n, h, w, c), dtype=torch.float32, device=dev)
        y_t = torch.empty((n, h, w, ct), dtype=torch.float32, device=dev)
        nm = _mb_norm(pend, training, seed_dev, True)
        if resident(3 * nb):
            phase(_rn.MB_PHASE_POINTWISE, nm, pend_res, x_last, tail_w, y_t, h, w, c, ct, 1, None, 0)
        else:
            assert not phases, "the resident section runs to the end of the chain"
            _rn.check(L.rn_mb_pointwise_fwd(None, C.byref(nm), _rn.f32(pend_res) if pend_res is not None else None, _rn.f32(x_last), _rn.f32(tail_w),
                                            _rn.f32(y_t), n, h * w, c, ct, None, 0, st_), "rn_mb_pointwise_fwd")
        if phases:
            _count_resident(len(phases))
            arr = (_rn.MbPhase * len(phases))(*phases)
            _rn.check(L.rn_mb_resident_fwd(arr, len(phases), n, _rn.resident_sync(dev).data_ptr(), st_), "rn_mb_resident_fwd")
        if (nb - 1) in tap_after:
            taps.append(x_last)
        ctx.cfg = cfg
        ctx.saved = saved
        ctx.x_last = x_last
        ctx.params = params
        ctx.shape_in = tuple(x.shape)
        ctx.set_materialize_grads(False)
        return tuple(taps) + (y_t,)

    @staticmethod
    def backward(ctx, *grads):
        blocks_cfg, tail_cfg, tap_after, training, seed_dev = ctx.cfg
        L = _rn.lib()
        params = ctx.params
        saved = ctx.saved
        nb = len(blocks_cfg)
        dev = ctx.x_last.device
        st_ = _rn.stream()
        taps_sorted = sorted(tap_after)
        tap_grad = {t: grads[k] for k, t in enumerate(taps_sorted)}
        dy_t = grads[-1]
        pgrads = [None] * len(params)
        n = ctx.shape_in[0]

        def grows_for(query, args, c):
            lay, nbytes = _rows(query, *args)
            assert nbytes
            rows = torch.empty(nbytes // 4, dtype=torch.float32, device=dev)
            planes = torch.empty((2, n * lay.rows_per_sample, c), dtype=torch.float32, device=dev)
            if ops._deferring:
                ops._deferred_keep.append(planes)
            return lay, rows, planes

        def norm_param_grads(planes, nm, slot_g, slot_b):
            c, nrows = planes.shape[2], planes.shape[1]
            db_buf, db = ops._grad_slot(nm.beta)
            dg_buf, dg = ops._grad_slot(nm.gamma)
            _rn.check(L.rn_reduce_rows(_rn.f32(planes[0]), _rn.f32(db_buf), c, nrows, 0, st_, ops._defer_arg()), "rn_reduce_rows")
            _rn.check(L.rn_reduce_rows(_rn.f32(planes[1]), _rn.f32(dg_buf), c, nrows, 0, st_, ops._defer_arg()), "rn_reduce_rows")
            pgrads[slot_g], pgrads[slot_b] = dg, db

        def pw_bwd(x_plain, in_stage, dy, w, gout, hw, cin, cout, const_w=False):
            if const_w:
                dw_buf, dw = torch.empty_like(w), None
                if ops._deferring:
                    ops._deferred_keep.append(dw_buf)
            else:
                dw_buf, dw = ops._grad_slot(w)
            need = L.rn_mb_pointwise_bwd_workspace(n, hw, cin, cout)
            ws = ops._grad_workspace(need, dev)
            nm_in = _mb_norm(in_stage, training, seed_dev, False) if in_stage is not None else None
            _rn.check(L.rn_mb_pointwise_bwd(_rn.f32(x_plain) if x_plain is not None else None, C.byref(nm_in) if nm_in is not None else None,
                                            C.byref(dy), _rn.f32(w), _rn.f32(dw_buf), C.byref(gout), n, hw, cin, cout, ws.data_ptr(), ws.numel(),
                                            st_, ops._defer_arg()), "rn_mb_pointwise_bwd")
            return dw

        x_last = ctx.x_last
        _, hl, wl, cl = x_last.shape
        tail_w = params[9 * nb]
        ct = tail_w.shape[3]
        if dy_t is None:
            dy_t = torch.zeros((n, hl, wl, ct), dtype=torch.float32, device=dev)
        dy_t = dy_t.contiguous()
        s3_last = saved[-1][3]
        lay3, rows3, planes3 = grows_for(L.rn_mb_pointwise_bwd_rows, (n, hl * wl, cl, ct, s3_last.groups), cl)
        D = torch.empty((n, hl, wl, cl), dtype=torch.float32, device=dev)
        nm3 = _mb_norm(s3_last, training, seed_dev, False)
        tg = tap_grad.get(nb - 1)
        tg = tg.contiguous() if tg is not None else None
        gout = _rn.MbGout(D.data_ptr(), None, _rn.f32(tg) if tg is not None else None, C.pointer(nm3), 1,
                          _rn.MbRows(rows3.data_ptr(), lay3.rows_per_sample, lay3.width, lay3.bn), planes3.data_ptr())
        dyd = _rn.MbDy(dy_t.data_ptr(), None, None, 0, _rn.MbRows())
        pgrads[9 * nb] = pw_bwd(x_last, None, dyd, tail_w, gout, hl * wl, cl, ct, const_w=bool(tail_cfg))
        rows3, lay3 = _compact(rows3, lay3, n, dev)
        keep = [tg]

        dx0 = None
        flushed = False
        for i in range(nb - 1, -1, -1):
            stride, residual, n1, n2, n3 = blocks_cfg[i]
            x_in, s1, s2, s3 = saved[i]
            if not flushed and saved[i][0].shape[1] * saved[i][0].shape[2] >= 16384:
                ops.flush_deferred_midway(dev)
                flushed = True
            w1, g1_, b1_, wd, g2_, b2_, w3, g3_, b3_ = params[9 * i:9 * i + 9]
            _, h, w, c = x_in.shape
            wide, cout = w1.shape[3], w3.shape[3]
            _, oh, ow, _ = s2.y.shape
            norm_param_grads(planes3, n3, 9 * i + 7, 9 * i + 8)
            nm3 = _mb_norm(s3, training, seed_dev, False)
            nm2 = _mb_norm(s2, training, seed_dev, False)
            dy3 = _rn.MbDy(None, C.pointer(nm3), D.data_ptr(), 1, _rn.MbRows(rows3.data_ptr(), lay3.rows_per_sample, lay3.width, lay3.bn))
            lay2, rows2, planes2 = grows_for(L.rn_mb_pointwise_bwd_rows, (n, oh * ow, wide, cout, s2.groups), wide)
            g2 = torch.empty_like(s2.y)
            gout = _rn.MbGout(g2.data_ptr(), None, None, C.pointer(nm2), 0,
                              _rn.MbRows(rows2.data_ptr(), lay2.rows_per_sample, lay2.width, lay2.bn), planes2.data_ptr())
            pgrads[9 * i + 6] = pw_bwd(None, s2, dy3, w3, gout, oh * ow, wide, cout)
            rows2, lay2 = _compact(rows2, lay2, n, dev)
            norm_param_grads(planes2, n2, 9 * i + 4, 9 * i + 5)
            nm1 = _mb_norm(s1, training, seed_dev, False)
            dy2 = _rn.MbDy(None, C.pointer(nm2), g2.data_ptr(), 0, _rn.MbRows(rows2.data_ptr(), lay2.rows_per_sample, lay2.width, lay2.bn))
            lay1, rows1, planes1 = grows_for(L.rn_mb_depthwise_bwd_rows, (n, h, w, wide, stride, s1.groups), wide)
            g1 = torch.empty_like(s1.y)
            gout = _rn.MbGout(g1.data_ptr(), None, None, C.pointer(nm1), 0,
                              _rn.MbRows(rows1.data_ptr(), lay1.rows_per_sample, lay1.width, lay1.bn), planes1.data_ptr())
            dwd_buf, dwd = ops._grad_slot(wd)
            need = L.rn_mb_depthwise_bwd_workspace(n, h, w, wide, stride)
            ws = ops._grad_workspace(need, dev)
            _rn.check(L.rn_mb_depthwise_bwd(C.byref(nm1), C.byref(dy2), _rn.f32(wd), _rn.f32(dwd_buf), C.byref(gout), n, h, w, stride,
                                            ws.data_ptr(), ws.numel(), st_, ops._defer_arg()), "rn_mb_depthwise_bwd")
            pgrads[9 * i + 3] = dwd
            rows1, lay1 = _compact(rows1, lay1, n, dev)
            norm_param_grads(planes1, n1, 9 * i + 1, 9 * i + 2)
            dy1 = _rn.MbDy(None, C.pointer(nm1), g1.data_ptr(), 0, _rn.MbRows(rows1.data_ptr(), lay1.rows_per_sample, lay1.width, lay1.bn))
            Dn = torch.empty((n, h, w, c), dtype=torch.float32, device=dev)
            add1 = D.data_ptr() if residual else None
            if i > 0:
                s3p = saved[i - 1][3]
                lay3n, rows3n, planes3n = grows_for(L.rn_mb_pointwise_bwd_rows, (n, h * w, c, wide, s3p.groups), c)
                nm3p = _mb_norm(s3p, training, seed_dev, False)
                tg = tap_grad.get(i - 1)
                tg = tg.contiguous() if tg is not None else None
                keep.append(tg)
                gout = _rn.MbGout(Dn.data_ptr(), add1, _rn.f32(tg) if tg is not None else None, C.pointer(nm3p), 1,
                                  _rn.MbRows(rows3n.data_ptr(), lay3n.rows_per_sample, lay3n.width, lay3n.bn), planes3n.data_ptr())
            else:
                gout = _rn.MbGout(Dn.data_ptr(), add1, None, None, 1, _rn.MbRows(), None)
            pgrads[9 * i] = pw_bwd(x_in, None, dy1, w1, gout, h * w, c, wide)
            if i > 0:
                rows3n, lay3n = _compact(rows3n, lay3n, n, dev)
                lay3, rows3, planes3 = lay3n, rows3n, planes3n
            else:
                dx0 = Dn
            D_prev, D = D, Dn
            del D_prev
        return (None, dx0) + tuple(pgrads)


def mb_chain(x, blocks, tail_w, tap_after=(), training=True, seed_dev=None, tail_const=False):
    cfg_blocks = tuple((b.stride, b.residual, b.n1, b.n2, b.n3) for b in blocks)
    flat = []
    for b in blocks:
        flat += [b.w1, b.n1.gamma, b.n1.beta, b.wd, b.n2.gamma, b.n2.beta, b.w3, b.n3.gamma, b.n3.beta]
    flat.append(tail_w)
    cfg = (cfg_blocks, bool(tail_const), frozenset(tap_after), bool(training), seed_dev)
    out = _MbChain.apply(cfg, x, *flat)
    return list(out[:-1]), out[-1]
```

Baseline: 476.6.

## Save depthwise input activations and signed act-grad factors in forward for backward reuse

For large-resolution MobileNet blocks with ELU in training, the depthwise forward kernel now writes out the normalised, activated input and a signed activation-derivative factor that encodes the dropout mask. The depthwise backward kernel reads these instead of recomputing normalisation, ELU, its gradient and the dropout hash, and it prefetches the per-tile interior pixels one tile ahead. Small side tweaks cache gamma and the weight column in shared memory for the group reductions. The cost is two extra full-size activation buffers per saved block, plus more forward write traffic and register pressure in the new kernel variants.

```diff
diff --git a/include/rn_hip.h b/include/rn_hip.h
--- a/include/rn_hip.h
+++ b/include/rn_hip.h
@@ -26,7 +26,7 @@
 
 typedef struct rn_reduce_list rn_reduce_list;
 
-#define RN_API_VERSION 408
+#define RN_API_VERSION 409
 int rn_version(void);
 const char* rn_last_error(void);
 
@@ -327,6 +327,7 @@
   int32_t c, groups, act;
   float eps, drop_rate;
   uint64_t drop_seed; const uint64_t* drop_seed_dev;
+  float* saved_act; float* saved_fac;
 } rn_mb_norm;
 
 int rn_mb_rows_max(void);
@@ -339,6 +340,7 @@
 size_t rn_mb_depthwise_rows(int n, int h, int w, int c, int stride, int groups, rn_mb_rows* layout);
 int rn_mb_depthwise_fwd(const rn_mb_norm* in, const float* w, float* y, int n, int h, int wd, int stride, const rn_mb_rows* stat_out,
                         int stat_groups, rn_stream_t stream);
+int rn_mb_depthwise_saved_bytes(int n, int h, int w, int c, int stride, int groups, int training, size_t* bytes);
 int rn_mb_apply(const rn_mb_norm* in, const float* residual, float* out, int n, int hw, rn_stream_t stream);
 
 enum { RN_MB_PHASE_POINTWISE = 0, RN_MB_PHASE_DEPTHWISE = 1 };
diff --git a/retinanet-tensorflow_amd/_rn.py b/retinanet-tensorflow_amd/_rn.py
--- a/retinanet-tensorflow_amd/_rn.py
+++ b/retinanet-tensorflow_amd/_rn.py
@@ -12,7 +12,7 @@
 OPT = {"momentum": 0, "rmsprop": 1, "adam": 2}
 OPT_BLOCK = 1024
 LOSS_STATS_HEADER = 8
-API_VERSION = 408
+API_VERSION = 409
 
 
 class RnError(RuntimeError):
@@ -108,7 +108,8 @@
 class MbNorm(C.Structure):
     _fields_ = [("y", C.c_void_p), ("stat", MbRows), ("mean", C.c_void_p), ("rstd", C.c_void_p), ("gamma", C.c_void_p),
                 ("beta", C.c_void_p), ("c", C.c_int32), ("groups", C.c_int32), ("act", C.c_int32), ("eps", C.c_float),
-                ("drop_rate", C.c_float), ("drop_seed", C.c_uint64), ("drop_seed_dev", C.c_void_p)]
+                ("drop_rate", C.c_float), ("drop_seed", C.c_uint64), ("drop_seed_dev", C.c_void_p),
+                ("saved_act", C.c_void_p), ("saved_fac", C.c_void_p)]
 
 
 class MbPhase(C.Structure):
@@ -167,7 +168,7 @@
     "rn_iou", "rn_anchor_assign", "rn_anchor_assign_levels", "rn_anchor_assign_levels_pair", "rn_decode_boxes", "rn_detect_workspace", "rn_detect",
     "rn_boxes_decode", "rn_nms_classwise_workspace", "rn_nms_classwise",
     "rn_optimizer_workspace", "rn_grad_norm_l2reg", "rn_optimizer_step", "rn_counter_add", "rn_add_segs",
-    "rn_mb_rows_max", "rn_mb_compact_rows_layout", "rn_mb_compact_rows", "rn_mb_pointwise_rows", "rn_mb_pointwise_fwd", "rn_mb_depthwise_rows", "rn_mb_depthwise_fwd", "rn_mb_apply",
+    "rn_mb_rows_max", "rn_mb_compact_rows_layout", "rn_mb_compact_rows", "rn_mb_pointwise_rows", "rn_mb_pointwise_fwd", "rn_mb_depthwise_rows", "rn_mb_depthwise_fwd", "rn_mb_depthwise_saved_bytes", "rn_mb_apply",
     "rn_mb_resident_sync_bytes", "rn_mb_resident_rows", "rn_mb_resident_fwd", "rn_set_product_mode", "rn_get_product_mode",
     "rn_set_x3_bfrag", "rn_get_x3_bfrag", "rn_x3_bfrag_ok", "rn_x3_bfrag_bytes", "rn_x3_pack_bfrag", "rn_gemm_batched_bfrag", "rn_conv3x3_winograd_gn_u_bytes", "rn_conv3x3_winograd_gn_weights",
     "rn_conv2d_f16_stats_tiles", "rn_group_norm_fwd_f16_tiles",
@@ -341,6 +342,7 @@
         L.rn_mb_pointwise_fwd.argtypes = [C.c_void_p] * 6 + [C.c_int] * 4 + [C.c_void_p, C.c_int, C.c_void_p]
         L.rn_mb_depthwise_rows.argtypes = [C.c_int] * 6 + [C.c_void_p]
         L.rn_mb_depthwise_fwd.argtypes = [C.c_void_p] * 3 + [C.c_int] * 4 + [C.c_void_p, C.c_int, C.c_void_p]
+        L.rn_mb_depthwise_saved_bytes.argtypes = [C.c_int] * 7 + [C.POINTER(C.c_size_t)]
         L.rn_mb_apply.argtypes = [C.c_void_p] * 3 + [C.c_int, C.c_int, C.c_void_p]
         L.rn_mb_pointwise_bwd_rows.argtypes = [C.c_int] * 5 + [C.c_void_p]
         L.rn_mb_pointwise_bwd_workspace.argtypes = [C.c_int] * 4
diff --git a/retinanet-tensorflow_amd/csrc/mb_common.h b/retinanet-tensorflow_amd/csrc/mb_common.h
--- a/retinanet-tensorflow_amd/csrc/mb_common.h
+++ b/retinanet-tensorflow_amd/csrc/mb_common.h
@@ -166,6 +166,8 @@
   const int lane = tid & 63, wave = (tid >> 6) % (WM * WN), wm = wave / WN, wn = wave % WN, l31 = lane & 31;
   float* red = smem;
   float* chan = smem + WM * BN * 2;
+  float* wcol = chan + BN * 2;
+  const float wpre = (wgt && tid < BN && n0 + tid < C) ? wgt[n0 + tid] : 1.f;
 #pragma unroll
   for (int tn = 0; tn < TN; ++tn) {
     float a = s1[tn], b = s2[tn];
@@ -183,6 +185,7 @@
 #pragma unroll
     for (int w = 0; w < WM; ++w) { t1 += red[(w * BN + tid) * 2 + 0]; t2 += red[(w * BN + tid) * 2 + 1]; }
     chan[tid * 2 + 0] = t1; chan[tid * 2 + 1] = t2;
+    if (wgt) wcol[tid] = wpre;
     if (plane1 && n0 + tid < C) { plane1[n0 + tid] = t1; plane2[n0 + tid] = t2; }
   }
   __syncthreads();
@@ -193,7 +196,7 @@
     const int c_lo = max(g * cpg, n0), c_hi = min((g + 1) * cpg, cend);
     float t1 = 0.f, t2 = 0.f;
     for (int c = c_lo; c < c_hi; ++c) {
-      const float w = wgt ? wgt[c] : 1.f;
+      const float w = wgt ? wcol[c - n0] : 1.f;
       t1 += w * chan[(c - n0) * 2 + 0]; t2 += w * chan[(c - n0) * 2 + 1];
     }
     row[g + tile_n] = make_float2(t1, t2);
diff --git a/retinanet-tensorflow_amd/csrc/mbconv.hip b/retinanet-tensorflow_amd/csrc/mbconv.hip
--- a/retinanet-tensorflow_amd/csrc/mbconv.hip
+++ b/retinanet-tensorflow_amd/csrc/mbconv.hip
@@ -129,9 +129,23 @@
   }
 }
 
-
-template <int ACT, bool PF>
-__global__ __launch_bounds__(T) void mb_dw_fwd_kernel(const DwFwdArgs a) {
+template <int ACT>
+__device__ __forceinline__ float4 actgrad_signed(float4 v, float4 sc, float4 sh, int act_rt, bool drop, float rate, uint64_t seed, uint64_t eidx) {
+  float o[4] = {fmaf(v.x, sc.x, sh.x), fmaf(v.y, sc.y, sh.y), fmaf(v.z, sc.z, sh.z), fmaf(v.w, sc.w, sh.w)};
+#pragma unroll
+  for (int j = 0; j < 4; ++j) o[j] = fabsf(actgrad_of<ACT>(o[j], act_rt));
+  if (drop) {
+    float m[4];
+    keep4(seed, eidx, rate, 1.f, m);
+#pragma unroll
+    for (int j = 0; j < 4; ++j) o[j] = m[j] == 0.f ? -o[j] : o[j];
+  }
+  return make_float4(o[0], o[1], o[2], o[3]);
+}
+
+
+template <int ACT, bool PF, bool SAVE = false>
+__global__ __launch_bounds__(T) void mb_dw_fwd_kernel(const DwFwdArgs a, float* __restrict__ save_act, float* __restrict__ save_fac) {
   extern __shared__ __attribute__((aligned(16))) float dsm[];
   __shared__ __attribute__((aligned(16))) float tab[2 * 128];
   __shared__ float gstat[GMAX][2];
@@ -181,10 +195,18 @@
     for (int j = 0; j < NP; ++j) {
       const PatchElem e = patch_at(pk[j], ih0, iw0, a.h, a.wd);
       if (e.live) {
-        float4 o = norm_act_drop<ACT>(pv[j], *reinterpret_cast<const float4*>(&tab[e.q * 4]), *reinterpret_cast<const float4*>(&tab[128 + e.q * 4]),
-                                      a.in.act, drop, a.in.drop_rate, a.in.keep_scale, seed, samp_off + (uint64_t)e.pix * C + c0 + e.q * 4);
+        const float4 sc4 = *reinterpret_cast<const float4*>(&tab[e.q * 4]), sh4 = *reinterpret_cast<const float4*>(&tab[128 + e.q * 4]);
+        const uint64_t eidx = samp_off + (uint64_t)e.pix * C + c0 + e.q * 4;
+        float4 o = norm_act_drop<ACT>(pv[j], sc4, sh4, a.in.act, drop, a.in.drop_rate, a.in.keep_scale, seed, eidx);
         if (!e.inside) o = make_float4(0.f, 0.f, 0.f, 0.f);
         *reinterpret_cast<float4*>(&dsm[(size_t)(tid + j * T) * 4]) = o;
+        if (SAVE) {
+          const int oy = ((pk[j] >> 8) & 255) - a.pad_t, ox = ((pk[j] >> 16) & 255) - a.pad_l;
+          if (e.inside && (unsigned)oy < (unsigned)(a.th * a.stride) && (unsigned)ox < (unsigned)(a.tw * a.stride)) {
+            *reinterpret_cast<float4*>(save_act + eidx) = o;
+            *reinterpret_cast<float4*>(save_fac + eidx) = actgrad_signed<ACT>(pv[j], sc4, sh4, a.in.act, drop, a.in.drop_rate, seed, eidx);
+          }
+        }
       }
     }
     __syncthreads();
@@ -983,7 +1005,7 @@
   if (tid < ond.groups) {
     float t1 = 0.f, t2 = 0.f;
     for (int c = tid * ond.cpg; c < (tid + 1) * ond.cpg; ++c) {
-      const float w = ond.gamma[c];
+      const float w = tabO[2 * CI + c];
       t1 += w * chan[c * 2 + 0]; t2 += w * chan[c * 2 + 1];
     }
     go.grows.rows[(size_t)prow * go.grows.W + tid] = make_float2(t1, t2);
@@ -997,16 +1019,18 @@
   int th, tw, tiles_h, tiles_w, sw, nslab;
   int oph, opw;
   int tpb, nblk;
+  const float* save_act; const float* save_fac;
 };
 
 __device__ __forceinline__ int floor_div(int a, int b) { return a >= 0 ? a / b : -((-a + b - 1) / b); }
 
-template <int ACT, bool MULTI, int S, int NPA = NP, int NPD = NP, bool PF = false>
+template <int ACT, bool MULTI, int S, int NPA = NP, int NPD = NP, bool PF = false, bool SV = false, int NPI = 1>
 __global__ __launch_bounds__(T, 2) void mb_dw_bwd_kernel(const DwBwdArgs a) {
   extern __shared__ __attribute__((aligned(16))) float dsm[];
   __shared__ __attribute__((aligned(16))) float tabA[4 * 128];
   __shared__ __attribute__((aligned(16))) float tabD[3 * 128];
   __shared__ __attribute__((aligned(16))) float wtab[9 * 128];
+  __shared__ float gam[128];
   __shared__ float gstat[GMAX][2];
   __shared__ float gc[GMAX][2];
   const int tid = threadIdx.x;
@@ -1030,7 +1054,7 @@
   const GroupPre gp_d = prefetch_groups(a.dy.nd, sample, g0, ng, tid);
   const int atotal = aph * apw * SQ;
   const int dtotal = a.oph * a.opw * SQ;
-  const __amdgpu_buffer_rsrc_t xs = make_rsrc(a.in.y + (size_t)sample * a.h * a.wd * C + c0, (unsigned)(a.h * a.wd * C - c0) * 4u);
+  const __amdgpu_buffer_rsrc_t xs = make_rsrc((SV ? a.save_act : a.in.y) + (size_t)sample * a.h * a.wd * C + c0, (unsigned)(a.h * a.wd * C - c0) * 4u);
   const __amdgpu_buffer_rsrc_t gs = make_rsrc(a.dy.g + (size_t)sample * a.oh * a.ow * C + c0, (unsigned)(a.oh * a.ow * C - c0) * 4u);
   const __amdgpu_buffer_rsrc_t ys = make_rsrc(a.dy.nd.y + (size_t)sample * a.oh * a.ow * C + c0, (unsigned)(a.oh * a.ow * C - c0) * 4u);
   float4 av[NPA], gv[NPD], yv2[NPD];
@@ -1059,6 +1083,22 @@
   load_patches(tile_lo);
   const int lanes = T / SQ, q4 = tid % SQ, pl = tid / SQ;
   const bool active = pl < lanes;
+  const __amdgpu_buffer_rsrc_t yis = make_rsrc(a.in.y + (size_t)sample * a.h * a.wd * C + c0, (unsigned)(a.h * a.wd * C - c0) * 4u);
+  const __amdgpu_buffer_rsrc_t fis = make_rsrc((SV ? a.save_fac : a.in.y) + (size_t)sample * a.h * a.wd * C + c0, (unsigned)(a.h * a.wd * C - c0) * 4u);
+  float4 yi[NPI], fi[NPI];
+  auto load_interior = [&](int tile) {
+    const int ih0 = (tile / a.tiles_w) * a.th, iw0 = (tile % a.tiles_w) * a.tw;
+#pragma unroll
+    for (int k = 0; k < NPI; ++k) {
+      const int p = pl + k * lanes;
+      const int ty = p >> tw_shift, tx = p - (ty << tw_shift);
+      const int ih = ih0 + ty, iw = iw0 + tx;
+      const unsigned off = (active && p < a.th * a.tw && ih < a.h && iw < a.wd) ? ((unsigned)(ih * a.wd + iw) * C + q4 * 4) * 4u : OOB;
+      yi[k] = Vec<4>::load(yis, off);
+      if (SV) fi[k] = Vec<4>::load(fis, off);
+    }
+  };
+  if (SV) load_interior(tile_lo);
   float4 wv[9];
   if (MULTI) {
     for (int e = tid; e < 9 * SQ; e += T)
@@ -1073,6 +1113,7 @@
   for (int i = tid; i < SW; i += T) {
     const int g = (c0 + i) / a.in.cpg - g0;
     tabA[256 + i] = gstat[g][0]; tabA[384 + i] = gstat[g][1];
+    gam[i] = pre_a.g[0];
   }
   __syncthreads();
   if (a.dbg == 1) { if (av[0].x == 123.456f && gv[0].x == 1.f && yv2[0].x == 1.f) a.go.out[0] = 0.f; return; }
@@ -1093,8 +1134,9 @@
     for (int j = 0; j < NPA; ++j) {
       const PatchElem e = patch_at(pka[j], ay0, ax0, a.h, a.wd);
       if (e.live) {
-        float4 o = norm_act_drop<ACT>(av[j], *reinterpret_cast<const float4*>(&tabA[e.q * 4]), *reinterpret_cast<const float4*>(&tabA[128 + e.q * 4]),
-                                      a.in.act, drop, a.in.drop_rate, a.in.keep_scale, seed, samp_off + (uint64_t)e.pix * C + c0 + e.q * 4);
+        float4 o = av[j];
+        if (!SV) o = norm_act_drop<ACT>(av[j], *reinterpret_cast<const float4*>(&tabA[e.q * 4]), *reinterpret_cast<const float4*>(&tabA[128 + e.q * 4]),
+                                        a.in.act, drop, a.in.drop_rate, a.in.keep_scale, seed, samp_off + (uint64_t)e.pix * C + c0 + e.q * 4);
         if (!e.inside) o = make_float4(0.f, 0.f, 0.f, 0.f);
         *reinterpret_cast<float4*>(&a1p[(size_t)(tid + j * T) * 4]) = o;
       }
@@ -1113,11 +1155,11 @@
     if (active) {
       const float4 sc = *reinterpret_cast<const float4*>(&tabA[q4 * 4]), sh = *reinterpret_cast<const float4*>(&tabA[128 + q4 * 4]);
       const float4 mn = *reinterpret_cast<const float4*>(&tabA[256 + q4 * 4]), rs = *reinterpret_cast<const float4*>(&tabA[384 + q4 * 4]);
-      for (int p = pl; p < a.th * a.tw; p += lanes) {
+      auto pixel = [&](int p, const float4* ypre, const float4* fpre) {
         const int ty = p >> tw_shift, tx = p - (ty << tw_shift);
         const int ih = ih0 + ty, iw = iw0 + tx;
         if (ih < a.h && iw < a.wd) {
-          const float4 yv = *reinterpret_cast<const float4*>(y1 + (size_t)(ih * a.wd + iw) * C);
+          const float4 yv = SV ? *ypre : *reinterpret_cast<const float4*>(y1 + (size_t)(ih * a.wd + iw) * C);
           float4 acc = make_float4(0.f, 0.f, 0.f, 0.f);
 #pragma unroll
           for (int kh = 0; kh < 3; ++kh) {
@@ -1140,20 +1182,35 @@
           const float yy[4] = {yv.x, yv.y, yv.z, yv.w}, dd[4] = {acc.x, acc.y, acc.z, acc.w};
           const float scv[4] = {sc.x, sc.y, sc.z, sc.w}, shv[4] = {sh.x, sh.y, sh.z, sh.w};
           const float mnv[4] = {mn.x, mn.y, mn.z, mn.w}, rsv[4] = {rs.x, rs.y, rs.z, rs.w};
-          float g[4], mk[4] = {1.f, 1.f, 1.f, 1.f};
-          if (drop) keep4(seed, samp_off + (uint64_t)(ih * a.wd + iw) * C + c0 + q4 * 4, a.in.drop_rate, a.in.keep_scale, mk);
+          float g[4], mk[4] = {1.f, 1.f, 1.f, 1.f}, ag[4];
+          if (SV) {
+            const float ff[4] = {fpre->x, fpre->y, fpre->z, fpre->w};
+#pragma unroll
+            for (int j = 0; j < 4; ++j) { ag[j] = fabsf(ff[j]); mk[j] = (__float_as_uint(ff[j]) >> 31) ? 0.f : a.in.keep_scale; }
+          } else {
+            if (drop) keep4(seed, samp_off + (uint64_t)(ih * a.wd + iw) * C + c0 + q4 * 4, a.in.drop_rate, a.in.keep_scale, mk);
+#pragma unroll
+            for (int j = 0; j < 4; ++j) ag[j] = actgrad_of<ACT>(fmaf(yy[j], scv[j], shv[j]), a.in.act);
+          }
 #pragma unroll
           for (int j = 0; j < 4; ++j) {
-            const float z = fmaf(yy[j], scv[j], shv[j]);
             const float xh = (yy[j] - mnv[j]) * rsv[j];
-            const float t = dd[j] * actgrad_of<ACT>(z, a.in.act) * mk[j];
+            const float t = dd[j] * ag[j] * mk[j];
             g[j] = t;
             s1[j] += t; s2[j] = fmaf(t, xh, s2[j]);
           }
           *reinterpret_cast<float4*>(go + (size_t)(ih * a.wd + iw) * C) = make_float4(g[0], g[1], g[2], g[3]);
         }
-      }
-    }
+      };
+      if (SV) {
+#pragma unroll
+        for (int k = 0; k < NPI; ++k)
+          if (pl + k * lanes < a.th * a.tw) pixel(pl + k * lanes, &yi[k], &fi[k]);
+      } else {
+        for (int p = pl; p < a.th * a.tw; p += lanes) pixel(p, nullptr, nullptr);
+      }
+    }
+    if (SV && tile + 1 < tile_hi) load_interior(tile + 1);
     if (active) {
       const int noy = (a.th + s - 1) / s, nox = (a.tw + s - 1) / s;
       const int oyb = ih0 / s, oxb = iw0 / s;
@@ -1213,7 +1270,7 @@
   if (tid < ng) {
     float t1 = 0.f, t2 = 0.f;
     for (int j = 0; j < cpg; ++j) {
-      const float w = a.in.gamma[c0 + tid * cpg + j];
+      const float w = gam[tid * cpg + j];
       t1 += w * chan[(tid * cpg + j) * 2 + 0]; t2 += w * chan[(tid * cpg + j) * 2 + 1];
     }
     a.go.grows.rows[(size_t)brow * a.go.grows.W + g0 + tid] = make_float2(t1, t2);
@@ -1328,11 +1385,26 @@
   const dim3 grid((unsigned)((long)n * p.nblk * p.nslab));
   hipStream_t st = (hipStream_t)stream;
   static const bool pf = !(getenv("RN_MB_DW_NO_PF") && atoi(getenv("RN_MB_DW_NO_PF")));
-  if (in->act == RN_ACT_ELU && pf && p.tpb > 1) hipLaunchKernelGGL((mb_dw_fwd_kernel<RN_ACT_ELU, true>), grid, dim3(T), lds, st, a);
-  else if (in->act == RN_ACT_ELU) hipLaunchKernelGGL((mb_dw_fwd_kernel<RN_ACT_ELU, false>), grid, dim3(T), lds, st, a);
-  else if (in->act == RN_ACT_RELU6) hipLaunchKernelGGL((mb_dw_fwd_kernel<RN_ACT_RELU6, false>), grid, dim3(T), lds, st, a);
-  else hipLaunchKernelGGL((mb_dw_fwd_kernel<-1, false>), grid, dim3(T), lds, st, a);
+  RN_CHECK_ARG((in->saved_act != nullptr) == (in->saved_fac != nullptr), "mb depthwise fwd: saved_act and saved_fac come together");
+  float* const sa = in->saved_act; float* const sf = in->saved_fac;
+  if (sa && in->act == RN_ACT_ELU && pf && p.tpb > 1) hipLaunchKernelGGL((mb_dw_fwd_kernel<RN_ACT_ELU, true, true>), grid, dim3(T), lds, st, a, sa, sf);
+  else if (sa && in->act == RN_ACT_ELU) hipLaunchKernelGGL((mb_dw_fwd_kernel<RN_ACT_ELU, false, true>), grid, dim3(T), lds, st, a, sa, sf);
+  else if (sa) hipLaunchKernelGGL((mb_dw_fwd_kernel<-1, false, true>), grid, dim3(T), lds, st, a, sa, sf);
+  else if (in->act == RN_ACT_ELU && pf && p.tpb > 1) hipLaunchKernelGGL((mb_dw_fwd_kernel<RN_ACT_ELU, true>), grid, dim3(T), lds, st, a, sa, sf);
+  else if (in->act == RN_ACT_ELU) hipLaunchKernelGGL((mb_dw_fwd_kernel<RN_ACT_ELU, false>), grid, dim3(T), lds, st, a, sa, sf);
+  else if (in->act == RN_ACT_RELU6) hipLaunchKernelGGL((mb_dw_fwd_kernel<RN_ACT_RELU6, false>), grid, dim3(T), lds, st, a, sa, sf);
+  else hipLaunchKernelGGL((mb_dw_fwd_kernel<-1, false>), grid, dim3(T), lds, st, a, sa, sf);
   RN_LAUNCH_CHECK();
+  return RN_OK;
+}
+
+extern "C" int rn_mb_depthwise_saved_bytes(int n, int h, int w, int c, int stride, int groups, int training, size_t* bytes) {
+  RN_CHECK_ARG(bytes && n >= 1 && h >= 1 && w >= 1 && c >= 4 && groups >= 1 && c % groups == 0 && (stride == 1 || stride == 2),
+               "mb depthwise saved bytes: bad argument");
+  *bytes = 0;
+  RN_UNSUPPORTED(c % 4 || !rn_mb_depthwise_rows(n, h, w, c, stride, groups, nullptr) || (double)n * h * w * c >= 536870912.0,
+                 "mb depthwise saved bytes: shape outside rn_mb_depthwise_fwd");
+  if (training) *bytes = (size_t)n * h * w * c * sizeof(float);
   return RN_OK;
 }
 
@@ -1612,6 +1684,10 @@
   const dim3 grid((unsigned)((long)nrows * p.nslab));
   hipStream_t st = (hipStream_t)stream;
   RN_CHECK_ARG((p.tw & (p.tw - 1)) == 0, "mb depthwise bwd: tile width %d is not a power of two", p.tw);
+  RN_CHECK_ARG((in->saved_act != nullptr) == (in->saved_fac != nullptr), "mb depthwise bwd: saved_act and saved_fac come together");
+  RN_UNSUPPORTED(in->saved_act && in->act != RN_ACT_ELU, "mb depthwise bwd: the saved-activation variants are built for ELU");
+  a.save_act = in->saved_act; a.save_fac = in->saved_fac;
+  const int npi = rn::ceil_div(p.th * p.tw, T / (p.sw / 4));
 #define RN_DWB(ACT_, MULTI_)                                                                                           \
   do {                                                                                                                 \
     if (stride == 1) hipLaunchKernelGGL((mb_dw_bwd_kernel<ACT_, MULTI_, 1>), grid, dim3(T), lds, st, a);               \
@@ -1619,7 +1695,28 @@
   } while (0)
   static const bool pf_on = !(getenv("RN_MB_DWB_PF") && atoi(getenv("RN_MB_DWB_PF")) == 0);
   const int npa = rn::ceil_div((p.th + 2) * (p.tw + 2) * (p.sw / 4), T), npd = rn::ceil_div(p.oph * p.opw * (p.sw / 4), T);
-  if (in->act == RN_ACT_ELU && p.tpb > 1 && pf_on && stride == 1 && npa <= 4 && npd <= 4)
+#define RN_DWB_SV()                                                                                                                      \
+  do {                                                                                                                                   \
+    if (p.tpb > 1 && pf_on && stride == 1 && npa <= 4 && npd <= 4 && npi <= 2)                                                           \
+      hipLaunchKernelGGL((mb_dw_bwd_kernel<RN_ACT_ELU, true, 1, 4, 4, true, true, 2>), grid, dim3(T), lds, st, a);                        \
+    else if (p.tpb > 1 && pf_on && stride == 1 && npa <= 4 && npd <= 4 && npi <= 3)                                                      \
+      hipLaunchKernelGGL((mb_dw_bwd_kernel<RN_ACT_ELU, true, 1, 4, 4, true, true, 3>), grid, dim3(T), lds, st, a);                        \
+    else if (p.tpb > 1 && pf_on && stride == 1 && npa <= 4 && npd <= 4 && npi <= 4)                                                      \
+      hipLaunchKernelGGL((mb_dw_bwd_kernel<RN_ACT_ELU, true, 1, 4, 4, true, true, 4>), grid, dim3(T), lds, st, a);                        \
+    else if (p.tpb > 1 && pf_on && stride == 1 && npa <= 5 && npd <= 5 && npi <= 4)                                                      \
+      hipLaunchKernelGGL((mb_dw_bwd_kernel<RN_ACT_ELU, true, 1, 5, 5, true, true, 4>), grid, dim3(T), lds, st, a);                        \
+    else if (p.tpb > 1 && pf_on && stride == 2 && npa <= 4 && npd <= 2 && npi <= 4)                                                      \
+      hipLaunchKernelGGL((mb_dw_bwd_kernel<RN_ACT_ELU, true, 2, 4, 2, true, true, 4>), grid, dim3(T), lds, st, a);                        \
+    else if (p.tpb > 1 && pf_on && stride == 2 && npa <= 5 && npd <= 2 && npi <= 4)                                                      \
+      hipLaunchKernelGGL((mb_dw_bwd_kernel<RN_ACT_ELU, true, 2, 5, 2, true, true, 4>), grid, dim3(T), lds, st, a);                        \
+    else if (p.tpb == 1 && stride == 1) hipLaunchKernelGGL((mb_dw_bwd_kernel<RN_ACT_ELU, false, 1, NP, NP, false, true, NP>), grid, dim3(T), lds, st, a); \
+    else if (p.tpb == 1) hipLaunchKernelGGL((mb_dw_bwd_kernel<RN_ACT_ELU, false, 2, NP, NP, false, true, NP>), grid, dim3(T), lds, st, a); \
+    else if (stride == 1) hipLaunchKernelGGL((mb_dw_bwd_kernel<RN_ACT_ELU, true, 1, NP, NP, false, true, NP>), grid, dim3(T), lds, st, a); \
+    else hipLaunchKernelGGL((mb_dw_bwd_kernel<RN_ACT_ELU, true, 2, NP, NP, false, true, NP>), grid, dim3(T), lds, st, a);                 \
+  } while (0)
+  RN_CHECK_ARG(npi <= NP, "mb depthwise bwd: %d own pixels per thread", npi);
+  if (in->saved_act) RN_DWB_SV();
+  else if (in->act == RN_ACT_ELU && p.tpb > 1 && pf_on && stride == 1 && npa <= 4 && npd <= 4)
     hipLaunchKernelGGL((mb_dw_bwd_kernel<RN_ACT_ELU, true, 1, 4, 4, true>), grid, dim3(T), lds, st, a);
   else if (in->act == RN_ACT_ELU && p.tpb > 1 && pf_on && stride == 1 && npa <= 5 && npd <= 5)
     hipLaunchKernelGGL((mb_dw_bwd_kernel<RN_ACT_ELU, true, 1, 5, 5, true>), grid, dim3(T), lds, st, a);
@@ -1632,6 +1729,7 @@
   else if (in->act == RN_ACT_RELU6) RN_DWB(RN_ACT_RELU6, true);
   else RN_DWB(-1, true);
 #undef RN_DWB
+#undef RN_DWB_SV
   RN_LAUNCH_CHECK();
   return rn::launch_reduce_rows((const float*)workspace, dw, (int64_t)9 * c, nrows, 0, st);
 }
diff --git a/retinanet-tensorflow_amd/ops_mb.py b/retinanet-tensorflow_amd/ops_mb.py
--- a/retinanet-tensorflow_amd/ops_mb.py
+++ b/retinanet-tensorflow_amd/ops_mb.py
@@ -28,6 +28,7 @@
 
 
 COMPACT_ABOVE = int(os.environ.get('RN_MB_COMPACT_ABOVE', '256'))
+SAVE_A1_ABOVE = int(os.environ.get('RN_MB_SAVE_A1_ABOVE', '16384'))
 RESIDENT = os.environ.get('RN_MB_RESIDENT', '0') == '1'
 RESIDENT_MAX_HW = int(os.environ.get('RN_MB_RESIDENT_MAX_HW', '1024'))
 RESIDENT_MAX_IN_BYTES = int(os.environ.get('RN_MB_RESIDENT_MAX_IN_BYTES', str(3328 * 1024)))
@@ -48,10 +49,10 @@
 
 
 class _Stage(object):
-    __slots__ = ("y", "rows", "lay", "mean", "rstd", "norm", "c", "groups", "hw")
-
-
-def _mb_norm(st, training, seed_dev, with_rows):
+    __slots__ = ("y", "rows", "lay", "mean", "rstd", "norm", "c", "groups", "hw", "a1", "fac")
+
+
+def _mb_norm(st, training, seed_dev, with_rows, saved=False):
     nm = st.norm
     m = _rn.MbNorm()
     m.y = st.y.data_ptr()
@@ -63,7 +64,18 @@
     rate = nm.rate if training else 0.0
     m.drop_rate, m.drop_seed = rate, nm.seed
     m.drop_seed_dev = seed_dev.data_ptr() if (seed_dev is not None and rate > 0.0) else None
+    if saved and st.a1 is not None:
+        m.saved_act = st.a1.data_ptr()
+        m.saved_fac = st.fac.data_ptr()
     return m
+
+
+def saved_act_bytes(n, h, w, c, stride, groups, training, act='elu'):
+    if not training or SAVE_A1_ABOVE <= 0 or h * w < SAVE_A1_ABOVE or act != 'elu':
+        return 0
+    nbytes = C.c_size_t(0)
+    _rn.check(_rn.lib().rn_mb_depthwise_saved_bytes(n, h, w, c, stride, groups, 1, C.byref(nbytes)), "rn_mb_depthwise_saved_bytes")
+    return int(nbytes.value)
 
 
 def _count_resident(nphases):
@@ -159,6 +171,7 @@
             s.rows = torch.empty(nbytes // 4, dtype=torch.float32, device=dev)
             s.mean = torch.empty((y.shape[0], groups), dtype=torch.float32, device=dev)
             s.rstd = torch.empty((y.shape[0], groups), dtype=torch.float32, device=dev)
+            s.a1 = s.fac = None
             return s
 
         def rows_arg(s):
@@ -202,7 +215,11 @@
             y2 = torch.empty((n, oh, ow, wide), dtype=torch.float32, device=dev)
             s2 = new_stage(y2, (n, h, w, wide, stride, gr1), L.rn_mb_depthwise_rows, gr1, n2,
                            _rn.MB_PHASE_DEPTHWISE if r1 else None, (n, h, w, wide, wide, stride, gr1))
-            nm = _mb_norm(s1, training, seed_dev, True)
+            keep_bytes = 0 if r1 else saved_act_bytes(n, h, w, wide, stride, gr1, training and any(ctx.needs_input_grad), n1.act)
+            if keep_bytes:
+                s1.a1 = torch.empty(keep_bytes // 4, dtype=torch.float32, device=dev)
+                s1.fac = torch.empty(keep_bytes // 4, dtype=torch.float32, device=dev)
+            nm = _mb_norm(s1, training, seed_dev, True, saved=True)
             if r1:
                 phase(_rn.MB_PHASE_DEPTHWISE, nm, None, None, wd, y2, h, w, wide, wide, stride, s2, gr1)
             else:
@@ -337,7 +354,7 @@
             pgrads[9 * i + 6] = pw_bwd(None, s2, dy3, w3, gout, oh * ow, wide, cout)
             rows2, lay2 = _compact(rows2, lay2, n, dev)
             norm_param_grads(planes2, n2, 9 * i + 4, 9 * i + 5)
-            nm1 = _mb_norm(s1, training, seed_dev, False)
+            nm1 = _mb_norm(s1, training, seed_dev, False, saved=True)
             dy2 = _rn.MbDy(None, C.pointer(nm2), g2.data_ptr(), 0, _rn.MbRows(rows2.data_ptr(), lay2.rows_per_sample, lay2.width, lay2.bn))
             lay1, rows1, planes1 = grows_for(L.rn_mb_depthwise_bwd_rows, (n, h, w, wide, stride, s1.groups), wide)
             g1 = torch.empty_like(s1.y)
```

New measurement: 479.8 (median of 6 runs). No clear change (+0.7%).
